# dnbaker/dashing2

Measured on AMD Instinct MI355X. Metric: all-pairs sketch comparison throughput (pairs/s), higher is better.
Workload: dtype u64

## Files before the change

### dashing2_amd/capi.py

```python
import ctypes as C
import os
import subprocess

import numpy as np

_HERE = os.path.dirname(os.path.abspath(__file__))
LIB_PATH = os.environ.get("D2G_LIB") or os.path.join(_HERE, "libd2g.so")
_lib = None

SIMILARITY, CONTAINMENT, SYMMETRIC_CONTAINMENT, POISSON_LLR, INTERSECTION, UNION_SIZE = range(6)
CMP_AUTO, CMP_DIRECT, CMP_BITSLICE, CMP_PLANES = 0, 1, 2, 3
BITSLICE_OPS_PER_GROUP_EXTRA = 1


TIME_K1, TIME_K2, TIME_K2PREP, TIME_K3, TIME_K0 = 2, 4, 8, 16, 32
TIME_KNN = 64
TIME_DEDUP = 128
TIME_FILTER = 256
TIME_KSET = 512
TIME_SCREEN = 1024


class D2GError(RuntimeError):
    def __init__(self, status, detail=""):
# ... 12 lines not shown
_pu64, _pu32, _pdbl, _pf32, _pu8 = (C.POINTER(C.c_uint64), C.POINTER(C.c_uint32), C.POINTER(C.c_double),
                                    C.POINTER(C.c_float), C.POINTER(C.c_uint8))

SIGNATURES = {
    "d2g_version": (_int, []),
    "d2g_strerror": (_cp, [_int]),
    "d2g_device_count": (_int, []),
    "d2g_ctx_create": (_int, [_int, C.POINTER(_vp)]),
    "d2g_ctx_destroy": (None, [_vp]),
    "d2g_last_error": (_cp, [_vp]),
    "d2g_ctx_device": (_int, [_vp]),
    "d2g_ctx_reload_tuning": (_int, [_vp]),
    "d2g_ctx_tuning": (_int, [_vp, C.c_char_p, _sz]),
    "d2g_sync": (_int, [_vp, _vp]),
    "d2g_malloc": (_int, [_vp, _sz, C.POINTER(_vp)]),
    "d2g_free": (_int, [_vp, _vp]),
    "d2g_malloc_host": (_int, [_vp, _sz, C.POINTER(_vp)]),
    "d2g_host_register": (_int, [_vp, _vp, _sz]),
    "d2g_host_unregister": (_int, [_vp, _vp]),
    "d2g_free_host": (_int, [_vp, _vp]),
    "d2g_memcpy_h2d": (_int, [_vp, _vp, _vp, _sz, _vp]),
    "d2g_memcpy_d2h": (_int, [_vp, _vp, _vp, _sz, _vp]),
    "d2g_set_timing": (_int, [_vp, _int]),
    "d2g_kernel_ms": (_int, [_vp, _cp, _int, C.POINTER(_int), C.POINTER(_f32), C.POINTER(_f32)]),
    "d2g_wang_hash": (_u64, [_u64]),
    "d2g_wang_hash_inverse": (_u64, [_u64]),
    "d2g_oph_kmer_ids": (_int, [_vp, _sz, _sz, _sz, _vp]),
    "d2g_seed_mask": (_u64, [_u64]),
    "d2g_oph_xor_const": (_u64, []),
    "d2g_oph_m": (_sz, [_sz]),
    "d2g_oph_card": (_dbl, [_pu64, _sz]),
    "d2g_oph_signatures": (_int, [_pu64, _sz, _pdbl]),
    "d2g_oph_finalize": (_int, [_pu64, _sz, _sz, _sz, _pdbl, _pdbl, _int]),
    "d2g_densify": (_int, [_pdbl, _sz, _sz, C.POINTER(_sz), _int]),
    "d2g_epilogue_gtlt": (_f32, [_u64, _u64, _sz, _dbl, _dbl, _int, _int]),
    "d2g_epilogue_neq": (_f32, [_u64, _sz, _dbl, _dbl, _int, _int]),
    "d2g_epilogue_ut": (_int, [_vp, _vp, _vp, _sz, _sz, _sz, _sz, _int, _int, _int, _int, _vp]),
    "d2g_epilogue_lut": (_int, [_sz, _int, _int, _int, _pf32]),
    "d2g_regs_truncate": (_int, [_vp, _sz, _sz, _int, _int, _vp, _vp, _vp, _int, C.c_char_p, _sz]),
    "d2g_epilogue_trunc_neq": (_f32, [_u64, _sz, _int, _dbl, _dbl, _int, _int]),
    "d2g_epilogue_trunc_gtlt": (_f32, [_u64, _u64, _sz, _vp, _dbl, _dbl, _int, _int]),
    "d2g_epilogue_trunc_ut": (_int, [_vp, _vp, _vp, _sz, _sz, _sz, _sz, _int, _int, _int, _vp, _int, _vp]),
    "d2g_epilogue_trunc_rect": (_int, [_vp, _vp, _vp, _sz, _sz, _sz, _sz, _sz, _sz, _int, _int, _int, _vp, _int, _vp]),
    "d2g_seqpack_create": (_int, [_int, C.POINTER(_vp)]),
    "d2g_seqpack_create_alphabet": (_int, [_int, _int, C.POINTER(_vp)]),
    "d2g_seqpack_alphabet": (_int, [_vp]),
    "d2g_alphabet_size": (_int, [_int]),
    "d2g_alphabet_max_k": (_int, [_int]),
    "d2g_alphabet_code": (_int, [_int, _int]),
    "d2g_alphabet_name": (C.c_char_p, [_int]),
    "d2g_key_bits": (_int, [_int, _int]),
    "d2g_oph_plan_create_alphabet": (_int, [_vp, _vp, _vp, _sz, _vp, _sz, _int, _int, C.POINTER(_vp)]),
    "d2g_sketcher_set_alphabet": (_int, [_vp, _int]),
    "d2g_kmer_filter_create_alphabet": (_int, [_vp, _vp, _sz, _vp, _vp, _sz, _int, _int, C.POINTER(_vp)]),
    "d2g_seqpack_destroy": (None, [_vp]),
    "d2g_seqpack_clear": (None, [_vp]),
    "d2g_seqpack_add_path": (_int, [_vp, _cp]),
    "d2g_seqpack_add_fastx": (_int, [_vp, _cp, _sz]),
    "d2g_seqpack_add_sequence": (_int, [_vp, _cp, _sz]),
    "d2g_seqpack_ngenomes": (_sz, [_vp]),
    "d2g_seqpack_nruns": (_sz, [_vp]),
    "d2g_seqpack_packed_bytes": (_sz, [_vp]),
    "d2g_seqpack_packed": (_pu8, [_vp]),
    "d2g_seqpack_run_start": (_pu64, [_vp]),
    "d2g_seqpack_run_len": (_pu32, [_vp]),
    "d2g_seqpack_genome_run_off": (_pu64, [_vp]),
    "d2g_seqpack_nkmers": (_u64, [_vp, _sz]),
    "d2g_seqpack_nbases": (_u64, [_vp]),
    "d2g_oph_sketch": (_int, [_vp, _vp, _sz, _vp, _vp, _sz, _vp, _sz, _int, _int, _u64, _sz, _vp]),
    "d2g_oph_plan_create": (_int, [_vp, _vp, _vp, _sz, _vp, _sz, _int, C.POINTER(_vp)]),
    "d2g_oph_plan_create_windowed": (_int, [_vp, _vp, _vp, _sz, _vp, _sz, _int, _int, C.POINTER(_vp)]),
    "d2g_run_emissions": (_u64, [_u64, _int, _int]),
    "d2g_sketcher_set_window": (_int, [_vp, _int]),
    "d2g_oph_plan_destroy": (None, [_vp]),
    "d2g_oph_plan_nkmers": (_u64, [_vp]),
    "d2g_oph_plan_nbases": (_u64, [_vp]),
    "d2g_oph_sketch_dev": (_int, [_vp, _vp, _vp, _int, _u64, _sz, _vp, _vp]),
    "d2g_oph_count_dev": (_int, [_vp, _vp, _vp, _int, _u64, _sz, _vp, _vp, _vp]),
    "d2g_oph_sketch_counts": (_int, [_vp, _vp, _sz, _vp, _vp, _sz, _vp, _sz, _int, _int, _u64, _sz, _vp, _vp]),
    "d2g_sketcher_run_counts": (_int, [_vp, _vp, _sz, _vp, _vp, _sz, _vp, _sz, _int, _int, _u64, _sz, _vp, _vp]),
    "d2g_oph_sketch_mincount": (_int, [_vp, _vp, _sz, _vp, _vp, _sz, _vp, _sz, _int, _int, _u64, _sz, C.c_uint32, _vp, _vp]),
    "d2g_sketcher_run_mincount": (_int, [_vp, _vp, _sz, _vp, _vp, _sz, _vp, _sz, _int, _int, _u64, _sz, C.c_uint32, _vp, _vp]),
    "d2g_oph_sketch_mincount_dev": (_int, [_vp, _vp, _vp, _int, _u64, _sz, C.c_uint32, _vp, _vp]),
    "d2g_kmer_filter_create_dev": (_int, [_vp, _vp, _vp, _int, _vp, C.POINTER(_vp)]),
    "d2g_kmer_filter_create": (_int, [_vp, _vp, _sz, _vp, _vp, _sz, _int, _int, C.POINTER(_vp)]),
    "d2g_kmer_filter_create_windowed": (_int, [_vp, _vp, _sz, _vp, _vp, _sz, _int, _int, _int, C.POINTER(_vp)]),
    "d2g_kmer_filter_destroy": (None, [_vp]),
    "d2g_kmer_filter_info": (_int, [_vp, _vp, C.POINTER(_u64), C.POINTER(_u64), C.POINTER(_sz)]),
    "d2g_kmer_filter_contains": (_int, [_vp, _vp, _vp, _sz, _vp]),
    "d2g_screen_create": (_int, [_vp, _vp, _sz, _sz, _int, _int, _u64, _sz, C.POINTER(_vp)]),
    "d2g_screen_destroy": (None, [_vp]),
    "d2g_screen_table_slots": (_int, [_u64, C.POINTER(_u64)]),
    "d2g_screen_reset": (_int, [_vp, _vp]),
    "d2g_screen_info": (_int, [_vp, _vp, C.POINTER(_u64), C.POINTER(_sz), C.POINTER(_sz)]),
    "d2g_screen_fed": (_int, [_vp, _vp, _sz, C.POINTER(_u64)]),
    "d2g_screen_set_fed": (_int, [_vp, _vp, _sz, _u64]),
    "d2g_screen_add_dev": (_int, [_vp, _vp, _vp, _vp, _vp, _vp]),
    "d2g_sketcher_run_screen": (_int, [_vp, _vp, _sz, _vp, _vp, _sz, _vp, _sz, _int, _int, _vp, _vp]),
    "d2g_screen_result": (_int, [_vp, _vp, _sz, _sz, _vp, _vp]),
    "d2g_screen_key_counts": (_int, [_vp, _vp, _sz, _vp, _vp]),
    "d2g_epilogue_contain": (_int, [_vp, _vp, _sz, _sz, _vp, _vp]),
    "d2g_mem_info": (_int, [_vp, C.POINTER(_sz), C.POINTER(_sz)]),
    "d2g_seqpack_add_file": (_int, [_vp, _cp]),
    "d2g_oph_plan_set_filter": (_int, [_vp, _vp]),
    "d2g_sketcher_set_filter": (_int, [_vp, _vp]),
    "d2g_sketcher_create": (_int, [_vp, C.POINTER(_vp)]),
    "d2g_sketcher_destroy": (None, [_vp]),
    "d2g_sketcher_run": (_int, [_vp, _vp, _sz, _vp, _vp, _sz, _vp, _sz, _int, _int, _u64, _sz, _vp]),
    "d2g_sketcher_run_bmh": (_int, [_vp, _vp, _sz, _vp, _vp, _sz, _vp, _sz, _int, _int, _u64, _sz, C.c_double, _vp, _vp]),
    "d2g_bmh_sketch_dev": (_int, [_vp, _vp, _vp, _int, _u64, _sz, C.c_double, _vp, _vp, _vp]),
    "d2g_bmh_sketch": (_int, [_vp, _vp, _sz, _vp, _vp, _sz, _vp, _sz, _int, _int, _u64, _sz, C.c_double, _vp, _vp]),
    "d2g_kmer_count": (_int, [_vp, _vp, _sz, _vp, _vp, _sz, _vp, _sz, _int, _int, _u64, C.c_double, _vp, _vp, _sz, _vp]),
    "d2g_kmer_distinct": (_int, [_vp, _vp, _sz, _vp, _vp, _sz, _vp, _sz, _int, _int, _u64, _vp]),
    "d2g_kmer_sets": (_int, [_vp, _vp, _sz, _vp, _vp, _sz, _vp, _sz, _int, _int, _u64, C.c_double, _vp, _vp, _sz, _vp, _vp]),
    "d2g_sketcher_run_sets": (_int, [_vp, _vp, _sz, _vp, _vp, _sz, _vp, _sz, _int, _int, _u64, C.c_double, _vp, _vp, _sz, _vp, _vp]),
    "d2g_kmer_sets_dev": (_int, [_vp, _vp, _vp, _int, _u64, C.c_double, _vp, _vp, _sz, _vp, _vp, _vp]),
    "d2g_kset_check": (_int, [_vp, _vp, _vp, _sz, C.c_char_p, _sz]),
    "d2g_kset_create": (_int, [_vp, _vp, _vp, _vp, _sz, C.POINTER(_vp)]),
    "d2g_kset_create_dev": (_int, [_vp, _vp, _vp, _vp, _sz, _vp, C.POINTER(_vp)]),
    "d2g_kset_destroy": (None, [_vp]),
    "d2g_kset_size": (_sz, [_vp]),
    "d2g_kset_device_bytes": (_sz, [_vp]),
    "d2g_kset_slice_bits": (_int, [_vp]),
    "d2g_kset_isz_ut_dev": (_int, [_vp, _vp, _sz, _sz, _vp, _vp]),
    "d2g_kset_isz_rect_dev": (_int, [_vp, _vp, _sz, _sz, _sz, _sz, _vp, _vp]),
    "d2g_epilogue_exact": (_f32, [_u64, _dbl, _dbl, _int, _int]),
    "d2g_epilogue_exact_ut": (_int, [_vp, _vp, _sz, _sz, _sz, _int, _int, _int, _vp]),
    "d2g_epilogue_exact_rect": (_int, [_vp, _vp, _sz, _sz, _sz, _sz, _sz, _int, _int, _int, _vp]),
    "d2g_sketcher_run_distinct": (_int, [_vp, _vp, _sz, _vp, _vp, _sz, _vp, _sz, _int, _int, _u64, _vp]),
    "d2g_sketcher_ingest_fasta": (_int, [_vp, _vp, _sz, _vp, _vp, _sz, _vp, _sz, _int]),
    "d2g_sketcher_ingested_runs": (_int, [_vp, C.POINTER(_vp), C.POINTER(_vp), C.POINTER(_sz), C.POINTER(_vp), C.POINTER(_vp), C.POINTER(_u64)]),
    "d2g_seqpack_add_path_by_record": (_int, [_vp, C.c_char_p]),
    "d2g_seqpack_add_fastx_by_record": (_int, [_vp, C.c_char_p, _sz]),
    "d2g_seqpack_name": (C.c_char_p, [_vp, _sz]),
    "d2g_bmh_sketch_cs": (_int, [_vp, _vp, _sz, _vp, _vp, _sz, _vp, _sz, _int, _int, _u64, _sz, _u64, C.c_double, _vp, _vp]),
    "d2g_bmh_sketch_cs_dev": (_int, [_vp, _vp, _vp, _int, _u64, _sz, _u64, C.c_double, _vp, _vp, _vp]),
    "d2g_sketcher_run_bmh_cs": (_int, [_vp, _vp, _sz, _vp, _vp, _sz, _vp, _sz, _int, _int, _u64, _sz, _u64, C.c_double, _vp, _vp]),
    "d2g_countsketch_table": (_int, [_vp, _vp, _sz, _vp, _vp, _sz, _vp, _sz, _int, _int, _u64, _u64, _vp]),
    "d2g_countsketch_cells": (_int, [_vp, _vp, _sz, _vp, _vp, _sz, _vp, _sz, _int, _int, _u64, _u64, C.c_double, _vp, _vp, _sz, _vp, _vp]),
    "d2g_countsketch_lds_cells": (_int, []),
    "d2g_countsketch_stats": (_int, [_vp, _vp, _vp, _vp]),
    "d2g_bmh_check_weights": (_int, [_vp, _vp, _sz, _sz, _dbl, C.c_char_p, _sz]),
    "d2g_bmh_from_weighted": (_int, [_vp, _vp, _vp, _vp, _sz, _sz, _vp, _vp]),
    "d2g_bmh_from_weighted_ids": (_int, [_vp, _vp, _vp, _vp, _sz, _sz, _vp, _vp, _vp]),
    "d2g_ut_count": (_sz, [_sz, _sz, _sz]),
    "d2g_cmp_set_create_dev": (_int, [_vp, _vp, _sz, _sz, _int, _vp, C.POINTER(_vp)]),
    "d2g_cmp_set_create": (_int, [_vp, _vp, _sz, _sz, _int, C.POINTER(_vp)]),
    "d2g_cmp_set_update_dev": (_int, [_vp, _vp, _vp, _vp]),
    "d2g_cmp_set_planes": (_int, [_vp, _vp, _vp, C.POINTER(C.c_uint), C.POINTER(_int), C.POINTER(_f32)]),
    "d2g_cmp_set_status": (_int, [_vp, _vp, _vp]),
    "d2g_cmp_set_sparse_info": (_int, [_vp, _vp, _vp, _vp]),
    "d2g_cmp_set_debug_pairs": (_int, [_vp, _vp, _vp, _vp, _sz, C.POINTER(_sz), _vp]),
    "d2g_cmp_set_sparse_detail": (_int, [_vp, _vp, _vp, _vp]),
    "d2g_sparse_bin_geometry": (_int, [_sz, C.POINTER(C.c_uint32), C.POINTER(C.c_uint32), C.POINTER(C.c_uint32), C.POINTER(_int)]),
    "d2g_warmup": (_int, [_vp, _int]),
    "d2g_device_name": (_int, [_int, C.c_char_p, _sz]),
    "d2g_comm_unique_id": (_int, [_vp]),
    "d2g_comm_create": (_int, [_vp, _vp, _int, _int, C.POINTER(_vp)]),
    "d2g_comm_create_all": (_int, [C.POINTER(_vp), _int, C.POINTER(_vp)]),
    "d2g_comm_destroy": (None, [_vp]),
    "d2g_comm_rank": (_int, [_vp]),
    "d2g_comm_world": (_int, [_vp]),
    "d2g_comm_is_rccl": (_int, [_vp]),
    "d2g_bcast_sigs": (_int, [C.POINTER(_vp), C.POINTER(_vp), _int, _vp, _sz, _sz, C.POINTER(_vp)]),
    "d2g_allpairs_create": (_int, [_vp, _vp, _sz, _sz, C.POINTER(_vp)]),
    "d2g_allpairs_destroy": (None, [_vp]),
    "d2g_allpairs_rows_held": (_int, [_vp, C.POINTER(_sz), C.POINTER(_sz)]),
    "d2g_allpairs_rows_computed": (_int, [_vp, C.POINTER(_sz), C.POINTER(_sz)]),
    "d2g_allpairs_prepare_dev": (_int, [_vp, _vp, _vp]),
    "d2g_allpairs_prepare_all": (_int, [C.POINTER(_vp), _int, C.POINTER(_vp), C.POINTER(_vp)]),
    "d2g_allpairs_operand": (_vp, [_vp]),
    "d2g_allpairs_status": (_int, [_vp, _vp]),
    "d2g_allpairs_chunks": (_int, [_vp]),
    "d2g_allpairs_set_phase_timing": (_int, [_vp, _int]),
    "d2g_allpairs_phase_times": (_int, [_vp, _int, C.POINTER(_int), _vp, _vp, _vp, _vp]),
    "d2g_allpairs_sparse_info": (_int, [_vp, _vp]),
    "d2g_allpairs_step_lut_dev": (_int, [_vp, _vp, _vp, _vp, _vp]),
    "d2g_allpairs_step_eqcount_dev": (_int, [_vp, _vp, _vp, _vp]),
    "d2g_allpairs_step_all": (_int, [C.POINTER(_vp), _int, C.POINTER(_vp), C.POINTER(_vp), C.POINTER(_vp), C.POINTER(_vp)]),
    "d2g_allpairs_enqueue_lut_dev": (_int, [_vp, _vp, _vp, _vp, _vp, _int]),
    "d2g_operand_layout": (_int, [_sz, _sz, C.POINTER(_sz), C.POINTER(_sz)]),
    "d2g_cmp_set_export_operand_dev": (_int, [_vp, _vp, _vp, _vp, _vp]),
    "d2g_cmp_set_from_planes_dev": (_int, [_vp, _sz, _sz, _vp, _vp, C.POINTER(_vp)]),
    "d2g_pack_column_slices_dev": (_int, [_vp, _vp, _sz, _sz, _int, _vp, _vp]),
    "d2g_cmp_set_destroy": (None, [_vp]),
    "d2g_cmp_set_algo": (_int, [_vp]),
    "d2g_cmp_eqcount_ut_dev": (_int, [_vp, _vp, _sz, _sz, _vp, _vp]),
    "d2g_cmp_lut_ut_dev": (_int, [_vp, _vp, _sz, _sz, _vp, _vp, _vp]),
    "d2g_cmp_ut_prefill_dev": (_int, [_vp, _vp, _sz, _sz, _vp, _vp, _vp, _vp]),
    "d2g_cmp_ut_announce_dev": (_int, [_vp, _vp, _sz, _sz, _vp, _vp, _vp]),
    "d2g_cmp_set_forget": (_int, [_vp, _vp]),
    "d2g_cmp_gtlt_ut_dev": (_int, [_vp, _vp, _sz, _sz, _vp, _vp, _vp]),
    "d2g_cmp_eqcount_rect_dev": (_int, [_vp, _vp, _sz, _sz, _sz, _sz, _vp, _vp]),
    "d2g_cmp_gtlt_rect_dev": (_int, [_vp, _vp, _sz, _sz, _sz, _sz, _vp, _vp, _vp]),
    "d2g_cmp_eqcount_ut": (_int, [_vp, _vp, _sz, _sz, _sz, _sz, _int, _vp]),
    "d2g_cmp_dist_ut": (_int, [_vp, _vp, _vp, _sz, _sz, _sz, _sz, _int, _int, _int, _int, _int, _vp]),
    "d2g_ut_partition": (_int, [_sz, _int, C.POINTER(_sz)]),
    "d2g_cmp_set_create_codes_dev": (_int, [_vp, _vp, _sz, _sz, _int, _vp, C.POINTER(_vp)]),
    "d2g_cmp_set_create_codes": (_int, [_vp, _vp, _sz, _sz, _int, C.POINTER(_vp)]),
    "d2g_cmp_set_operand_bytes": (_sz, [_vp]),
    "d2g_cmp_set_id_bits": (_int, [_vp]),
    "d2g_cmp_dist_trunc_ut": (_int, [_vp, _vp, _vp, _sz, _sz, _sz, _sz, _int, _int, _int, _int, _int, _vp]),
    "d2g_cmp_knn_dev": (_int, [_vp, _vp, _sz, _sz, _sz, C.c_uint32, _vp, _sz, _vp, _vp, _vp, _sz, _vp]),
    "d2g_knn_finish": (_int, [_vp, _vp, _vp, _sz, _sz, _vp, _sz, _int, _vp, _vp, _vp, _sz, C.POINTER(_sz), C.POINTER(_sz)]),
    "d2g_cmp_set_knn": (_int, [_vp, _vp, _sz, _sz, _vp, _int, _sz, _dbl, _sz, _sz, _vp, _vp, _vp, _sz, C.POINTER(_sz)]),
    "d2g_cmp_knn": (_int, [_vp, _vp, _sz, _sz, _sz, _sz, _int, _int, _int, _int, _sz, _dbl, _sz, _sz, _vp, _vp, _vp, _sz, C.POINTER(_sz)]),
    "d2g_cmp_dedup_dev": (_int, [_vp, _vp, C.c_uint32, _vp, _vp, _sz, _vp]),
    "d2g_dedup_clusters": (_int, [_vp, _sz, _vp, _vp, C.POINTER(_sz)]),
    "d2g_cmp_set_dedup": (_int, [_vp, _vp, _vp, _dbl, _sz, _vp]),
    "d2g_cmp_dedup": (_int, [_vp, _vp, _sz, _sz, _int, _int, _int, _int, _dbl, _sz, _vp]),
}


def sparse_info_dict(a):
    return {"sorted_operand": bool(a[0]), "tiles_listed": int(a[1]), "dense_decided_by_prepare": bool(a[2] & 1), "dense_kernel_ran": bool(a[2] & 2),
            "tiles_and_pair_list": bool(a[2] & 4), "callers_order_kept": bool(a[2] & 8), "ordering_skipped": bool(a[2] & 16), "pairs_listed": int(a[3])}


def lib():
    global _lib
    if _lib is None:
        if os.environ.get("D2G_NO_TORCH_PRELOAD") != "1":
            try:
                import torch
            except Exception:
                pass
        if not os.path.exists(LIB_PATH):
            raise OSError(f"{LIB_PATH} is missing: run `python -c 'import __graft_entry__ as g; g.build()'` "
                          "(dashing2_amd has no CPU fallback)")
        l = C.CDLL(LIB_PATH)
        for name, (res, args) in SIGNATURES.items():
            try:
                f = getattr(l, name)
            except AttributeError:
                if os.environ.get("D2G_LIB"):
                    continue
                raise
            f.restype = res
            f.argtypes = args
        _lib = l
    return _lib


def _np_ptr(a):
    return a.ctypes.data if a is not None else None


class _Runs:

    def __init__(self, src, canon):
        if hasattr(src, "arrays"):
            src = tuple(src.arrays()) + (src.k,)
        elif src[0] is None:
            src = (None,) + tuple(src[1][:3]) + (src[2],)
        packed, rs, rl, go, self.k = src
        self.packed = None if packed is None else np.ascontiguousarray(packed, np.uint8)
        self.rs, self.rl, self.go = np.ascontiguousarray(rs, np.uint64), np.ascontiguousarray(rl, np.uint32), np.ascontiguousarray(go, np.uint64)
        self.n = self.go.size - 1
        self.args = (_np_ptr(self.packed), 0 if packed is None else self.packed.size, _np_ptr(self.rs), _np_ptr(self.rl), self.rs.size,
                     _np_ptr(self.go), self.n, self.k, int(canon))

    @property
    def nkmers(self):
        return int(self.rl.astype(np.int64).sum()) - (self.k - 1) * self.rl.size if self.rl.size else 0


def wang_hash(x):
    return int(lib().d2g_wang_hash(x & 0xFFFFFFFFFFFFFFFF))


def wang_hash_inverse(x):
    return int(lib().d2g_wang_hash_inverse(x & 0xFFFFFFFFFFFFFFFF))


SCREEN_MAX_KEYS = 1 << 30


def run_emissions(length, k, w=0):
    return int(lib().d2g_run_emissions(int(length), int(k), int(w)))


def countsketch_lds_cells():
    return int(lib().d2g_countsketch_lds_cells())


def screen_table_slots(ndistinct):
    s = _u64()
    rc = lib().d2g_screen_table_slots(ndistinct, C.byref(s))
    if rc:
        raise D2GError(rc)
    return int(s.value)


def epilogue_contain(matches, matchsums, S):
    m = np.ascontiguousarray(matches, np.uint32)
    s = np.ascontiguousarray(matchsums, np.uint32)
    cov, dep = np.empty(m.shape, np.float32), np.empty(m.shape, np.float32)
    rc = lib().d2g_epilogue_contain(_np_ptr(m), _np_ptr(s), m.size, S, _np_ptr(cov), _np_ptr(dep))
    if rc:
        raise D2GError(rc)
    return cov, dep


def oph_kmer_ids(regs, S):
    regs = np.ascontiguousarray(regs, np.uint64)
    n, m = regs.shape
# ... 885 lines not shown

    def close(self):
        if getattr(self, "_h", None):
            lib().d2g_kmer_filter_destroy(self._h)
            self._h = None

    __del__ = close


class Screen:

    def __init__(self, ctx, h, nrefs, S, k, canon, nrows):
        self.ctx, self._h, self.nrefs, self.S, self.k, self.canon, self.nrows = ctx, h, nrefs, S, k, canon, nrows

    def info(self):
        nd, tb, cb = _u64(), _sz(), _sz()
        self.ctx._check(lib().d2g_screen_info(self.ctx._h, self._h, C.byref(nd), C.byref(tb), C.byref(cb)))
        return int(nd.value), int(tb.value), int(cb.value)

    def reset(self):
        self.ctx._check(lib().d2g_screen_reset(self.ctx._h, self._h))

    def fed(self, row):
        n = _u64()
        self.ctx._check(lib().d2g_screen_fed(self.ctx._h, self._h, row, C.byref(n)))
        return int(n.value)

    def set_fed(self, row, nkmers):
        self.ctx._check(lib().d2g_screen_set_fed(self.ctx._h, self._h, row, nkmers))

    def add_dev(self, plan, packed_dev_ptr, genome_row, stream=None):
        rows = np.ascontiguousarray(genome_row, np.uint32)
        assert rows.size == plan.n
        self.ctx._check(lib().d2g_screen_add_dev(self.ctx._h, self._h, plan._h, packed_dev_ptr, _np_ptr(rows), stream))

    def result(self, row0=0, nrows=None):
        nrows = self.nrows - row0 if nrows is None else nrows
        m = np.zeros((nrows, self.nrefs), np.uint32)
        s = np.zeros((nrows, self.nrefs), np.uint32)
        self.ctx._check(lib().d2g_screen_result(self.ctx._h, self._h, row0, nrows, _np_ptr(m), _np_ptr(s)))
        return m, s

    def key_counts(self, row):
        D = self.info()[0]
        keys, cnt = np.zeros(D, np.uint64), np.zeros(D, np.uint32)
        self.ctx._check(lib().d2g_screen_key_counts(self.ctx._h, self._h, row, _np_ptr(keys), _np_ptr(cnt)))
        return keys, cnt

    def close(self):
        if getattr(self, "_h", None):
            lib().d2g_screen_destroy(self._h)
            self._h = None

    __del__ = close


class KSet:

    def __init__(self, ctx, h):
        self.ctx, self._h = ctx, h
        self.N = int(lib().d2g_kset_size(h))

    @property
    def device_bytes(self):
        return int(lib().d2g_kset_device_bytes(self._h))

    @property
    def slice_bits(self):
        return int(lib().d2g_kset_slice_bits(self._h))

    def isz_ut_dev(self, r0, r1, out_dev_ptr, stream=None):
        self.ctx._check(lib().d2g_kset_isz_ut_dev(self.ctx._h, self._h, r0, r1, out_dev_ptr, stream))

    def isz_rect_dev(self, a0, a1, b0, b1, out_dev_ptr, stream=None):
        self.ctx._check(lib().d2g_kset_isz_rect_dev(self.ctx._h, self._h, a0, a1, b0, b1, out_dev_ptr, stream))

    def close(self):
        if getattr(self, "_h", None):
            lib().d2g_kset_destroy(self._h)
            self._h = None

    __del__ = close


class OphPlan:
    def __init__(self, ctx, h, n):
        self.ctx, self._h, self.n = ctx, h, n

    def set_filter(self, filt):
        self.ctx._check(lib().d2g_oph_plan_set_filter(self._h, filt._h if filt is not None else None))
        self._filter = filt

    @property
    def nkmers(self):
        return int(lib().d2g_oph_plan_nkmers(self._h))

    @property
    def nbases(self):
        return int(lib().d2g_oph_plan_nbases(self._h))

    def close(self):
        if self._h:
            lib().d2g_oph_plan_destroy(self._h)
            self._h = None

    __del__ = close


class CmpSet:

    def __init__(self, ctx, h, N, S, owned=True):
        self.ctx, self._h, self.N, self.S, self._owned = ctx, h, N, S, owned

    @property
    def algo(self):
        return int(lib().d2g_cmp_set_algo(self._h))

    @property
    def operand_bytes(self):
        return int(lib().d2g_cmp_set_operand_bytes(self._h))

    @property
    def id_bits(self):
        return int(lib().d2g_cmp_set_id_bits(self._h))

    def close(self):
        if getattr(self, "_h", None):
            if self._owned:
                lib().d2g_cmp_set_destroy(self._h)
            self._h = None

    __del__ = close

    def export_operand_dev(self, planes_out_ptr, meta_out_ptr, stream=None):
        self.ctx._check(lib().d2g_cmp_set_export_operand_dev(self.ctx._h, self._h, planes_out_ptr, meta_out_ptr, stream))

    def update_dev(self, dev_ptr, stream=None):
        self.ctx._check(lib().d2g_cmp_set_update_dev(self.ctx._h, self._h, dev_ptr, stream))

    def status(self, stream=None):
        self.ctx._check(lib().d2g_cmp_set_status(self.ctx._h, self._h, stream))

    def sparse_info(self, stream=None):
        a = np.zeros(4, np.uint32)
        self.ctx._check(lib().d2g_cmp_set_sparse_info(self.ctx._h, self._h, stream, a.ctypes.data))
        return sparse_info_dict(a)

    def sparse_detail(self, stream=None):
        a = np.zeros(10, np.uint64)
        self.ctx._check(lib().d2g_cmp_set_sparse_detail(self.ctx._h, self._h, stream, a.ctypes.data))
        return {"looked": bool(a[0]), "looked_dense": bool(a[1]), "entries": int(a[2]), "family_pairs": int(a[3]), "shared_values": int(a[4]),
                "planes": int(a[5]), "binned": bool(a[6]), "bin_cshift": int(a[7]), "schedule": "merged" if a[8] else "classic", "prepare_kernels": int(a[9])}

    def debug_pairs(self, cap=1 << 24, stream=None):
        buf = np.empty(cap, np.uint64)
        roots = np.empty(self.N, np.uint32)
        n = _sz()
        self.ctx._check(lib().d2g_cmp_set_debug_pairs(self.ctx._h, self._h, stream, buf.ctypes.data, cap, C.byref(n), roots.ctypes.data))
        e = buf[:n.value]
        e = e[e != np.uint64(0xFFFFFFFFFFFFFFFF)]
        return np.stack([(e & np.uint64(0xFFFFFFFF)).astype(np.uint32), (e >> np.uint64(32)).astype(np.uint32)], axis=1), roots

    def planes(self, stream=None):
        md, nb, mean = C.c_uint(), _int(), _f32()
        self.ctx._check(lib().d2g_cmp_set_planes(self.ctx._h, self._h, stream, C.byref(md), C.byref(nb), C.byref(mean)))
        return int(md.value), int(nb.value), float(mean.value)

    def eqcount_ut_dev(self, out_dev_ptr, r0=0, r1=None, stream=None):
        r1 = self.N if r1 is None else r1
        self.ctx._check(lib().d2g_cmp_eqcount_ut_dev(self.ctx._h, self._h, r0, r1, out_dev_ptr, stream))

    def lut_ut_dev(self, lut_dev_ptr, out_dev_ptr, r0=0, r1=None, stream=None):
        r1 = self.N if r1 is None else r1
        self.ctx._check(lib().d2g_cmp_lut_ut_dev(self.ctx._h, self._h, r0, r1, lut_dev_ptr, out_dev_ptr, stream))

    def prefill_ut_dev(self, out_dev_ptr, r0=0, r1=None, lut_dev_ptr=None, stream=None):
        r1 = self.N if r1 is None else r1
        if lut_dev_ptr is None:
            self.ctx._check(lib().d2g_cmp_ut_prefill_dev(self.ctx._h, self._h, r0, r1, out_dev_ptr, None, None, stream))
        else:
            self.ctx._check(lib().d2g_cmp_ut_prefill_dev(self.ctx._h, self._h, r0, r1, None, lut_dev_ptr, out_dev_ptr, stream))

    def forget(self):
        self.ctx._check(lib().d2g_cmp_set_forget(self.ctx._h, self._h))

    def announce_ut_dev(self, out_dev_ptr, r0=0, r1=None, lut_dev_ptr=None):
        r1 = self.N if r1 is None else r1
        if lut_dev_ptr is None:
            self.ctx._check(lib().d2g_cmp_ut_announce_dev(self.ctx._h, self._h, r0, r1, out_dev_ptr, None, None))
        else:
            self.ctx._check(lib().d2g_cmp_ut_announce_dev(self.ctx._h, self._h, r0, r1, None, lut_dev_ptr, out_dev_ptr))

    def gtlt_ut_dev(self, gt_dev_ptr, lt_dev_ptr, r0=0, r1=None, stream=None):
        r1 = self.N if r1 is None else r1
        self.ctx._check(lib().d2g_cmp_gtlt_ut_dev(self.ctx._h, self._h, r0, r1, gt_dev_ptr, lt_dev_ptr, stream))

    def eqcount_rect_dev(self, out_dev_ptr, a0, a1, b0, b1, stream=None):
        self.ctx._check(lib().d2g_cmp_eqcount_rect_dev(self.ctx._h, self._h, a0, a1, b0, b1, out_dev_ptr, stream))

    def knn_dev(self, rowcnt_dev_ptr, ids_dev_ptr, counts_dev_ptr, cap, K=0, min_count=0, cls_dev_ptr=None, r0=0, r1=None,
                band_rows=0, stream=None):
        r1 = self.N if r1 is None else r1
        self.ctx._check(lib().d2g_cmp_knn_dev(self.ctx._h, self._h, r0, r1, K, min_count, cls_dev_ptr, cap, rowcnt_dev_ptr, ids_dev_ptr,
                                              counts_dev_ptr, band_rows, stream))

    def knn(self, lut, isdist=False, K=0, threshold=0.0, r0=0, r1=None, cap=0, band_rows=0):
        lut = np.ascontiguousarray(lut, np.float32)
        assert lut.size == self.S + 1
        r1 = self.N if r1 is None else r1
        return _knn_csr(self.ctx, r1 - r0, K, lambda ip, ix, dt, oc, need: lib().d2g_cmp_set_knn(
            self.ctx._h, self._h, r0, r1, _np_ptr(lut), int(bool(isdist)), K, float(threshold), cap, band_rows, ip, ix, dt, oc, need))

    def dedup_dev(self, assign_dev_ptr, min_count, cls_dev_ptr=None, band_rows=0, stream=None):
        self.ctx._check(lib().d2g_cmp_dedup_dev(self.ctx._h, self._h, min_count, cls_dev_ptr, assign_dev_ptr, band_rows, stream))

    def dedup(self, lut, threshold, band_rows=0):
        lut = np.ascontiguousarray(lut, np.float32)
        assert lut.size == self.S + 1
        out = np.empty(self.N, np.uint32)
        self.ctx._check(lib().d2g_cmp_set_dedup(self.ctx._h, self._h, _np_ptr(lut), float(threshold), band_rows, _np_ptr(out)))
        return out

    def gtlt_rect_dev(self, gt_dev_ptr, lt_dev_ptr, a0, a1, b0, b1, stream=None):
        self.ctx._check(lib().d2g_cmp_gtlt_rect_dev(self.ctx._h, self._h, a0, a1, b0, b1, gt_dev_ptr, lt_dev_ptr, stream))

    def eqcount_ut(self, r0=0, r1=None):
        r1 = self.N if r1 is None else r1
        out = np.empty(ut_count(self.N, r0, r1) if r0 <= r1 <= self.N else 0, np.uint32)
        d = self.ctx.malloc(max(out.nbytes, 4))
        try:
            self.eqcount_ut_dev(d, r0, r1)
            if out.size:
                self.ctx.d2h(out, d)
        finally:
            self.ctx.free(d)
        return out

    def gtlt_ut(self, r0=0, r1=None):
        r1 = self.N if r1 is None else r1
        n = ut_count(self.N, r0, r1)
        gt, lt = np.empty(n, np.uint32), np.empty(n, np.uint32)
        if n == 0:
            return gt, lt
        dg, dl = self.ctx.malloc(gt.nbytes), self.ctx.malloc(lt.nbytes)
        try:
            self.gtlt_ut_dev(dg, dl, r0, r1)
            self.ctx.d2h(gt, dg)
            self.ctx.d2h(lt, dl)
        finally:
            self.ctx.free(dg)
            self.ctx.free(dl)
        return gt, lt

    def gtlt_rect(self, a0, a1, b0, b1):
        gt, lt = np.empty((a1 - a0, b1 - b0), np.uint32), np.empty((a1 - a0, b1 - b0), np.uint32)
        if gt.size == 0:
            return gt, lt
        dg, dl = self.ctx.malloc(gt.nbytes), self.ctx.malloc(lt.nbytes)
        try:
            self.gtlt_rect_dev(dg, dl, a0, a1, b0, b1)
            self.ctx.d2h(gt, dg)
            self.ctx.d2h(lt, dl)
        finally:
            self.ctx.free(dg)
            self.ctx.free(dl)
        return gt, lt

    def eqcount_rect(self, a0, a1, b0, b1):
        out = np.empty((a1 - a0, b1 - b0), np.uint32)
        if out.size == 0:
            return out
        d = self.ctx.malloc(out.nbytes)
        try:
            self.eqcount_rect_dev(d, a0, a1, b0, b1)
            self.ctx.d2h(out, d)
        finally:
            self.ctx.free(d)
        return out

    def lut_ut(self, lut, r0=0, r1=None):
        r1 = self.N if r1 is None else r1
        lut = np.ascontiguousarray(lut, np.float32)
        out = np.empty(ut_count(self.N, r0, r1), np.float32)
        if out.size == 0:
            return out
        dl, d = self.ctx.malloc(lut.nbytes), self.ctx.malloc(out.nbytes)
        try:
            self.ctx.h2d(dl, lut)
            self.lut_ut_dev(dl, d, r0, r1)
            self.ctx.d2h(out, d)
        finally:
            self.ctx.free(dl)
            self.ctx.free(d)
        return out


COMM_ID_BYTES = 128


def comm_unique_id():
    buf = C.create_string_buffer(COMM_ID_BYTES)
    rc = lib().d2g_comm_unique_id(buf)
    if rc:
        raise D2GError(rc, "d2g_comm_unique_id (RCCL not loadable?)")
    return buf.raw

# ... 124 lines not shown
```

### dashing2_amd/csrc/d2g_internal.h

```cpp
#pragma once
#include "../../include/d2g.h"
#include <hip/hip_runtime.h>
#include <cstdio>
#include <memory>
#include <string>
#include <utility>

#include <vector>
struct d2g_ctx;
int d2g_hip_status(d2g_ctx *ctx, hipError_t e, const char *what);

template <class T, bool Pinned> class d2g_owned {
    T *p_ = nullptr; size_t cap_ = 0;
public:
    d2g_owned() = default;
    d2g_owned(d2g_owned &&o) noexcept : p_(o.p_), cap_(o.cap_) { o.p_ = nullptr; o.cap_ = 0; }
    d2g_owned &operator=(d2g_owned &&o) noexcept { if (this != &o) { reset(); p_ = o.p_; cap_ = o.cap_; o.p_ = nullptr; o.cap_ = 0; } return *this; }
    ~d2g_owned() { reset(); }
    void reset() { if (p_) (void)(Pinned ? hipHostFree(p_) : hipFree(p_)); p_ = nullptr; cap_ = 0; }
    int alloc(d2g_ctx *ctx, size_t n, const char *what, unsigned flags = hipHostMallocDefault) {
        reset();
        const hipError_t e = Pinned ? hipHostMalloc((void **)&p_, n * sizeof(T), flags) : hipMalloc((void **)&p_, n * sizeof(T));
        if (e != hipSuccess) p_ = nullptr; else cap_ = n;
        return d2g_hip_status(ctx, e, what);
    }
    int grow(d2g_ctx *ctx, size_t need, size_t slack, const char *what = "work buffer", unsigned flags = hipHostMallocDefault) {
        return need <= cap_ ? D2G_OK : alloc(ctx, need + need / 4 + slack, what, flags);
    }
    T *get() const { return p_; }
    operator T *() const { return p_; }
    size_t cap() const { return cap_; }
};
template <class T> using d2g_dev = d2g_owned<T, false>;
template <class T> using d2g_pinned = d2g_owned<T, true>;

template <class H, hipError_t (*Destroy)(H)> class d2g_handle {
protected:
    H h_ = nullptr;
public:
    d2g_handle() = default;
    d2g_handle(d2g_handle &&o) noexcept : h_(o.h_) { o.h_ = nullptr; }
    d2g_handle &operator=(d2g_handle &&o) noexcept { if (this != &o) { reset(); h_ = o.h_; o.h_ = nullptr; } return *this; }
    ~d2g_handle() { reset(); }
    void reset() { if (h_) (void)Destroy(h_); h_ = nullptr; }
    operator H() const { return h_; }
};
struct d2g_stream : d2g_handle<hipStream_t, hipStreamDestroy> {
    hipError_t create(unsigned flags = hipStreamDefault) { reset(); return hipStreamCreateWithFlags(&h_, flags); }
};
struct d2g_event : d2g_handle<hipEvent_t, hipEventDestroy> {
    hipError_t create(unsigned flags = hipEventDefault) { reset(); return hipEventCreateWithFlags(&h_, flags); }
};

struct d2g_evlog {
    std::vector<d2g_event> a, b;
};

struct d2g_tuning {
    std::vector<std::pair<std::string, std::string>> kv;
    const char *get(const char *name) const {
        for (const auto &p : kv) if (p.first == name) return p.second.c_str();
        return nullptr;
    }
};
void d2g_tuning_load(d2g_tuning &t);
struct d2g_k2_tuning {
    bool sparse = true;
    size_t min_n = 8192;
    int link = 1;
    double tile_frac = 0.35;
    int olink = 1;
    int emit_big = 0;
    int ride = 63;
    int merge = 1;
    int remember = 1;
    size_t long_list = 786432;
    int predict = 1;
    int list_form = 0;
    size_t list_div = 8;
    bool sort = true;
    int tagbits_max = 31;
    int id16 = 1;
    int nsplit_req = 0;
};
d2g_k2_tuning d2g_k2_tuning_resolve(const d2g_tuning &t);
std::string d2g_k2_tuning_json(const d2g_ctx *ctx);
uint64_t d2g_k2_tuning_hash(const d2g_ctx *ctx);

constexpr int K3_MAXBBITS = 12;
constexpr int K3_ROUND_KEYS = 1400;
constexpr int K3_TARGET = 1024;
constexpr int K3_L1BITS = 8;
constexpr uint64_t K3_SPLIT_MIN = 4 * 1400;
struct d2g_k3_tuning {
    bool compact = false;
    bool light = true;
    uint32_t l1bits = K3_L1BITS;
    uint64_t bucket_keys = K3_TARGET;
    uint64_t sub_keys = K3_TARGET;
    uint64_t split_min = 0;
    size_t subbatch = 0;
    uint32_t round_keys = K3_ROUND_KEYS;
    double guess_scale = 1.0;
    size_t grid_per_cu = 48;
    bool gq_scale_set = false;
    double gq_scale = 2.0;
    uint64_t gq_slack = 256;
    uint64_t sort_keys = K3_TARGET;
    uint64_t cs_table_bytes = 0;
    int cs_lds_cells = -1;
};
struct d2g_kset_tuning {
    int split = 0;
    int pbits = -1;
};
d2g_k3_tuning d2g_k3_tuning_resolve(const d2g_tuning &t);
constexpr int MG_MAX_CHUNKS = 4;
void d2g_tuning_resolve(d2g_ctx *ctx);

struct d2g_ctx {
    int device = -1;
    d2g_tuning tune;
    d2g_k2_tuning k2;
    d2g_k3_tuning k3_tune;
    d2g_kset_tuning kset;
    int mgpu_chunks = 0;
    int num_cus = 0;
    std::string last_error;
    int timing = 0;
    d2g_evlog ev_k1, ev_k2, ev_k2prep, ev_k3, ev_k0, ev_knn;
    d2g_evlog ev_k1count;
    d2g_evlog ev_filter;
    d2g_evlog ev_k3k, ev_k3kcompact, ev_k3kbmh;
    d2g_evlog ev_k3s, ev_kset, ev_ksetprep;
    d2g_evlog ev_screen, ev_screenreduce, ev_screenbuild;
    d2g_evlog ev_dedup, ev_dedup_resolve;
    struct d2g_k3_state *k3 = nullptr;
    uint64_t cs_table_bytes = 0, cs_groups = 0, cs_batches = 0;
    d2g_dev<uint32_t> knn_band;
    d2g_dev<unsigned long long> dedup_keys;
};
void d2g_k3_state_destroy(struct d2g_k3_state *st);
void d2g_screen_rank_keys(const uint64_t *keys, size_t n, uint64_t xormask, std::vector<uint64_t> &distinct, std::vector<uint64_t> &raw,
                          std::vector<uint32_t> &rank);
inline int d2g_hip_status(d2g_ctx *ctx, hipError_t e, const char *what) {
    if (e == hipSuccess) return D2G_OK;
    ctx->last_error = std::string(what) + ": " + hipGetErrorString(e);
    return e == hipErrorOutOfMemory ? D2G_ERR_NOMEM : D2G_ERR_HIP;
}

#define D2G_HIP(ctx, call)                                                            \
    do {                                                                              \
        hipError_t e__ = (call);                                                      \
        if (e__ != hipSuccess) {                                                      \
            (ctx)->last_error = std::string(#call) + ": " + hipGetErrorString(e__);   \
            return e__ == hipErrorOutOfMemory ? D2G_ERR_NOMEM : D2G_ERR_HIP;          \
        }                                                                             \
    } while (0)

#define D2G_CHECK(ctx, cond, msg)                      \
    do {                                               \
        if (!(cond)) {                                 \
            (ctx)->last_error = (msg);                 \
            return D2G_ERR_INVALID;                    \
        }                                              \
    } while (0)

struct d2g_timer {
    d2g_evlog *ev; hipStream_t s; bool on;
    d2g_timer(d2g_ctx *c, d2g_evlog *e, hipStream_t st) : ev(e), s(st), on(false) {
        const int bit = (e == &c->ev_k1 || e == &c->ev_k1count) ? D2G_TIME_K1 : e == &c->ev_k2 ? D2G_TIME_K2 : e == &c->ev_k2prep ? D2G_TIME_K2PREP : e == &c->ev_k0 ? D2G_TIME_K0 : e == &c->ev_knn ? D2G_TIME_KNN : e == &c->ev_filter ? D2G_TIME_FILTER : (e == &c->ev_k3s || e == &c->ev_kset || e == &c->ev_ksetprep) ? D2G_TIME_KSET : (e == &c->ev_dedup || e == &c->ev_dedup_resolve) ? D2G_TIME_DEDUP : (e == &c->ev_screen || e == &c->ev_screenreduce || e == &c->ev_screenbuild) ? D2G_TIME_SCREEN : D2G_TIME_K3;
        on = (c->timing & bit) != 0;
        if (on) {
            d2g_event x, y;
            if (x.create() != hipSuccess || y.create() != hipSuccess) { on = false; return; }
            (void)hipEventRecord(x, s);
            ev->a.push_back(std::move(x)); ev->b.push_back(std::move(y));
        }
    }
    void stop() { if (on) (void)hipEventRecord(ev->b.back(), s); }
};

void d2g_warm_filter(); void d2g_warm_k0(); void d2g_warm_k1(); void d2g_warm_k2(); void d2g_warm_k2_bitslice(); void d2g_warm_k2_planes(); void d2g_warm_k3(); void d2g_warm_kset(); void d2g_warm_screen(); void d2g_warm_knn(); void d2g_warm_dedup();

static inline hipStream_t as_stream(void *s) { return reinterpret_cast<hipStream_t>(s); }

template <class T> static inline T div_up(T a, T b) { return (a + b - 1) / b; }
```

### dashing2_amd/csrc/d2g_k2.h

```cpp
#pragma once
#include "d2g_internal.h"

#include <algorithm>

struct SpRider { uint32_t *out; size_t cnt; const uint32_t *vsrc; uint32_t vimm, own, piece0; };
constexpr SpRider SP_NO_RIDER{nullptr, 0, nullptr, 0u, 0xFFFFFFFFu, 0u};
constexpr int SP_FILL_PER_THREAD = 8, SP_FILL_THREADS = 256;
inline size_t sp_fill_pieces(size_t cnt) { return div_up<size_t>(cnt / 4 + 1, (size_t)SP_FILL_THREADS * SP_FILL_PER_THREAD); }
#ifndef D2G_SP_RW_M_LINK0
#define D2G_SP_RW_M_LINK0 8
#endif
#ifndef D2G_SP_RW_M_PLANES
#define D2G_SP_RW_M_PLANES 5
#endif
constexpr unsigned SP_RW_PLAN = 6, SP_RW_FLATTEN = 5, SP_RW_COUNT = 5, SP_RW_ATTACH = 5, SP_RW_SCAN = 8, SP_RW_ALL = 35;
constexpr unsigned SP_RW_M_LINK0 = D2G_SP_RW_M_LINK0, SP_RW_M_PLANES = D2G_SP_RW_M_PLANES;

struct SpInit {
    uint32_t *label = nullptr, *ones = nullptr, *zero = nullptr;
    uint32_t n = 0, owords = 0, zwords = 0;
};
#ifdef __HIPCC__
__device__ __forceinline__ void sp_init_part(const SpInit &si, size_t lin, size_t nthreads) {
    if (!si.label) return;
    if (lin < si.n) si.label[lin] = (uint32_t)lin;
    for (size_t x = lin; x < si.owords; x += nthreads) si.ones[x] = 0xFFFFFFFFu;
    for (size_t x = lin; x < si.zwords; x += nthreads) si.zero[x] = 0;
}
#endif

struct SpAnnounced {
    uint32_t *out = nullptr; size_t cnt = 0; const uint32_t *vsrc = nullptr; uint32_t vimm = 0;
    uint32_t next = 0, total = 0;
    int mask = 0;
    void announce(uint32_t *o, size_t n, const uint32_t *src) { out = o; cnt = n; vsrc = src; vimm = 0; }
    void cancel() { out = nullptr; }
    void served() { out = nullptr; total = 0; }
    void begin(int ride_mask, bool carry) {
        mask = ride_mask; next = 0;
        const size_t pieces = sp_fill_pieces(cnt);
        total = (out && carry && mask && pieces <= 0x7FFFFFFFu) ? (uint32_t)pieces : 0u;
    }
    uint32_t riding() const { return total; }
    SpRider take_all() { next = total; return SpRider{out, cnt, vsrc, vimm, 0u, 0u}; }
    SpRider take(unsigned own, unsigned weight, bool last, int bit, unsigned *grid) {
        *grid = own;
        if (next >= total || !(mask & bit)) return SP_NO_RIDER;
        const uint32_t left = total - next;
        uint32_t n = last ? left : (uint32_t)std::min<uint64_t>(left, ((uint64_t)total * weight + SP_RW_ALL - 1) / SP_RW_ALL);
        n = std::min<uint32_t>(n, 0x7FFFFFFFu - own);
        const SpRider r{out, cnt, vsrc, vimm, own, next};
        next += n;
        *grid = own + n;
        return r;
    }
};

struct SpFilled {
    uint32_t *out = nullptr;
    size_t cnt = 0;
    size_t pieces = 0;
    const uint32_t *src = nullptr;
    bool by_riders = false;
    void set_early(uint32_t *o, size_t n, const uint32_t *s) { out = o; cnt = n; pieces = (size_t)-1; src = s; by_riders = false; }
    void set_by_riders(const SpAnnounced &a) { out = a.out; cnt = a.cnt; pieces = a.next; src = a.vsrc; by_riders = true; }
    size_t done_for(const uint32_t *o, size_t n, const uint32_t *s, size_t npieces) const { return (out == o && cnt == n && src == s) ? std::min(pieces, npieces) : 0; }
    void void_after_prepare() { if (by_riders) out = nullptr; }
    void clear() { out = nullptr; }
};

enum SpMappedWord : uint32_t { SP_MW_GAVEUP = 0, SP_MW_LIST_LEN = 1, SP_MW_SUMS = 2, SP_MW_TICKET = 6, SP_MW_WORDS = 16 };

struct SpDecision {
    unsigned prepares = 0; bool skipped = false;
    bool merged = false; unsigned kernels = 0;
    int skip_cached = -1;
    bool sample_pending = false; uint32_t sample_ticket = 0;
    bool pred_valid = false, pred_dense = false; double pred_entries = 0, pred_family_pairs = 0;
    bool big = true;
    bool looked = false, looked_dense = false; uint32_t samp_sums[4] = {0, 0, 0, 0};
};

struct SpState {
    unsigned sp_launch = 0;
    d2g_dev<uint32_t> d_stream_s;
    d2g_dev<uint32_t> d_sperm;
    d2g_dev<uint32_t> d_sinv;
    d2g_dev<uint32_t> d_label;
    d2g_dev<uint32_t> d_owner;
    size_t owner_stride = 0;
    d2g_dev<uint32_t> d_segend;
    d2g_dev<uint32_t> d_posseg;
    d2g_dev<uint32_t> d_hint;
    d2g_dev<uint32_t> d_spz;
    size_t spz_words = 0;
    uint32_t *d_lcnt = nullptr;
    uint32_t *d_gbm = nullptr;
    uint32_t *d_order = nullptr;
    uint32_t *d_plctl = nullptr;
    d2g_dev<uint32_t> d_rowpos;
    d2g_dev<uint32_t> d_rowk;
    d2g_dev<uint32_t> d_rowstream;
    d2g_dev<uint32_t> d_tiles, d_spctl; uint32_t *d_tilebm = nullptr;
    d2g_dev<uint32_t> d_tiles_full; uint32_t *d_fullctl = nullptr;
    bool full_list_valid = false;
    d2g_pinned<uint32_t> h_gaveup; uint32_t *d_gaveup = nullptr;
    d2g_stream fill_stream; d2g_event fill_fork, fill_join;
    d2g_stream samp_stream; d2g_event samp_event;
    d2g_dev<uint32_t> d_samp;
    SpDecision dec;
    SpAnnounced announced;
    SpFilled filled;
    const uint32_t *last_ctl = nullptr;
    d2g_dev<unsigned long long> d_plist;
    size_t plist_cap = 0;
    d2g_dev<unsigned long long> d_plist2;
    uint32_t *d_binc = nullptr;
    d2g_dev<uint32_t> d_bstart;
    d2g_dev<uint32_t> d_cw_ents; d2g_dev<unsigned long long> d_cw_vals; size_t cw_ecap = 0, cw_vcap = 0;
    d2g_dev<uint32_t> d_hoff;
    uint32_t nbins = 0, bin_nch = 0, bin_cshift = 10, bin_nwg = 1;
    bool bin_ok = true;
    size_t tilebm_words = 0, tiles_cap = 0;
};

struct d2g_cmp_set {
    d2g_ctx *ctx = nullptr;
    size_t N = 0, S = 0;
    size_t Npad = 0;
    int algo = D2G_CMP_DIRECT;
    d2g_dev<uint64_t> d_rows;
    d2g_dev<uint64_t> d_cols;
    d2g_dev<uint32_t> d_cplanes;
    int cplanes = 0;
    d2g_dev<uint32_t> own_planes, own_meta;
    uint32_t *d_planes = nullptr;
    d2g_dev<uint32_t> d_stream;
    size_t Nstride = 0;
    int nbits_cap = 0;
    int ntb = 0;
    uint32_t *d_meta = nullptr;
    d2g_dev<uint32_t> d_ids;
    int id_bits = 32;
    uint32_t T = 0; int logT = 0;
    bool borrowed = false;
    bool want_exchange = false;
    d2g_dev<uint32_t> d_colcnt;
    d2g_dev<uint32_t> d_perm;
    int nsplit = 1;
    bool export_only = false;
    uint32_t *ex_planes = nullptr, *ex_meta = nullptr, *ex_status = nullptr;
    bool managed = false;
    const uint32_t *status_words = nullptr; int n_status = 0;
    std::unique_ptr<SpState> sp;
    bool sparse_ok() const { return sp != nullptr; }
    size_t ncols = 0;
    bool srt_valid = false;
    mutable bool nat_valid = false;
};
constexpr int BS_CC_STRIDE = 8;

struct PairShape;
int  finish_shape(d2g_ctx *ctx, PairShape &sh, unsigned rb);

int  d2g_planes_gtlt(d2g_ctx *ctx, const d2g_cmp_set *set, const PairShape &sh, uint32_t *gt, uint32_t *lt, hipStream_t s);
int  d2g_planes_eq(d2g_ctx *ctx, const d2g_cmp_set *set, const PairShape &sh, uint32_t *eq, hipStream_t s);

void d2g_bitslice_geometry(d2g_cmp_set *set);
int  d2g_bitslice_alloc(d2g_ctx *ctx, d2g_cmp_set *set);
int  d2g_bitslice_prepare(d2g_ctx *ctx, d2g_cmp_set *set, hipStream_t s);
int  d2g_bitslice_export(d2g_ctx *ctx, d2g_cmp_set *set, hipStream_t s);
int  d2g_bitslice_alloc_stream(d2g_ctx *ctx, d2g_cmp_set *set);
int  d2g_bitslice_ensure_natural(d2g_ctx *ctx, const d2g_cmp_set *set, hipStream_t s);
int  d2g_bitslice_managed_sparse_alloc(d2g_ctx *ctx, d2g_cmp_set *set);
int  d2g_bitslice_managed_ready(d2g_ctx *ctx, d2g_cmp_set *set, hipStream_t s);
int  d2g_bitslice_sparse_info(d2g_ctx *ctx, const d2g_cmp_set *set, hipStream_t s, uint32_t *out4);
int  d2g_bitslice_sparse_detail(d2g_ctx *ctx, const d2g_cmp_set *set, hipStream_t s, uint64_t *out10);
SpInit d2g_bitslice_sp_init(const d2g_cmp_set *set);
int  d2g_bitslice_debug_read(d2g_ctx *ctx, const d2g_cmp_set *set, hipStream_t s, uint64_t *pairs_out, size_t cap, size_t *npairs, uint32_t *root_out);
int  d2g_bitslice_status(d2g_ctx *ctx, const d2g_cmp_set *set, hipStream_t s);
int  d2g_bitslice_exporter_create(d2g_ctx *ctx, size_t N, size_t S_local, d2g_cmp_set **out);
void d2g_bitslice_set_export_target(d2g_cmp_set *set, uint32_t *planes, uint32_t *meta, uint32_t *status);
int  d2g_bitslice_prepare_slice(d2g_ctx *ctx, d2g_cmp_set *set, const uint64_t *rows_dev, hipStream_t s);
int  d2g_bitslice_derive_groups(d2g_ctx *ctx, const d2g_cmp_set *set, int g0, int g1, hipStream_t s);
int  d2g_bitslice_ut(d2g_ctx *ctx, const d2g_cmp_set *set, size_t r0, size_t r1, uint32_t *eq_out,
                     const float *lut, float *fout, hipStream_t s);
int  d2g_bitslice_prefill(d2g_ctx *ctx, d2g_cmp_set *set, size_t r0, size_t r1, uint32_t *eq_out, const float *lut, float *fout, hipStream_t s);
int  d2g_bitslice_announce(d2g_ctx *ctx, d2g_cmp_set *set, size_t r0, size_t r1, uint32_t *eq_out, const float *lut, float *fout);
void d2g_bitslice_forget(d2g_cmp_set *set);
int  d2g_bitslice_rect(d2g_ctx *ctx, const d2g_cmp_set *set, size_t a0, size_t a1, size_t b0, size_t b1,
                       uint32_t *eq_out, hipStream_t s);
```

### dashing2_amd/csrc/d2g_k2.hip

```cpp
#include "d2g_internal.h"
#include "d2g_k2.h"
#include "d2g_k2_shape.h"
#include <algorithm>
#include <new>
#include <vector>

namespace {

constexpr int K2_THREADS = 256;
constexpr int K2_IW = 8;
constexpr int K2_JR = 4;
constexpr int K2_RB = 4 * K2_IW;
constexpr int K2_CB = 64 * K2_JR;
constexpr int K2_TC = 2;

}
int finish_shape(d2g_ctx *ctx, PairShape &sh, unsigned rb) {
    sh.rb = rb;
    sh.nrt = (unsigned)div_up<size_t>(sh.i_hi - sh.i_lo, rb);
    sh.ct0 = (unsigned)(sh.j_lo / 256);
    sh.nct = (unsigned)(div_up<size_t>(sh.j_hi, 256) - sh.ct0);
    size_t total = 0;
    for (unsigned c = 0; c < sh.nct; ++c) total += tiles_in_column(sh, c);
    D2G_CHECK(ctx, total < (1ull << 31), "pair tile grid too large; shard rows");
// ... 147 lines not shown
    delete set;
}

int d2g_cmp_set_algo(const d2g_cmp_set *set) { return set ? set->algo : D2G_ERR_INVALID; }

int d2g_cmp_set_id_bits(const d2g_cmp_set *set) { return (set && set->algo == D2G_CMP_BITSLICE && set->d_ids) ? set->id_bits : 0; }

size_t d2g_cmp_set_operand_bytes(const d2g_cmp_set *set) {
    if (!set) return 0;
    return (set->d_rows.cap() + set->d_cols.cap()) * sizeof(uint64_t) +
           (set->own_planes.cap() + set->d_stream.cap() + (set->sp ? set->sp->d_stream_s.cap() : 0) + set->d_cplanes.cap()) * sizeof(uint32_t);
}

#define D2G_NO_CODE_SET(ctx, set, what) D2G_CHECK(ctx, (set)->algo != D2G_CMP_PLANES, what ": not available for a set of truncated codes")

static int cmp_set_load(d2g_ctx *ctx, d2g_cmp_set *set, const uint64_t *sig_bits_dev, hipStream_t s) {
    const size_t N = set->N, S = set->S;
    if (set->d_rows) D2G_HIP(ctx, hipMemcpyAsync(set->d_rows, sig_bits_dev, N * S * sizeof(uint64_t), hipMemcpyDeviceToDevice, s));
    d2g_timer tm(ctx, &ctx->ev_k2prep, s);
    launch_transpose(ctx, sig_bits_dev, set->d_cols, N, S, set->Npad, set->algo == D2G_CMP_BITSLICE ? set->d_meta + set->ntb : nullptr,
                     set->algo == D2G_CMP_BITSLICE ? d2g_bitslice_sp_init(set) : SpInit{}, s);
    int rc = D2G_OK;
    if (set->algo == D2G_CMP_BITSLICE) rc = d2g_bitslice_prepare(ctx, set, s);
    tm.stop();
    if (rc) return rc;
    D2G_HIP(ctx, hipGetLastError());
    return D2G_OK;
}

}

int d2g_bitslice_prepare_slice(d2g_ctx *ctx, d2g_cmp_set *set, const uint64_t *rows_dev, hipStream_t s) {
    d2g_timer tm(ctx, &ctx->ev_k2prep, s);
    launch_transpose(ctx, rows_dev, set->d_cols, set->N, set->S, set->Npad, set->d_meta + set->ntb, d2g_bitslice_sp_init(set), s);
    const int rc = d2g_bitslice_prepare(ctx, set, s);
    tm.stop();
    if (rc) return rc;
    D2G_HIP(ctx, hipGetLastError());
    return D2G_OK;
}

extern "C" {

int d2g_cmp_set_create_dev(d2g_ctx *ctx, const uint64_t *sig_bits_dev, size_t N, size_t S, int algo,
                           void *stream, d2g_cmp_set **out) {
    if (!ctx || !out) return D2G_ERR_INVALID;
    *out = nullptr;
    D2G_CHECK(ctx, N >= 1 && S >= 1, "cmp_set: empty matrix");
    D2G_CHECK(ctx, S < (1ull << 31), "cmp_set: sketchsize too large");
    D2G_CHECK(ctx, sig_bits_dev != nullptr, "cmp_set: null signatures");
    D2G_CHECK(ctx, algo == D2G_CMP_AUTO || algo == D2G_CMP_DIRECT || algo == D2G_CMP_BITSLICE, "cmp_set: bad algo");
    D2G_HIP(ctx, hipSetDevice(ctx->device));
    hipStream_t s = as_stream(stream);
    d2g_cmp_set *set = new (std::nothrow) d2g_cmp_set();
    if (!set) return D2G_ERR_NOMEM;
    set->ctx = ctx; set->N = N; set->S = S;
    set->Npad = div_up<size_t>(N, K2_CB) * K2_CB;
    if (int rc = set->d_cols.alloc(ctx, set->Npad * S, "cmp_set alloc")) { d2g_cmp_set_destroy(set); return rc; }
    set->algo = D2G_CMP_DIRECT;
    if (algo != D2G_CMP_DIRECT) {
        int rc = d2g_bitslice_alloc(ctx, set);
        if (rc == D2G_OK) set->algo = D2G_CMP_BITSLICE;
        else if (!(rc == D2G_ERR_UNSUPPORTED && algo == D2G_CMP_AUTO)) { d2g_cmp_set_destroy(set); return rc; }
    }
    if (set->algo == D2G_CMP_DIRECT) {
        if (int rc = set->d_rows.alloc(ctx, (N + K2_RB) * S, "cmp_set alloc")) { d2g_cmp_set_destroy(set); return rc; }
        (void)hipMemsetAsync(set->d_rows + N * S, 0, (size_t)K2_RB * S * sizeof(uint64_t), s);
    }
    int rc = cmp_set_load(ctx, set, sig_bits_dev, s);
    if (rc) { d2g_cmp_set_destroy(set); return rc; }
    *out = set;
    return D2G_OK;
}

int d2g_cmp_set_update_dev(d2g_ctx *ctx, d2g_cmp_set *set, const uint64_t *sig_bits_dev, void *stream) {
    if (!ctx) return D2G_ERR_INVALID;
    D2G_CHECK(ctx, set && set->ctx == ctx, "cmp_set_update: set belongs to another context");
    D2G_CHECK(ctx, !set->borrowed, "cmp_set_update: this set wraps a caller-owned operand");
    D2G_NO_CODE_SET(ctx, set, "cmp_set_update");
    D2G_CHECK(ctx, sig_bits_dev != nullptr, "cmp_set_update: null signatures");
    D2G_HIP(ctx, hipSetDevice(ctx->device));
    return cmp_set_load(ctx, set, sig_bits_dev, as_stream(stream));
}

int d2g_cmp_set_planes(d2g_ctx *ctx, const d2g_cmp_set *set, void *stream, unsigned *max_distinct, int *nbits, float *mean_nbits) {
    if (!ctx) return D2G_ERR_INVALID;
    D2G_CHECK(ctx, set && set->ctx == ctx, "cmp_set_planes: set belongs to another context");
    unsigned md = 0; int nb = 0;
    if (set->algo == D2G_CMP_BITSLICE) {
        std::vector<unsigned> m(set->ntb);
        D2G_HIP(ctx, hipSetDevice(ctx->device));
        D2G_HIP(ctx, hipMemcpyAsync(m.data(), set->d_meta, m.size() * sizeof(unsigned), hipMemcpyDeviceToHost, as_stream(stream)));
        D2G_HIP(ctx, hipStreamSynchronize(as_stream(stream)));
        double sum = 0;
        if (int rc = d2g_bitslice_status(ctx, set, as_stream(stream))) return rc;
        for (unsigned x : m) {
            md = std::max(md, x);
            int b = 1;
            while ((1ull << b) <= x) ++b;
            nb = std::max(nb, b);
            sum += b;
        }
        if (mean_nbits) *mean_nbits = m.empty() ? 0.f : float(sum / m.size());
    } else if (mean_nbits) *mean_nbits = 0.f;
    if (max_distinct) *max_distinct = md;
    if (nbits) *nbits = nb;
    return D2G_OK;
}

int d2g_cmp_set_create(d2g_ctx *ctx, const uint64_t *sig_bits_host, size_t N, size_t S, int algo, d2g_cmp_set **out) {
    if (!ctx || !out) return D2G_ERR_INVALID;
    D2G_CHECK(ctx, sig_bits_host != nullptr && N >= 1 && S >= 1, "cmp_set: bad host matrix");
    D2G_HIP(ctx, hipSetDevice(ctx->device));
    d2g_dev<uint64_t> tmp;
    if (int rc = tmp.alloc(ctx, N * S, "cmp_set staging alloc")) return rc;
    hipError_t e = hipMemcpy(tmp, sig_bits_host, N * S * sizeof(uint64_t), hipMemcpyHostToDevice);
    if (e != hipSuccess) { ctx->last_error = hipGetErrorString(e); return D2G_ERR_HIP; }
    int rc = d2g_cmp_set_create_dev(ctx, tmp, N, S, algo, nullptr, out);
    (void)hipStreamSynchronize(nullptr);
    if (rc == D2G_OK && (*out)->algo == D2G_CMP_BITSLICE && d2g_bitslice_status(ctx, *out, nullptr) != D2G_OK) {
        d2g_cmp_set_destroy(*out);
        *out = nullptr;
        rc = algo == D2G_CMP_AUTO ? d2g_cmp_set_create_dev(ctx, tmp, N, S, D2G_CMP_DIRECT, nullptr, out) : (int)D2G_ERR_INTERNAL;
        (void)hipStreamSynchronize(nullptr);
    }
    return rc;
}

int d2g_cmp_set_sparse_info(d2g_ctx *ctx, const d2g_cmp_set *set, void *stream, uint32_t *info4) {
    if (!ctx || !set || !info4) return D2G_ERR_INVALID;
    D2G_NO_CODE_SET(ctx, set, "cmp_set_sparse_info");
    D2G_HIP(ctx, hipSetDevice(ctx->device));
    if (set->algo != D2G_CMP_BITSLICE) { info4[0] = info4[1] = info4[2] = info4[3] = 0; return D2G_OK; }
    return d2g_bitslice_sparse_info(ctx, set, as_stream(stream), info4);
}

int d2g_cmp_set_debug_pairs(d2g_ctx *ctx, const d2g_cmp_set *set, void *stream, uint64_t *pairs_out, size_t cap, size_t *npairs, uint32_t *root_out) {
    if (!ctx || !set || !npairs) return D2G_ERR_INVALID;
    D2G_NO_CODE_SET(ctx, set, "cmp_set_debug_pairs");
    D2G_HIP(ctx, hipSetDevice(ctx->device));
    *npairs = 0;
    if (set->algo != D2G_CMP_BITSLICE) return D2G_OK;
    return d2g_bitslice_debug_read(ctx, set, as_stream(stream), pairs_out, cap, npairs, root_out);
}

int d2g_cmp_set_sparse_detail(d2g_ctx *ctx, const d2g_cmp_set *set, void *stream, uint64_t *out10) {
    if (!ctx || !out10) return D2G_ERR_INVALID;
    D2G_CHECK(ctx, set && set->ctx == ctx, "cmp_set_sparse_detail: set belongs to another context");
    D2G_NO_CODE_SET(ctx, set, "cmp_set_sparse_detail");
    D2G_HIP(ctx, hipSetDevice(ctx->device));
    for (int x = 0; x < 10; ++x) out10[x] = 0;
    if (set->algo != D2G_CMP_BITSLICE) { D2G_HIP(ctx, hipStreamSynchronize(as_stream(stream))); return D2G_OK; }
    return d2g_bitslice_sparse_detail(ctx, set, as_stream(stream), out10);
}

int d2g_cmp_set_status(d2g_ctx *ctx, const d2g_cmp_set *set, void *stream) {
    if (!ctx) return D2G_ERR_INVALID;
    D2G_CHECK(ctx, set && set->ctx == ctx, "cmp_set_status: set belongs to another context");
    D2G_HIP(ctx, hipSetDevice(ctx->device));
    if (set->algo != D2G_CMP_BITSLICE) { D2G_HIP(ctx, hipStreamSynchronize(as_stream(stream))); return D2G_OK; }
    return d2g_bitslice_status(ctx, set, as_stream(stream));
}

static int check_rows(d2g_ctx *ctx, const d2g_cmp_set *set, size_t r0, size_t r1) {
    D2G_CHECK(ctx, set && set->ctx == ctx, "cmp: set belongs to another context");
    D2G_CHECK(ctx, r0 <= r1 && r1 <= set->N, "cmp: row range out of bounds");
    return D2G_OK;
}

int d2g_cmp_eqcount_ut_dev(d2g_ctx *ctx, const d2g_cmp_set *set, size_t r0, size_t r1, uint32_t *out, void *stream) {
    if (!ctx) return D2G_ERR_INVALID;
    if (int rc = check_rows(ctx, set, r0, r1)) return rc;
    if (d2g_ut_count(set->N, r0, r1) == 0) return D2G_OK;
    D2G_CHECK(ctx, out != nullptr, "cmp: null output");
    D2G_HIP(ctx, hipSetDevice(ctx->device));
    if (set->algo == D2G_CMP_BITSLICE) return d2g_bitslice_ut(ctx, set, r0, r1, out, nullptr, nullptr, as_stream(stream));
    if (set->algo == D2G_CMP_PLANES) return d2g_planes_eq(ctx, set, ut_shape(set->N, r0, r1), out, as_stream(stream));
    return launch_direct<false>(ctx, set, ut_shape(set->N, r0, r1), StoreEq{out}, as_stream(stream));
}

int d2g_cmp_lut_ut_dev(d2g_ctx *ctx, const d2g_cmp_set *set, size_t r0, size_t r1, const float *lut, float *out, void *stream) {
    if (!ctx) return D2G_ERR_INVALID;
    if (int rc = check_rows(ctx, set, r0, r1)) return rc;
    D2G_NO_CODE_SET(ctx, set, "cmp_lut_ut");
    if (d2g_ut_count(set->N, r0, r1) == 0) return D2G_OK;
    D2G_CHECK(ctx, out != nullptr && lut != nullptr, "cmp: null output/lut");
    D2G_HIP(ctx, hipSetDevice(ctx->device));
    if (set->algo == D2G_CMP_BITSLICE) return d2g_bitslice_ut(ctx, set, r0, r1, nullptr, lut, out, as_stream(stream));
    return launch_direct<false>(ctx, set, ut_shape(set->N, r0, r1), StoreLut{out, lut}, as_stream(stream));
}

int d2g_cmp_ut_prefill_dev(d2g_ctx *ctx, d2g_cmp_set *set, size_t r0, size_t r1, uint32_t *neq_out, const float *lut, float *out, void *stream) {
    if (!ctx) return D2G_ERR_INVALID;
    if (int rc = check_rows(ctx, set, r0, r1)) return rc;
    D2G_NO_CODE_SET(ctx, set, "cmp_ut_prefill");
    if (d2g_ut_count(set->N, r0, r1) == 0) return D2G_OK;
    D2G_CHECK(ctx, (neq_out != nullptr) != (lut != nullptr && out != nullptr), "cmp prefill: give the count output, or the table and the float output");
    if (set->algo != D2G_CMP_BITSLICE) return D2G_OK;
    D2G_HIP(ctx, hipSetDevice(ctx->device));
    return d2g_bitslice_prefill(ctx, set, r0, r1, neq_out, lut, out, as_stream(stream));
}

int d2g_cmp_ut_announce_dev(d2g_ctx *ctx, d2g_cmp_set *set, size_t r0, size_t r1, uint32_t *neq_out, const float *lut, float *out) {
    if (!ctx) return D2G_ERR_INVALID;
    if (int rc = check_rows(ctx, set, r0, r1)) return rc;
    D2G_NO_CODE_SET(ctx, set, "cmp_ut_announce");
    if (d2g_ut_count(set->N, r0, r1) == 0) return D2G_OK;
    if (set->algo != D2G_CMP_BITSLICE || set->borrowed) return D2G_OK;
    D2G_CHECK(ctx, (!neq_out && !out) || (neq_out != nullptr) != (lut != nullptr && out != nullptr), "cmp announce: give the count output, or the table and the float output");
    return d2g_bitslice_announce(ctx, set, r0, r1, neq_out, lut, out);
}

int d2g_cmp_set_forget(d2g_ctx *ctx, d2g_cmp_set *set) {
    if (!ctx) return D2G_ERR_INVALID;
    D2G_CHECK(ctx, set && set->ctx == ctx, "cmp_set_forget: set belongs to another context");
    if (set->algo == D2G_CMP_BITSLICE) d2g_bitslice_forget(set);
    return D2G_OK;
}

int d2g_cmp_gtlt_ut_dev(d2g_ctx *ctx, const d2g_cmp_set *set, size_t r0, size_t r1, uint32_t *gt, uint32_t *lt, void *stream) {
    if (!ctx) return D2G_ERR_INVALID;
    if (int rc = check_rows(ctx, set, r0, r1)) return rc;
    if (d2g_ut_count(set->N, r0, r1) == 0) return D2G_OK;
    D2G_CHECK(ctx, gt != nullptr && lt != nullptr, "cmp: null output");
    if (set->algo == D2G_CMP_PLANES) {
        D2G_HIP(ctx, hipSetDevice(ctx->device));
        return d2g_planes_gtlt(ctx, set, ut_shape(set->N, r0, r1), gt, lt, as_stream(stream));
    }
    D2G_CHECK(ctx, set->d_rows != nullptr, "cmp: (gt,lt) needs the raw patterns: create the set with D2G_CMP_DIRECT");
    D2G_HIP(ctx, hipSetDevice(ctx->device));
    return launch_direct<true>(ctx, set, ut_shape(set->N, r0, r1), StoreGtLt{gt, lt, (uint32_t)set->S}, as_stream(stream));
}

int d2g_cmp_eqcount_rect_dev(d2g_ctx *ctx, const d2g_cmp_set *set, size_t a0, size_t a1, size_t b0, size_t b1,
                             uint32_t *out, void *stream) {
    if (!ctx) return D2G_ERR_INVALID;
    D2G_CHECK(ctx, set && set->ctx == ctx, "cmp: set belongs to another context");
    D2G_CHECK(ctx, a0 <= a1 && a1 <= set->N && b0 <= b1 && b1 <= set->N, "cmp: rect out of bounds");
    if (a0 == a1 || b0 == b1) return D2G_OK;
    D2G_CHECK(ctx, out != nullptr, "cmp: null output");
    D2G_HIP(ctx, hipSetDevice(ctx->device));
    const PairShape sh = rect_shape(set->N, a0, a1, b0, b1);
    if (set->algo == D2G_CMP_BITSLICE) return d2g_bitslice_rect(ctx, set, a0, a1, b0, b1, out, as_stream(stream));
    if (set->algo == D2G_CMP_PLANES) return d2g_planes_eq(ctx, set, sh, out, as_stream(stream));
    return launch_direct<false>(ctx, set, sh, StoreEq{out}, as_stream(stream));
}

int d2g_cmp_gtlt_rect_dev(d2g_ctx *ctx, const d2g_cmp_set *set, size_t a0, size_t a1, size_t b0, size_t b1,
                          uint32_t *gt, uint32_t *lt, void *stream) {
    if (!ctx) return D2G_ERR_INVALID;
    D2G_CHECK(ctx, set && set->ctx == ctx, "cmp: set belongs to another context");
    D2G_CHECK(ctx, a0 <= a1 && a1 <= set->N && b0 <= b1 && b1 <= set->N, "cmp: rect out of bounds");
    if (a0 == a1 || b0 == b1) return D2G_OK;
    D2G_CHECK(ctx, gt != nullptr && lt != nullptr, "cmp: null output");
    D2G_CHECK(ctx, set->d_rows != nullptr || set->algo == D2G_CMP_PLANES, "cmp: (gt,lt) needs the raw patterns: create the set with D2G_CMP_DIRECT");
    D2G_HIP(ctx, hipSetDevice(ctx->device));
    const PairShape sh = rect_shape(set->N, a0, a1, b0, b1);
    if (set->algo == D2G_CMP_PLANES) return d2g_planes_gtlt(ctx, set, sh, gt, lt, as_stream(stream));
    return launch_direct<true>(ctx, set, sh, StoreGtLt{gt, lt, (uint32_t)set->S}, as_stream(stream));
}

int d2g_operand_layout(size_t N, size_t S, size_t *group_words, size_t *ngroups) {
    if (!N || !S) return D2G_ERR_INVALID;
    d2g_cmp_set tmp;
    tmp.N = N; tmp.S = S; tmp.Npad = div_up<size_t>(N, K2_CB) * K2_CB;
    d2g_bitslice_geometry(&tmp);
    if (group_words) *group_words = (size_t)(tmp.nbits_cap + 1) * tmp.Nstride;
    if (ngroups) *ngroups = (size_t)tmp.ntb;
    return D2G_OK;
}

int d2g_cmp_set_export_operand_dev(d2g_ctx *ctx, const d2g_cmp_set *set, uint32_t *planes_out_dev, uint32_t *meta_out_dev, void *stream) {
    if (!ctx) return D2G_ERR_INVALID;
    D2G_CHECK(ctx, set && set->ctx == ctx, "export_operand: set belongs to another context");
    D2G_CHECK(ctx, set->algo == D2G_CMP_BITSLICE, "export_operand: not a bit-sliced set");
    D2G_CHECK(ctx, planes_out_dev && meta_out_dev, "export_operand: null output");
    D2G_HIP(ctx, hipSetDevice(ctx->device));
    const size_t words = (size_t)set->ntb * (set->nbits_cap + 1) * set->Nstride;
    if (int rc = d2g_bitslice_export(ctx, const_cast<d2g_cmp_set *>(set), as_stream(stream))) return rc;
    D2G_HIP(ctx, hipMemcpyAsync(planes_out_dev, set->d_planes, words * sizeof(uint32_t), hipMemcpyDeviceToDevice, as_stream(stream)));
    D2G_HIP(ctx, hipMemcpyAsync(meta_out_dev, set->d_meta, (size_t)set->ntb * sizeof(uint32_t), hipMemcpyDeviceToDevice, as_stream(stream)));
    return D2G_OK;
}

int d2g_cmp_set_from_planes_dev(d2g_ctx *ctx, size_t N, size_t S, const uint32_t *planes_dev, const uint32_t *meta_dev, d2g_cmp_set **out) {
    if (!ctx || !out) return D2G_ERR_INVALID;
    *out = nullptr;
    D2G_CHECK(ctx, N >= 1 && S >= 1 && N < (1ull << 30) && S < (1ull << 31), "from_planes: bad shape");
    D2G_CHECK(ctx, planes_dev && meta_dev, "from_planes: null operand");
    d2g_cmp_set *set = new (std::nothrow) d2g_cmp_set();
    if (!set) return D2G_ERR_NOMEM;
    set->ctx = ctx; set->N = N; set->S = S;
    set->Npad = div_up<size_t>(N, K2_CB) * K2_CB;
    d2g_bitslice_geometry(set);
    set->algo = D2G_CMP_BITSLICE;
    set->borrowed = true;
    set->d_planes = const_cast<uint32_t *>(planes_dev);
    set->d_meta = const_cast<uint32_t *>(meta_dev);
    D2G_HIP(ctx, hipSetDevice(ctx->device));
    if (int rc = d2g_bitslice_alloc_stream(ctx, set)) { delete set; return rc; }
    *out = set;
    return D2G_OK;
}

int d2g_pack_column_slices_dev(d2g_ctx *ctx, const uint64_t *rows_dev, size_t n, size_t S, int W, uint64_t *out_dev, void *stream) {
    if (!ctx) return D2G_ERR_INVALID;
// ... 79 lines not shown
```

### dashing2_amd/csrc/d2g_k2_bitslice.hip

```cpp
#include "d2g_internal.h"
#include "d2g_k2.h"
#include "d2g_k2_shape.h"
#include <chrono>
#include <cstring>
#include <algorithm>
#include <vector>

namespace {

typedef uint32_t u32x16 __attribute__((ext_vector_type(16)));
typedef u32x16 __attribute__((aligned(4))) u32x16_u;
constexpr uint32_t BS_EMPTY = 0xFFFFFFFFu;
constexpr int BS_RANK_THREADS = 1024;

constexpr uint32_t BS_DUP = 0x80000000u;
constexpr uint32_t BS_UNIQ = 0x80000000u;
constexpr uint32_t BS_PENDING = 0x40000000u;
constexpr int BS_LOG_TLDS_MAX = 15;
template <typename IdT> struct BsId;
template <> struct BsId<uint32_t> { static constexpr uint32_t UNIQ = BS_UNIQ; static constexpr int UBIT = 31; };
template <> struct BsId<uint16_t> { static constexpr uint32_t UNIQ = 0x8000u; static constexpr int UBIT = 15; };
constexpr size_t BS_ID16_MAX_N = ((size_t(1) << BS_LOG_TLDS_MAX) * 2) / 3;
static_assert(BS_ID16_MAX_N / 2 < BsId<uint16_t>::UNIQ, "16-bit ids: the highest rank (N / 2) must stay below the unique flag");
static_assert((size_t(1) << BS_LOG_TLDS_MAX) - 1 <= 0xFFFFu, "16-bit ids: the general single-partition kernel parks a table slot in ids[] between its two loops");

__device__ __forceinline__ uint32_t bs_hash(uint64_t v, int logT) {
    return (uint32_t)((v * 0x9E3779B97F4A7C15ull) >> (64 - logT));
}

constexpr uint32_t BS_SPLIT_SHIFT = 28, BS_RANK_MASK = (1u << BS_SPLIT_SHIFT) - 1u;
#ifdef D2G_RANK_TRACE
__device__ unsigned long long g_rank_trace[8192 * 16];
#define RK_STAMP(k) do { if (threadIdx.x == 0 && blockIdx.x < 8192 && (k) < 16) g_rank_trace[blockIdx.x * 16 + (k)] = __builtin_amdgcn_s_memrealtime(); } while (0)
#else
#define RK_STAMP(k) do { } while (0)
#endif
template <bool MULTI, bool FAST, typename IdT = uint32_t>
__global__ __launch_bounds__(BS_RANK_THREADS) void bs_rank_kernel(const uint64_t *__restrict__ cols, size_t N, size_t Npad,
                                                                  uint32_t T, int logT, void *ids_void, uint32_t *colcnt,
                                                                  uint32_t *status, int tagbits_max, uint32_t S, int nsplit,
                                                                  uint32_t *__restrict__ owner_all, size_t ostride) {
    extern __shared__ __attribute__((aligned(16))) uint32_t own[];
    const uint32_t split = MULTI ? blockIdx.x / S : 0u;
    const size_t t = MULTI ? blockIdx.x - split * S : blockIdx.x;
    const uint32_t htag = (MULTI && nsplit > 1) ? split << BS_SPLIT_SHIFT : 0u;
    const uint64_t *col = cols + t * Npad;
    static_assert(!MULTI || sizeof(IdT) == 4, "bs_rank_kernel: the pending words and split tags of the MULTI kernel need 32-bit ids");
    IdT *ids = static_cast<IdT *>(ids_void) + t * Npad;
    const int tid = threadIdx.x;
    const int logTl = logT < BS_LOG_TLDS_MAX ? logT : BS_LOG_TLDS_MAX;
    const uint32_t Tl = 1u << logTl, mask = Tl - 1, nparts = MULTI ? (T >> logTl) : 1u;
    const uint32_t part_lo = MULTI ? split * (nparts / (uint32_t)nsplit) : 0u, part_hi = MULTI ? part_lo + nparts / (uint32_t)nsplit : 1u;
    __shared__ uint32_t wave_tot[BS_RANK_THREADS / 64];
    __shared__ uint32_t running;
    constexpr uint32_t BS_MAXFIX = 64;
    __shared__ uint32_t nfix, fix_j[BS_MAXFIX], fix_h[BS_MAXFIX];
    RK_STAMP(0);
    if (tid == 0) { running = 1; nfix = 0; }
    const int lane = tid & 63, wave = tid >> 6;
    uint32_t *owner = (owner_all && nsplit == 1) ? owner_all + t * ostride : nullptr;
    const int ib0 = 32 - __clz((uint32_t)N);
    const uint32_t ownmask = (ib0 >= 32 ? 0xFFFFFFFFu : (1u << ib0) - 1u) & ~BS_DUP;

    auto compact = [&]() {
        uint32_t cnt = 0;
        for (uint32_t h = tid; h < Tl; h += BS_RANK_THREADS) {
            const uint32_t cur = own[h];
            cnt += (cur != BS_EMPTY) && (cur & BS_DUP);
        }
        uint32_t incl = cnt;
        for (int o = 1; o < 64; o <<= 1) { const uint32_t x = __shfl_up(incl, o); if (lane >= o) incl += x; }
        if (lane == 63) wave_tot[wave] = incl;
        __syncthreads();
        uint32_t woff = 0, tot = 0;
        for (int w = 0; w < BS_RANK_THREADS / 64; ++w) {
            const uint32_t x = wave_tot[w];
            if (w < wave) woff += x;
            tot += x;
        }
        uint32_t r = running + woff + (incl - cnt);
        for (uint32_t h = tid; h < Tl; h += BS_RANK_THREADS) {
            const uint32_t cur = own[h];
            if (cur != BS_EMPTY) {
                if ((cur & BS_DUP) && owner) owner[r - 1] = cur & ownmask;
                own[h] = (cur & BS_DUP) ? (r++ | htag) : BsId<IdT>::UNIQ;
            }
        }
        __syncthreads();
        if (tid == 0) running += tot;
        __syncthreads();
    };
    const int ib = 32 - __clz((uint32_t)N);
    const uint32_t idxmask = (ib >= 32 ? 0xFFFFFFFFu : (1u << ib) - 1u) & ~BS_DUP;
    const uint32_t tagfield = ~BS_DUP & ~idxmask & (ib + tagbits_max >= 31 ? 0xFFFFFFFFu : (1u << (ib + tagbits_max)) - 1u);
    auto slot_word = [&](uint64_t prod, uint32_t j) {
        return j | ((uint32_t)((prod << logT) >> 33) & tagfield);
    };
    auto insert = [&](uint64_t v, uint32_t j, uint32_t h) {
        const uint32_t mine = slot_word(v * 0x9E3779B97F4A7C15ull, j);
        for (uint32_t probes = 0; probes < Tl; ++probes) {
            const uint32_t cur = atomicCAS(&own[h], BS_EMPTY, mine);
            if (cur == BS_EMPTY) return h;
            if (!((cur ^ mine) & tagfield) && col[cur & idxmask] == v) {
                if (!(cur & BS_DUP)) atomicOr(&own[h], BS_DUP);
                return h;
            }
            h = (h + 1) & mask;
        }
        atomicOr(status, 1u);
        return h;
    };

    constexpr int PF = 12;
    if constexpr (FAST) {
        uint64_t v[PF];
        uint32_t hs[PF];
#pragma unroll
        for (int i = 0; i < PF; ++i) {
            const size_t j = (size_t)i * BS_RANK_THREADS + tid;
            v[i] = j < N ? col[j] : 0;
        }
        for (uint32_t h = tid; h < Tl; h += BS_RANK_THREADS) own[h] = BS_EMPTY;
        __syncthreads();
        RK_STAMP(1);
        uint32_t candidate = 0;
#pragma unroll
        for (int i = 0; i < PF; ++i) {
            const size_t j = (size_t)i * BS_RANK_THREADS + tid;
            hs[i] = 0;
            if (j < N) {
                const uint64_t prod = v[i] * 0x9E3779B97F4A7C15ull;
                const uint32_t mine = slot_word(prod, (uint32_t)j);
                uint32_t h = (uint32_t)(prod >> (64 - logT)) & mask, probes = 0;
                for (; probes < Tl; ++probes) {
                    const uint32_t cur = atomicCAS(&own[h], BS_EMPTY, mine);
                    if (cur == BS_EMPTY) break;
                    if (!((cur ^ mine) & tagfield)) { candidate |= 1u << i; break; }
                    h = (h + 1) & mask;
                }
                if (probes == Tl) atomicOr(status, 1u);
                hs[i] = h;
            }
        }
        constexpr int CB = 2;
        uint32_t redo = 0;
#ifdef D2G_RANK_TRACE
        __syncthreads();
        RK_STAMP(2);
#endif
#pragma unroll
        for (int c = 0; c < PF; c += CB) {
            uint32_t o[CB];
            uint64_t w[CB];
#pragma unroll
            for (int g = 0; g < CB; ++g)
                if (candidate >> (c + g) & 1) o[g] = own[hs[c + g]];
#pragma unroll
            for (int g = 0; g < CB; ++g)
                if (candidate >> (c + g) & 1) w[g] = col[o[g] & idxmask];
#pragma unroll
            for (int g = 0; g < CB; ++g)
                if (candidate >> (c + g) & 1) {
                    if (w[g] == v[c + g]) {
                        if (!(o[g] & BS_DUP)) atomicOr(&own[hs[c + g]], BS_DUP);
                    } else redo |= 1u << (c + g);
                }
            __builtin_amdgcn_sched_barrier(0);
        }
        const uint32_t skip = redo;
        while (redo) {
            const int i = __ffs(redo) - 1;
            redo &= redo - 1;
            const uint32_t j = (uint32_t)i * BS_RANK_THREADS + tid;
            const uint64_t vv = col[j];
            const uint32_t h2 = insert(vv, j, bs_hash(vv, logT) & mask);
            const uint32_t k = atomicAdd(&nfix, 1u);
            if (k < BS_MAXFIX) { fix_j[k] = j; fix_h[k] = h2; }
            else atomicOr(status, 1u);
        }
        __syncthreads();
        RK_STAMP(3);
        compact();
        RK_STAMP(4);
#pragma unroll
        for (int i = 0; i < PF; ++i) {
            const size_t j = (size_t)i * BS_RANK_THREADS + tid;
            if (j < N && !(skip >> i & 1)) ids[j] = (IdT)own[hs[i]];
        }
#ifdef D2G_RANK_TRACE
        __syncthreads();
        RK_STAMP(5);
#endif
        for (uint32_t k = tid; k < nfix && k < BS_MAXFIX; k += BS_RANK_THREADS) ids[fix_j[k]] = (IdT)own[fix_h[k]];
        if (tid == 0) { colcnt[t * BS_CC_STRIDE] = running - 1; colcnt[t * BS_CC_STRIDE + 5] = running - 1; }
        return;
    }

    const bool tagged = MULTI && nsplit > 1;
    for (uint32_t part = part_lo; part < part_hi; ++part) {
        const uint32_t ptag = BS_PENDING | (tagged ? part << 15 : 0u);
        for (uint32_t h = tid; h < Tl; h += BS_RANK_THREADS) own[h] = BS_EMPTY;
        __syncthreads();
        constexpr int PG = 8;
        const bool mine_known = N <= (size_t)8 * PG * BS_RANK_THREADS;
        unsigned long long mine_all = 0;
        int batch = 0;
        for (size_t j0 = 0; j0 < N; j0 += (size_t)PG * BS_RANK_THREADS) {
            uint64_t v[PG];
            uint32_t hs[PG];
#pragma unroll
            for (int i = 0; i < PG; ++i) {
                const size_t j = j0 + (size_t)i * BS_RANK_THREADS + tid;
                v[i] = j < N ? col[j] : 0;
            }
            uint32_t mineb = 0, candidate = 0, redo = 0;
#pragma unroll
            for (int i = 0; i < PG; ++i) {
                const size_t j = j0 + (size_t)i * BS_RANK_THREADS + tid;
                const uint64_t prod = v[i] * 0x9E3779B97F4A7C15ull;
                const uint32_t hh = (uint32_t)(prod >> (64 - logT));
                hs[i] = 0;
                if (j < N && (!MULTI || (hh >> logTl) == part)) {
                    mineb |= 1u << i;
                    const uint32_t mine = slot_word(prod, (uint32_t)j);
                    uint32_t h = hh & mask, probes = 0;
                    for (; probes < Tl; ++probes) {
                        const uint32_t cur = atomicCAS(&own[h], BS_EMPTY, mine);
                        if (cur == BS_EMPTY) break;
                        if (!((cur ^ mine) & tagfield)) { candidate |= 1u << i; break; }
                        h = (h + 1) & mask;
                    }
                    if (probes == Tl) atomicOr(status, 1u);
                    hs[i] = h;
                }
            }
            {
                uint32_t o[PG];
                uint64_t w[PG];
#pragma unroll
                for (int i = 0; i < PG; ++i)
                    if (candidate >> i & 1) o[i] = own[hs[i]];
#pragma unroll
                for (int i = 0; i < PG; ++i)
                    if (candidate >> i & 1) w[i] = col[o[i] & idxmask];
#pragma unroll
                for (int i = 0; i < PG; ++i)
                    if (candidate >> i & 1) {
                        if (w[i] == v[i]) { if (!(o[i] & BS_DUP)) atomicOr(&own[hs[i]], BS_DUP); }
                        else redo |= 1u << i;
                    }
            }
#pragma unroll
            for (int i = 0; i < PG; ++i) {
                const size_t j = j0 + (size_t)i * BS_RANK_THREADS + tid;
                if ((mineb & ~redo) >> i & 1) ids[j] = (IdT)(hs[i] | (MULTI ? ptag : 0u));
                else if (MULTI && !tagged && part == 0 && j < N && !(redo >> i & 1)) ids[j] = 0;
            }
            while (redo) {
                const int i = __ffs(redo) - 1;
                redo &= redo - 1;
                const size_t j = j0 + (size_t)i * BS_RANK_THREADS + tid;
                const uint64_t vv = col[j];
                ids[j] = (IdT)(insert(vv, (uint32_t)j, bs_hash(vv, logT) & mask) | (MULTI ? ptag : 0u));
            }
            if (batch < 8) mine_all |= (unsigned long long)mineb << (8 * batch);
            ++batch;
        }
        __syncthreads();
        RK_STAMP(1 + 2 * (part - part_lo));
        compact();
        batch = 0;
        for (size_t j0 = 0; j0 < N; j0 += (size_t)PG * BS_RANK_THREADS, ++batch) {
            uint32_t sl[PG];
            const uint32_t mb = mine_known ? (uint32_t)(mine_all >> (8 * batch)) & 0xFFu : 0xFFu;
#pragma unroll
            for (int i = 0; i < PG; ++i) {
                const size_t j = j0 + (size_t)i * BS_RANK_THREADS + tid;
                sl[i] = (j < N && (mb >> i & 1)) ? ids[j] : 0;
            }
#pragma unroll
            for (int i = 0; i < PG; ++i) {
                const size_t j = j0 + (size_t)i * BS_RANK_THREADS + tid;
                if (j < N && (mb >> i & 1) && (mine_known || !MULTI || (tagged ? (sl[i] & ~0x7FFFu) == ptag : (sl[i] & BS_PENDING) != 0)))
                    ids[j] = (IdT)own[sl[i] & (tagged ? 0x7FFFu : ~BS_PENDING)];
            }
        }
        __syncthreads();
        RK_STAMP(2 + 2 * (part - part_lo));
    }
    if (tid == 0) { colcnt[t * BS_CC_STRIDE + split] = running - 1; if (nsplit == 1) colcnt[t * BS_CC_STRIDE + 5] = running - 1; }
}

__device__ __forceinline__ int live_planes(const uint32_t *meta, int tb) {
    const uint32_t md = meta[tb];
    return md <= 1 ? 1 : 32 - __clz(md);
}

__device__ __forceinline__ size_t stream_slot(const uint32_t *meta, int tb) {
    size_t q = 0;
    for (int t = 0; t < tb; ++t) q += (size_t)live_planes(meta, t);
    return q;
}

__device__ __forceinline__ size_t stream_slot_wave(const uint32_t *meta, int tb) {
    const int lane = threadIdx.x & 63;
    uint32_t q = 0;
    for (int t0 = 0; t0 < tb; t0 += 64) {
        const int t = t0 + lane;
        uint32_t v = t < tb ? (uint32_t)live_planes(meta, t) : 0u;
        for (int o = 32; o > 0; o >>= 1) v += __shfl_xor(v, o);
        q += v;
    }
    return (size_t)__builtin_amdgcn_readfirstlane(q);
}

__device__ __forceinline__ void sp_ride_piece(const SpRider &r, size_t piece) {
    typedef uint32_t u32x4 __attribute__((ext_vector_type(4)));
    const uint32_t v = r.vsrc ? r.vsrc[0] : r.vimm;
    const size_t head = min(r.cnt, (size_t)((16 - ((uintptr_t)r.out & 15)) & 15) / 4);
    u32x4 *body = reinterpret_cast<u32x4 *>(r.out + head);
    const size_t nb = (r.cnt - head) / 4;
    const size_t end = min((piece + 1) * (size_t)2048, nb);
    for (size_t i = piece * 2048 + threadIdx.x; i < end; i += blockDim.x) __builtin_nontemporal_store(u32x4{v, v, v, v}, &body[i]);
    if (piece == 0) {
        if (threadIdx.x < head) r.out[threadIdx.x] = v;
        const size_t tail0 = head + nb * 4;
        if (tail0 + threadIdx.x < r.cnt) r.out[tail0 + threadIdx.x] = v;
    }
}
__device__ __forceinline__ void sp_ride(const SpRider &r) { sp_ride_piece(r, (size_t)r.piece0 + (blockIdx.x - r.own)); }
#define SP_RIDE_OR_WORK(r) do { if (blockIdx.x >= (r).own) { sp_ride(r); return; } } while (0)
__global__ __launch_bounds__(256) void sp_side_fill_kernel(SpRider r, uint32_t pieces) {
    for (size_t p = blockIdx.x; p < pieces; p += gridDim.x) sp_ride_piece(r, p);
}
constexpr uint32_t SP_SIDE_FILL_PIECES = 32768;
inline unsigned sp_side_fill_grid(const d2g_ctx *ctx, uint32_t pieces, size_t words, size_t N, size_t S) {
    const double need = (double)words * 4.0 / (1.3 * 21.0 * (double)N * ((double)S / 1024.0));
    const unsigned cus = (unsigned)ctx->num_cus;
    const unsigned g = need <= 3700.0 ? cus / 2 : need <= 4400.0 ? cus * 3 / 4 : need <= 5000.0 ? cus * 3 / 2 : pieces;
    return std::max(1u, std::min<unsigned>(pieces, g));
}

constexpr int BS_PLAN_THREADS = 1024;
constexpr int BS_PLAN_MAXS = 4096;
constexpr uint32_t BS_NOCOL = 0xFFFFFFFFu;
__device__ __forceinline__ int plane_class(uint32_t d2) { return d2 == 0 ? 1 : 32 - __clz(d2 + 1); }

struct BsPlanArgs {
    uint32_t *colcnt; uint32_t S; int ntb, nsplit; uint32_t *perm, *meta; const uint32_t *status; uint32_t *ex_meta, *ex_status; int sort;
};
struct BsPlanLds { uint32_t *d2s, *cell, *wave_tot; uint16_t *perm_s; };
__host__ __device__ inline uint32_t bs_plan_sorted(uint32_t Spad, int sort) { return sort && Spad <= (uint32_t)BS_PLAN_MAXS; }
__host__ __device__ inline size_t bs_plan_lds_words(uint32_t Spad, int sort) {
    return bs_plan_sorted(Spad, sort) ? (size_t)Spad + 32 * (size_t)((Spad + 63) / 64) + 16 + (Spad + 1) / 2 : 0;
}
__device__ __forceinline__ BsPlanLds bs_plan_lds(uint32_t *base, uint32_t Spad) {
    const uint32_t ncell = 32 * ((Spad + 63) / 64);
    return BsPlanLds{base, base + Spad, base + Spad + ncell, reinterpret_cast<uint16_t *>(base + Spad + ncell + 16)};
}
template <int T>
__device__ __forceinline__ void bs_colplan_body(const BsPlanArgs &pa, const BsPlanLds &l) {
    static_assert(T % 64 == 0 && T <= 1024 && BS_PLAN_MAXS % T == 0 && (32 * (BS_PLAN_MAXS / 64)) % T == 0, "bs_colplan_body: block size");
    uint32_t *const colcnt = pa.colcnt, *const perm = pa.perm, *const meta = pa.meta, *const ex_meta = pa.ex_meta;
    const uint32_t S = pa.S;
    const int ntb = pa.ntb, nsplit = pa.nsplit;
    uint32_t *const d2s = l.d2s, *const cell = l.cell, *const wave_tot = l.wave_tot;
    uint16_t *const perm_s = l.perm_s;
    const int tid = threadIdx.x, lane = tid & 63, wave = tid >> 6;
    const uint32_t Spad = (uint32_t)ntb * 32u;
    auto column_total = [&](uint32_t t) {
        uint32_t run = 0;
        for (int h = 0; h < nsplit; ++h) { const uint32_t c = colcnt[(size_t)t * BS_CC_STRIDE + h]; colcnt[(size_t)t * BS_CC_STRIDE + h] = run; run += c; }
        colcnt[(size_t)t * BS_CC_STRIDE + 4] = run;
        return run;
    };
    if (tid == 0 && pa.ex_status) *pa.ex_status = *pa.status;
    if (!bs_plan_sorted(Spad, pa.sort)) {
        for (uint32_t t = tid; t < S; t += T) (void)column_total(t);
        for (uint32_t p = tid; p < Spad; p += T) perm[p] = p < S ? p : BS_NOCOL;
        __threadfence();
        __syncthreads();
        for (int g = tid; g < ntb; g += T) {
            uint32_t mx = 0;
            for (uint32_t x = 0; x < 32; ++x) { const uint32_t t = (uint32_t)g * 32 + x; if (t < S) mx = max(mx, colcnt[(size_t)t * BS_CC_STRIDE + 4]); }
            meta[g] = mx + 1;
            if (ex_meta) ex_meta[g] = mx + 1;
        }
        return;
    }
    const uint32_t nchunk = (Spad + 63) / 64, ncell = 32 * nchunk;
    for (uint32_t c = tid; c < ncell; c += T) cell[c] = 0;
    __syncthreads();
    constexpr int IT = BS_PLAN_MAXS / T;
    uint32_t mine[IT];
#pragma unroll
    for (int it = 0; it < IT; ++it) {
        const uint32_t t = (uint32_t)it * T + tid;
        mine[it] = 0;
        if (t - lane < Spad) {
            uint32_t d2 = 0;
            int cls = 0;
            if (t < S) { d2 = column_total(t); cls = plane_class(d2); }
            if (t < Spad) d2s[t] = d2;
            unsigned long long todo = __ballot(t < Spad);
            while (todo) {
                const int k = __shfl(cls, __ffsll((long long)todo) - 1);
                const unsigned long long m = __ballot(cls == k && t < Spad);
                const uint32_t ci = (uint32_t)(31 - k) * nchunk + t / 64;
                if (cls == k && t < Spad) mine[it] = ci << 6 | (uint32_t)__popcll(m & ((1ull << lane) - 1));
                if (lane == 0) cell[(uint32_t)(31 - k) * nchunk + (t - lane) / 64] = __popcll(m);
                todo &= ~m;
            }
        }
    }
    __syncthreads();
    {
        constexpr int CPT = 32 * (BS_PLAN_MAXS / 64) / T;
        const uint32_t c0 = (uint32_t)CPT * tid;
        uint32_t v[CPT], sum = 0;
#pragma unroll
        for (int x = 0; x < CPT; ++x) { v[x] = c0 + x < ncell ? cell[c0 + x] : 0u; sum += v[x]; }
        uint32_t incl = sum;
        for (int o = 1; o < 64; o <<= 1) { const uint32_t x = __shfl_up(incl, o); if (lane >= o) incl += x; }
        if (lane == 63) wave_tot[wave] = incl;
        __syncthreads();
        uint32_t ex = incl - sum;
        for (int w = 0; w < wave; ++w) ex += wave_tot[w];
#pragma unroll
        for (int x = 0; x < CPT; ++x) { if (c0 + x < ncell) cell[c0 + x] = ex; ex += v[x]; }
    }
    __syncthreads();
#pragma unroll
    for (int it = 0; it < IT; ++it) {
        const uint32_t t = (uint32_t)it * T + tid;
        if (t < Spad) perm_s[cell[mine[it] >> 6] + (mine[it] & 63u)] = (uint16_t)t;
    }
    __syncthreads();
    for (uint32_t p = tid; p < Spad; p += T) { const uint32_t t = perm_s[p]; perm[p] = t < S ? t : BS_NOCOL; }
    for (int g = tid; g < ntb; g += T) {
        uint32_t mx = 0;
        for (uint32_t x = 0; x < 32; ++x) mx = max(mx, d2s[perm_s[(uint32_t)g * 32 + x]]);
        meta[g] = mx + 1;
        if (ex_meta) ex_meta[g] = mx + 1;
    }
}

__global__ __launch_bounds__(BS_PLAN_THREADS) void bs_colplan_kernel(BsPlanArgs pa, SpRider rider) {
    SP_RIDE_OR_WORK(rider);
    extern __shared__ __attribute__((aligned(16))) uint32_t plan_lds[];
    bs_colplan_body<BS_PLAN_THREADS>(pa, bs_plan_lds(plan_lds, (uint32_t)pa.ntb * 32u));
}

constexpr int BS_FORM_STREAM = 1, BS_FORM_EXCHANGE = 2;
constexpr size_t BS_SLACK = 64;
struct BsPlanesArgs {
    const void *ids; size_t N, Npad; uint32_t *planes, *stream; size_t Nstride; int nbits_cap; const uint32_t *meta; int forms;
    const uint32_t *perm, *colcnt, *sperm;
};
BsPlanesArgs planes_args_of(const d2g_cmp_set *set, uint32_t *planes, int forms) {
    return BsPlanesArgs{set->d_ids.get(), set->N, set->Npad, planes, set->d_stream, set->Nstride, set->nbits_cap, set->d_meta, forms, set->d_perm, set->d_colcnt, nullptr};
}
template <bool SPLIT, typename IdT = uint32_t>
__device__ __forceinline__ void bs_planes_body(const BsPlanesArgs &a, size_t bx, size_t tb) {
    static_assert(!SPLIT || sizeof(IdT) == 4, "bs_planes_body: split ranks are 32-bit ids");
    constexpr int UBIT = BsId<IdT>::UBIT;
    const IdT *__restrict__ ids = static_cast<const IdT *>(a.ids);
    const uint32_t *__restrict__ meta = a.meta, *__restrict__ perm = a.perm, *__restrict__ colcnt = a.colcnt, *__restrict__ sperm = a.sperm;
    uint32_t *__restrict__ planes = a.planes, *__restrict__ stream = a.stream;
    const size_t N = a.N, Npad = a.Npad, Nstride = a.Nstride;
    const int nbits_cap = a.nbits_cap, forms = a.forms;
    const size_t jpos = bx * 256 + threadIdx.x;
    const size_t slot = (forms & BS_FORM_STREAM) ? stream_slot_wave(meta, (int)tb) : 0;
    if (jpos >= Nstride) return;
    const size_t j = sperm ? (size_t)sperm[jpos] : jpos;
    const int nbits = live_planes(meta, (int)tb);
    typedef const u32x16_u __attribute__((address_space(4))) *slots_ptr;
    const u32x16_u pa = *(slots_ptr)(uintptr_t)(perm + tb * 32), pb = *(slots_ptr)(uintptr_t)(perm + tb * 32 + 16);
    uint32_t id[32];
#pragma unroll
    for (int x = 0; x < 32; ++x) {
        const uint32_t t = x < 16 ? pa[x] : pb[x - 16];
// ... 144 lines not shown
    uint32_t acc[IW][JR];
#pragma unroll
    for (int i = 0; i < IW; ++i)
#pragma unroll
        for (int c = 0; c < JR; ++c) acc[i][c] = 0;

    const uint32_t *ptr = stream + iw0;
    const uint32_t coff = (uint32_t)(Nstride - iw0 + j0 + (size_t)lane) * 4u;
    const size_t step = 2 * Nstride;

    BsOperands<JR> nx = bs_fetch<JR>(ptr, coff, step);
    int nbits_nx = live_planes(meta, 0);
    for (int tb = 0; tb < ntb; ++tb) {
        const int nbits = nbits_nx;
        nbits_nx = live_planes(meta, tb + 1 < ntb ? tb + 1 : 0);
        bs_group<JR>(nbits, ptr, coff, step, nx, acc);
    }

    const bool interior = iw0 + IW <= sh.i_hi && j0 >= sh.j_lo && j0 + 64 * JR <= sh.j_hi &&
                          (sh.ut ? j0 > iw0 + IW - 1 : (j0 > iw0 + IW - 1 || j0 + 64 * JR <= iw0));
    if (interior) {
        uint32_t val[IW][JR];
#pragma unroll
        for (int i = 0; i < IW; ++i)
#pragma unroll
            for (int c = 0; c < JR; ++c) val[i][c] = store.value_from_mismatches(S, acc[i][c]);
        const uint32_t jl = (uint32_t)j0 + (uint32_t)lane;
#pragma unroll
        for (int i = 0; i < IW; ++i) {
            const size_t rb = out_row_base(sh, iw0 + i);
#pragma unroll
            for (int c = 0; c < JR; ++c) store.put_row(rb, jl + 64u * c, val[i][c]);
        }
        return;
    }
    uint32_t val[IW][JR];
#pragma unroll
    for (int i = 0; i < IW; ++i)
#pragma unroll
        for (int c = 0; c < JR; ++c)
            val[i][c] = store.value((iw0 + i) == (j0 + lane + 64 * c) ? S : S - acc[i][c]);
#pragma unroll
    for (int i = 0; i < IW; ++i) {
        const size_t ii = iw0 + i;
        if (ii >= sh.i_hi) break;
#pragma unroll
        for (int c = 0; c < JR; ++c) {
            const size_t jj = j0 + lane + 64 * c;
            if (jj < sh.j_hi && jj >= sh.j_lo && (!sh.ut || jj > ii)) store.put(out_pos(sh, ii, jj), val[i][c]);
        }
    }
}

#include "d2g_k2_sparse.h"

int refresh_borrowed(d2g_ctx *ctx, const d2g_cmp_set *set, hipStream_t s) {
    if (!set->borrowed || set->managed) return D2G_OK;
    return d2g_bitslice_derive_groups(ctx, set, 0, set->ntb, s);
}


template <class Store>
int launch_bitslice(d2g_ctx *ctx, const d2g_cmp_set *set, PairShape sh, Store store, hipStream_t s) {
    if (int rc = finish_shape(ctx, sh, BS_JR == 2 ? 32u : 64u)) return rc;
    if (sh.nvalid_total == 0) return D2G_OK;
    if (int rc = refresh_borrowed(ctx, set, s)) return rc;
    if (int rc = d2g_bitslice_ensure_natural(ctx, set, s)) return rc;
    d2g_timer tm(ctx, &ctx->ev_k2, s);
    hipLaunchKernelGGL((k2_bitslice_kernel<BS_JR, Store>), dim3(sh.per_xcd * 8), dim3(BS_THREADS), 0, s, set->d_stream,
                       set->Nstride, set->d_meta, set->ntb, (uint32_t)set->S, sh, store, (const uint32_t *)nullptr, 0u, SpPatchArgs{});
    tm.stop();
    D2G_HIP(ctx, hipGetLastError());
    return D2G_OK;
}

}

void d2g_bitslice_geometry(d2g_cmp_set *set) {
    set->nbits_cap = 1;
    while ((1ull << set->nbits_cap) < set->N / 2 + 2) ++set->nbits_cap;
    set->ntb = (int)div_up<size_t>(set->S, 32);
    set->Nstride = set->Npad + BS_SLACK;
}

int d2g_bitslice_alloc_stream(d2g_ctx *ctx, d2g_cmp_set *set) {
    return set->d_stream.alloc(ctx, ((size_t)set->ntb * set->nbits_cap + 1) * 2 * set->Nstride, "bitslice alloc");
}

namespace {
int alloc_prepare_workspace(d2g_ctx *ctx, d2g_cmp_set *set) {
    const size_t N = set->N, S = set->S, Npad = set->Npad;
    if (N >= (1ull << 30)) { ctx->last_error = "bitslice: N too large"; return D2G_ERR_UNSUPPORTED; }
    d2g_bitslice_geometry(set);
    set->T = 64; set->logT = 6;
    while ((uint64_t)set->T * 2 < (uint64_t)N * 3) { set->T <<= 1; ++set->logT; }
    set->nsplit = 1;
    if (set->logT > BS_LOG_TLDS_MAX && N < (1ull << BS_SPLIT_SHIFT)) {
        const uint32_t nparts = set->T >> BS_LOG_TLDS_MAX;
        int want = 1;
        while (want < 4 && (uint32_t)want * 2 <= nparts && S * (size_t)want < (size_t)std::max(ctx->num_cus, 1)) want *= 2;
        if (ctx->k2.nsplit_req && (uint32_t)ctx->k2.nsplit_req <= nparts) want = ctx->k2.nsplit_req;
        set->nsplit = want;
    }
    const char *what = "bitslice alloc";
    int rc;
    set->id_bits = (ctx->k2.id16 && set->logT <= BS_LOG_TLDS_MAX) ? 16 : 32;
    D2G_CHECK(ctx, set->id_bits == 32 || (N <= BS_ID16_MAX_N && set->nsplit == 1), "bitslice: 16-bit ids need a single-partition rank kernel");
    const size_t id_words = set->id_bits == 16 ? (S * Npad + 1) / 2 : S * Npad;
    if ((rc = set->d_ids.alloc(ctx, id_words, what)) ||
        (rc = d2g_hip_status(ctx, hipMemset(set->d_ids, 0, id_words * sizeof(uint32_t)), what)) ||
        (rc = set->d_colcnt.alloc(ctx, S * BS_CC_STRIDE, what)) ||
        (rc = set->d_perm.alloc(ctx, (size_t)set->ntb * 32, what)) ||
        (rc = set->own_meta.alloc(ctx, (size_t)(set->ntb + 4), what)) ||
        (rc = d2g_hip_status(ctx, hipMemset(set->own_meta, 0, (size_t)(set->ntb + 4) * sizeof(uint32_t)), what))) return rc;
    set->d_meta = set->own_meta;
    return D2G_OK;
}
int launch_planes(d2g_ctx *ctx, const d2g_cmp_set *set, uint32_t *planes, int forms, hipStream_t s) {
    const dim3 grid((unsigned)div_up<size_t>(set->Nstride, 256), (unsigned)set->ntb);
    const bool split = set->logT > BS_LOG_TLDS_MAX && set->nsplit > 1;
    D2G_CHECK(ctx, !(split && set->id_bits == 16), "bitslice: a split set with 16-bit ids");
    hipLaunchKernelGGL((set->id_bits == 16 ? bs_planes_kernel<false, uint16_t> : split ? bs_planes_kernel<true> : bs_planes_kernel<false>), grid, dim3(256), 0, s, planes_args_of(set, planes, forms));
    D2G_HIP(ctx, hipGetLastError());
    return D2G_OK;
}
struct JoinOnExit {
    hipStream_t s; hipEvent_t ev = nullptr;
    ~JoinOnExit() { if (ev) (void)hipStreamWaitEvent(s, ev, 0); }
};
}

int d2g_bitslice_alloc(d2g_ctx *ctx, d2g_cmp_set *set) {
    if (int rc = alloc_prepare_workspace(ctx, set)) return rc;
    if (int rc = set->own_planes.alloc(ctx, (size_t)set->ntb * (set->nbits_cap + 1) * set->Nstride, "bitslice alloc")) return rc;
    set->d_planes = set->own_planes;
    if (int rc = d2g_bitslice_alloc_stream(ctx, set)) return rc;
    set->ncols = set->S;
    if (sparse_enabled(ctx, set->N) && set->S < 65536 && sp_alloc(ctx, set) != D2G_OK) (void)hipGetLastError();
    if (set->sparse_ok() && set->nsplit == 1) {
        set->sp->owner_stride = set->N / 2 + 8;
        if (set->sp->d_owner.alloc(ctx, set->S * set->sp->owner_stride, "bitslice owner alloc") != D2G_OK) (void)hipGetLastError();
    }
    return D2G_OK;
}

int d2g_bitslice_prepare(d2g_ctx *ctx, d2g_cmp_set *set, hipStream_t s) {
    const size_t N = set->N, S = set->S, Npad = set->Npad;
    SpState *const sp = set->sp.get();
    const bool sparse_path = sp && !set->export_only && !set->want_exchange;
    JoinOnExit join{s};
    if (sp) {
        sp->dec.skip_cached = sparse_path ? (sp_will_skip(ctx, *sp) ? 1 : 0) : -1;
        sp->announced.begin(ctx->k2.ride, sparse_path && sp->dec.skip_cached != 1);
    }
    if (sp && sp->announced.riding() >= SP_SIDE_FILL_PIECES) {
        if (!sp->fill_stream) {
            if (sp->fill_stream.create(hipStreamNonBlocking) != hipSuccess || sp->fill_fork.create(hipEventDisableTiming) != hipSuccess ||
                sp->fill_join.create(hipEventDisableTiming) != hipSuccess) { (void)hipGetLastError(); sp->fill_stream.reset(); sp->fill_fork.reset(); sp->fill_join.reset(); }
        }
        if (sp->fill_stream) {
            hipStream_t fs = sp->fill_stream;
            D2G_HIP(ctx, hipEventRecord(sp->fill_fork, s));
            D2G_HIP(ctx, hipStreamWaitEvent(fs, sp->fill_fork, 0));
            join.ev = sp->fill_join;
            const uint32_t pieces = sp->announced.riding();
            const SpRider all = sp->announced.take_all();
            const unsigned fgrid = sp_side_fill_grid(ctx, pieces, all.cnt, N, S);
            hipLaunchKernelGGL(sp_side_fill_kernel, dim3(fgrid), dim3(256), 0, fs, all, pieces);
            D2G_HIP(ctx, hipEventRecord(sp->fill_join, fs));
        }
    }
    const bool multi = set->logT > BS_LOG_TLDS_MAX;
    const int nsplit = multi ? set->nsplit : 1;
    {
        const int logTl = set->logT < BS_LOG_TLDS_MAX ? set->logT : BS_LOG_TLDS_MAX;
        const size_t lds = (size_t(1) << logTl) * sizeof(uint32_t);
        const bool id16 = set->id_bits == 16;
        D2G_CHECK(ctx, !(multi && id16), "bitslice: the multi-partition rank kernel with 16-bit ids");
        void (*kern)(const uint64_t *, size_t, size_t, uint32_t, int, void *, uint32_t *, uint32_t *, int, uint32_t, int, uint32_t *, size_t) = bs_rank_kernel<false, false>;
        if (multi) kern = bs_rank_kernel<true, false>;
        else if (N <= (size_t)12 * BS_RANK_THREADS) kern = id16 ? bs_rank_kernel<false, true, uint16_t> : bs_rank_kernel<false, true>;
        else if (id16) kern = bs_rank_kernel<false, false, uint16_t>;
        if (lds > 48 * 1024)
            D2G_HIP(ctx, hipFuncSetAttribute((const void *)kern, hipFuncAttributeMaxDynamicSharedMemorySize, (int)lds));
        if (nsplit > 1) D2G_HIP(ctx, hipMemsetAsync(set->d_ids, 0, S * Npad * sizeof(uint32_t), s));
        hipLaunchKernelGGL(kern, dim3((unsigned)(S * nsplit)), dim3(BS_RANK_THREADS), lds, s, set->d_cols, N, Npad, set->T, set->logT,
                           (void *)set->d_ids.get(), set->d_colcnt, set->d_meta + set->ntb, ctx->k2.tagbits_max, (uint32_t)S, nsplit,
                           (sp && nsplit == 1) ? sp->d_owner.get() : (uint32_t *)nullptr, sp ? sp->owner_stride : 0);
        if (sp) sp->dec.kernels = 2 + (join.ev ? 1 : 0);
        const bool look = sparse_path && sp_sample_due(ctx, set);
        if (look) { if (int rc = sp_sample_enqueue(ctx, set, s)) return rc; if (sp->dec.sample_pending) sp->dec.kernels += 2; }
        const bool merged = sparse_path && !look && ctx->k2.merge && nsplit == 1 && sp->d_owner && ctx->k2.olink && ctx->k2.link && sp->dec.skip_cached != 1;
        if (sp) sp->dec.merged = merged;
        if (!merged) {
            unsigned g = 1; const SpRider rd = sp ? sp->announced.take(1, SP_RW_PLAN, false, 1, &g) : SP_NO_RIDER;
            const BsPlanArgs pa{set->d_colcnt, (uint32_t)S, set->ntb, nsplit, set->d_perm, set->d_meta, set->d_meta + set->ntb, set->ex_meta, set->ex_status, ctx->k2.sort ? 1 : 0};
            hipLaunchKernelGGL(bs_colplan_kernel, dim3(g), dim3(BS_PLAN_THREADS), bs_plan_lds_words((uint32_t)set->ntb * 32u, pa.sort) * 4, s, pa, rd);
            if (sp) sp->dec.kernels += 1;
        }
    }
    if (sparse_path) {
        if (!sp->dec.merged) { if (int rc = launch_planes(ctx, set, set->d_planes, BS_FORM_STREAM, s)) return rc; sp->dec.kernels += 1; }
        if (int rc = sp_sample_collect(ctx, set, s)) return rc;
        if (int rc = sp_prepare_order(ctx, set, nsplit > 1, s)) return rc;
        if (int rc = sp_permute(ctx, set, s)) return rc;
        set->srt_valid = true; set->nat_valid = true;
        if (sp->announced.riding()) sp->filled.set_by_riders(sp->announced);
        else sp->filled.void_after_prepare();
        sp->announced.served();
        D2G_HIP(ctx, hipGetLastError());
        return D2G_OK;
    }
    if (sp) sp->announced.served();
    const int forms = set->export_only ? BS_FORM_EXCHANGE : (BS_FORM_STREAM | (set->want_exchange ? BS_FORM_EXCHANGE : 0));
    if (int rc = launch_planes(ctx, set, set->export_only ? set->ex_planes : set->d_planes, forms, s)) return rc;
    if (sp) sp->dec.kernels += 1;
    set->srt_valid = false; set->nat_valid = true;
    return D2G_OK;
}

SpInit d2g_bitslice_sp_init(const d2g_cmp_set *set) { return sp_init_of(set); }

int d2g_bitslice_ensure_natural(d2g_ctx *ctx, const d2g_cmp_set *set, hipStream_t s) {
    if (set->nat_valid || set->borrowed || set->export_only) return D2G_OK;
    if (int rc = launch_planes(ctx, set, set->d_planes, BS_FORM_STREAM, s)) return rc;
    set->nat_valid = true;
    return D2G_OK;
}

int d2g_bitslice_export(d2g_ctx *ctx, d2g_cmp_set *set, hipStream_t s) {
    if (set->borrowed || set->want_exchange || set->export_only) return D2G_OK;
    set->want_exchange = true;
    return launch_planes(ctx, set, set->d_planes, BS_FORM_EXCHANGE, s);
}

int d2g_bitslice_exporter_create(d2g_ctx *ctx, size_t N, size_t S_local, d2g_cmp_set **out) {
    *out = nullptr;
    d2g_cmp_set *set = new (std::nothrow) d2g_cmp_set();
    if (!set) return D2G_ERR_NOMEM;
    set->ctx = ctx; set->N = N; set->S = S_local;
    set->Npad = div_up<size_t>(N, BS_CB) * BS_CB;
    set->algo = D2G_CMP_BITSLICE;
    set->export_only = true;
    if (int rc = set->d_cols.alloc(ctx, set->Npad * S_local, "bitslice exporter alloc")) { delete set; return rc; }
    if (int rc = alloc_prepare_workspace(ctx, set)) { delete set; return rc; }
    *out = set;
    return D2G_OK;
}
void d2g_bitslice_set_export_target(d2g_cmp_set *set, uint32_t *planes, uint32_t *meta, uint32_t *status) {
    set->ex_planes = planes; set->ex_meta = meta; set->ex_status = status;
}

int d2g_bitslice_derive_groups(d2g_ctx *ctx, const d2g_cmp_set *set, int g0, int g1, hipStream_t s) {
    if (g1 <= g0) return D2G_OK;
    dim3 grid((unsigned)div_up<size_t>(set->Nstride, 256), (unsigned)(g1 - g0));
    hipLaunchKernelGGL(bs_derive_kernel, grid, dim3(256), 0, s, set->d_planes, set->d_stream, set->Nstride, set->nbits_cap, set->d_meta, g0);
    D2G_HIP(ctx, hipGetLastError());
    return D2G_OK;
}

int d2g_bitslice_status(d2g_ctx *ctx, const d2g_cmp_set *set, hipStream_t s) {
    uint32_t st = 0;
    if (set->borrowed) {
        if (!set->status_words || set->n_status <= 0) { D2G_HIP(ctx, hipStreamSynchronize(s)); return D2G_OK; }
        std::vector<uint32_t> w((size_t)set->n_status);
        D2G_HIP(ctx, hipMemcpyAsync(w.data(), set->status_words, w.size() * sizeof(uint32_t), hipMemcpyDeviceToHost, s));
        D2G_HIP(ctx, hipStreamSynchronize(s));
        for (uint32_t x : w) st |= x;
    } else {
        D2G_HIP(ctx, hipMemcpyAsync(&st, set->d_meta + set->ntb, sizeof(st), hipMemcpyDeviceToHost, s));
        D2G_HIP(ctx, hipStreamSynchronize(s));
    }
    if (st & 1u) {
        ctx->last_error = "bitslice prepare: a register column put more distinct values into one hash partition than its LDS table holds "
                          "(adversarial / extremely skewed column); use D2G_CMP_DIRECT for this matrix";
        return D2G_ERR_INTERNAL;
    }
    return D2G_OK;
}

int d2g_bitslice_ut(d2g_ctx *ctx, const d2g_cmp_set *set, size_t r0, size_t r1, uint32_t *eq_out, const float *lut,
                    float *fout, hipStream_t s) {
    const PairShape sh = ut_shape(set->N, r0, r1);
    if (set->srt_valid) {
        if (eq_out) return launch_sparse(ctx, set, sh, StoreEq{eq_out}, eq_out, s);
        return launch_sparse(ctx, set, sh, StoreLut{fout, lut}, reinterpret_cast<uint32_t *>(fout), s);
    }
    if (set->sp) set->sp->filled.clear();
    if (eq_out) return launch_bitslice(ctx, set, sh, StoreEq{eq_out}, s);
    return launch_bitslice(ctx, set, sh, StoreLut{fout, lut}, s);
}

int d2g_bitslice_prefill(d2g_ctx *ctx, d2g_cmp_set *set, size_t r0, size_t r1, uint32_t *eq_out, const float *lut, float *fout, hipStream_t s) {
    if (eq_out) return sp_prefill(ctx, set, r0, r1, StoreEq{eq_out}, eq_out, s);
    return sp_prefill(ctx, set, r0, r1, StoreLut{fout, lut}, reinterpret_cast<uint32_t *>(fout), s);
}

int d2g_bitslice_announce(d2g_ctx *, d2g_cmp_set *set, size_t r0, size_t r1, uint32_t *eq_out, const float *lut, float *fout) {
    const size_t cnt = d2g_ut_count(set->N, r0, r1);
    if (!set->sp) return D2G_OK;
    SpAnnounced &an = set->sp->announced;
    an.cancel();
    if (!cnt || (!eq_out && !fout)) return D2G_OK;
    if (eq_out) an.announce(eq_out, cnt, nullptr);
    else an.announce(reinterpret_cast<uint32_t *>(fout), cnt, reinterpret_cast<const uint32_t *>(lut));
    return D2G_OK;
}

int d2g_bitslice_rect(d2g_ctx *ctx, const d2g_cmp_set *set, size_t a0, size_t a1, size_t b0, size_t b1, uint32_t *eq_out,
                      hipStream_t s) {
    return launch_bitslice(ctx, set, rect_shape(set->N, a0, a1, b0, b1), StoreEq{eq_out}, s);
}

int d2g_bitslice_managed_sparse_alloc(d2g_ctx *ctx, d2g_cmp_set *set) {
    if (!set->borrowed || set->sparse_ok()) return D2G_OK;
    set->ncols = (size_t)set->ntb * 32;
    if (!(sparse_enabled(ctx, set->N) && set->S < 65536)) return D2G_OK;
    const char *what = "bitslice sparse alloc";
    if (set->d_ids.alloc(ctx, set->ncols * set->Npad, what) != D2G_OK ||
        set->d_colcnt.alloc(ctx, set->ncols * BS_CC_STRIDE, what) != D2G_OK ||
        hipMemset(set->d_colcnt, 0, set->ncols * BS_CC_STRIDE * sizeof(uint32_t)) != hipSuccess) {
        set->d_ids.reset(); set->d_colcnt.reset();
        (void)hipGetLastError();
        return D2G_OK;
    }
    if (sp_alloc(ctx, set) != D2G_OK) (void)hipGetLastError();
    return D2G_OK;
}

int d2g_bitslice_managed_ready(d2g_ctx *ctx, d2g_cmp_set *set, hipStream_t s) {
    if (!set->borrowed || !set->sparse_ok()) return D2G_OK;
    dim3 grid((unsigned)div_up<size_t>(set->Npad, 256), (unsigned)set->ntb);
    set->sp->dec.merged = false; set->sp->dec.kernels = 1;
    hipLaunchKernelGGL(sp_unpack_kernel, grid, dim3(256), 0, s, set->d_planes, set->Nstride, set->nbits_cap, set->d_meta, set->N, set->Npad, set->d_ids, set->d_colcnt, sp_init_of(set));
    if (int rc = sp_prepare_order(ctx, set, false, s)) return rc;
    if (int rc = sp_permute(ctx, set, s)) return rc;
    D2G_HIP(ctx, hipGetLastError());
    set->srt_valid = true;
    return D2G_OK;
}

void d2g_bitslice_forget(d2g_cmp_set *set) {
    if (!set->sp) return;
    if (set->sp->h_gaveup) { set->sp->h_gaveup[SP_MW_GAVEUP] = 0; set->sp->h_gaveup[SP_MW_LIST_LEN] = 0; }
    set->sp->dec.prepares = 0; set->sp->dec.pred_valid = false;
}

int d2g_bitslice_sparse_info(d2g_ctx *ctx, const d2g_cmp_set *set, hipStream_t s, uint32_t *out4) {
    out4[0] = out4[1] = out4[2] = out4[3] = 0;
    if (!set->srt_valid || !set->sp) { D2G_HIP(ctx, hipStreamSynchronize(s)); return D2G_OK; }
    const SpState &sp = *set->sp;
    uint32_t c[4] = {0, 0, 0, 0}, ord[4] = {0, 0, 0, 0}, pl = 0;
    if (!sp.last_ctl) { D2G_HIP(ctx, hipStreamSynchronize(s)); out4[0] = 1; return D2G_OK; }
    D2G_HIP(ctx, hipMemcpyAsync(c, sp.last_ctl, sizeof c, hipMemcpyDeviceToHost, s));
    D2G_HIP(ctx, hipMemcpyAsync(ord, sp.d_order, sizeof ord, hipMemcpyDeviceToHost, s));
    D2G_HIP(ctx, hipMemcpyAsync(&pl, sp.d_plctl, sizeof pl, hipMemcpyDeviceToHost, s));
    D2G_HIP(ctx, hipStreamSynchronize(s));
    const bool dense = (c[1] & 1u) || (size_t)c[0] * 5 > (size_t)c[3] * 2;
    out4[0] = 1; out4[1] = c[0]; out4[2] = (ord[0] ? 1u : 0u) | (dense ? 2u : 4u) | (ord[0] ? 8u : 0u) | (sp.dec.skipped ? 16u : 0u);
    out4[3] = ord[0] ? 0u : (uint32_t)std::min<size_t>(pl, sp.plist_cap);
    return D2G_OK;
}

int d2g_bitslice_sparse_detail(d2g_ctx *ctx, const d2g_cmp_set *set, hipStream_t s, uint64_t *out8) {
    uint32_t binned = 0;
    if (set->sp) D2G_HIP(ctx, hipMemcpyAsync(&binned, set->sp->d_plctl + SP_PL_BINNED, 4, hipMemcpyDeviceToHost, s));
    D2G_HIP(ctx, hipStreamSynchronize(s));
    if (!set->sp) return D2G_OK;
    const SpState &sp = *set->sp;
    out8[0] = sp.dec.looked ? 1 : 0; out8[1] = sp.dec.looked_dense ? 1 : 0;
    if (sp.dec.looked) for (int x = 0; x < 4; ++x) out8[2 + x] = sp.dec.samp_sums[x];
    out8[6] = binned ? 1 : 0; out8[7] = sp.bin_cshift;
    out8[8] = sp.dec.merged ? 1 : 0; out8[9] = sp.dec.kernels;
    return D2G_OK;
}

int d2g_sparse_bin_geometry(size_t N, uint32_t *cshift, uint32_t *nch, uint32_t *nbins, int *binned_ok) {
    if (!N) return D2G_ERR_INVALID;
    const SpBinGeom g = sp_bin_geometry(N);
    if (cshift) *cshift = g.cshift;
    if (nch) *nch = g.nch;
    if (nbins) *nbins = g.nbins;
    if (binned_ok) *binned_ok = g.ok ? 1 : 0;
    return D2G_OK;
}

int d2g_bitslice_debug_read(d2g_ctx *ctx, const d2g_cmp_set *set, hipStream_t s, uint64_t *pairs_out, size_t cap, size_t *npairs, uint32_t *root_out ) {
    *npairs = 0;
    if (!set->srt_valid || !set->sp) { D2G_HIP(ctx, hipStreamSynchronize(s)); return D2G_OK; }
    const SpState &sp = *set->sp;
    uint32_t n = 0;
    D2G_HIP(ctx, hipMemcpyAsync(&n, sp.d_plctl, 4, hipMemcpyDeviceToHost, s));
    D2G_HIP(ctx, hipStreamSynchronize(s));
    const size_t m = std::min<size_t>(std::min<size_t>(n, sp.plist_cap), cap);
    if (m && pairs_out) D2G_HIP(ctx, hipMemcpy(pairs_out, sp.d_plist, m * 8, hipMemcpyDeviceToHost));
    if (root_out) D2G_HIP(ctx, hipMemcpy(root_out, sp.d_label + set->Npad, set->N * 4, hipMemcpyDeviceToHost));
    *npairs = m;
    return D2G_OK;
}

uint64_t d2g_k2_tuning_hash(const d2g_ctx *ctx) {
    const d2g_k2_tuning &t = ctx->k2;
    const long long v[] = {t.sparse, (long long)t.min_n, t.link, (long long)(t.tile_frac * 1e6), t.olink, t.emit_big, t.ride, t.remember, (long long)t.list_div, (long long)t.long_list,
                           t.list_form, t.predict, t.sort ? 1 : 0, t.tagbits_max, t.nsplit_req, t.merge};
    uint64_t h = 1469598103934665603ull;
    for (long long x : v) for (int b = 0; b < 8; ++b) { h ^= (uint64_t)(x >> (8 * b)) & 0xFF; h *= 1099511628211ull; }
    return h;
}

std::string d2g_k2_tuning_json(const d2g_ctx *ctx) {
    const d2g_k2_tuning &t = ctx->k2;
    char b[640];
    std::snprintf(b, sizeof b, "{\"D2G_BS_SPARSE\": %d, \"D2G_BS_SPARSE_MIN_N\": %zu, \"D2G_BS_SORT\": %d, \"D2G_SP_LINK\": %d, \"D2G_SP_OLINK\": %d, \"D2G_SP_TILE_FRAC\": %.3f, "
                  "\"D2G_SP_LIST_DIV\": %zu, \"D2G_SP_LONG_LIST\": %zu, \"D2G_SP_LIST_FORM\": %d, \"D2G_SP_PREDICT\": %d, \"D2G_SP_REMEMBER\": %d, \"D2G_SP_RIDE\": %d, \"D2G_SP_EMIT_BIG\": %d, \"D2G_K2_MERGE\": %d, \"D2G_BS_ID16\": %d}",
                  t.sparse ? 1 : 0, t.min_n, t.sort ? 1 : 0, t.link, t.olink, t.tile_frac, t.list_div, t.long_list, t.list_form, t.predict, t.remember, t.ride, t.emit_big, t.merge, t.id16);
    return b;
}

void d2g_warm_k2_bitslice() { hipFuncAttributes a; (void)hipFuncGetAttributes(&a, reinterpret_cast<const void *>(&bs_colplan_kernel)); }

#ifdef D2G_RANK_TRACE
extern "C" int d2g_debug_rank_trace(unsigned long long *out, size_t n) {
    return hipMemcpyFromSymbol(out, HIP_SYMBOL(g_rank_trace), std::min<size_t>(n, 8192 * 16) * 8) == hipSuccess ? 0 : -1;
}
#endif
#ifdef D2G_SP_TRACE
extern "C" int d2g_debug_emit_trace(unsigned long long *out, size_t n) {
    return hipMemcpyFromSymbol(out, HIP_SYMBOL(g_emit_trace), std::min<size_t>(n, 4096 * 16) * 8) == hipSuccess ? 0 : -1;
}
extern "C" int d2g_debug_sp_trace(unsigned long long *out, size_t n) {
    return hipMemcpyFromSymbol(out, HIP_SYMBOL(g_sp_trace), std::min<size_t>(n, 16384 * 8) * 8) == hipSuccess ? 0 : -1;
}
#endif
```

### dashing2_amd/csrc/d2g_runtime.hip

```cpp
#include "d2g_internal.h"
#include <algorithm>
#include <cstdlib>
#include <cstring>
#include <new>

static const char *const kTuningNames[] = {
    "D2G_BS_SORT", "D2G_BS_NSPLIT", "D2G_BS_TAGBITS", "D2G_BS_ID16", "D2G_K2_MERGE",
    "D2G_BS_SPARSE", "D2G_BS_SPARSE_MIN_N", "D2G_SP_LINK", "D2G_SP_TILE_FRAC", "D2G_SP_LIST_DIV", "D2G_SP_LONG_LIST", "D2G_SP_LIST_FORM", "D2G_SP_PREDICT", "D2G_SP_REMEMBER", "D2G_SP_EMIT_BIG", "D2G_SP_OLINK", "D2G_SP_RIDE",
    "D2G_MGPU_CHUNKS",
    "D2G_K3_COMPACT", "D2G_K3_L1BITS", "D2G_K3_BUCKET_KEYS", "D2G_K3_SUB_KEYS", "D2G_K3_SPLIT_MIN", "D2G_K3_SUBBATCH", "D2G_K3_ROUND_KEYS",
    "D2G_K3_GUESS_SCALE", "D2G_K3_GRID_PER_CU", "D2G_K3_LIGHT", "D2G_K3_GQ_SCALE",
    "D2G_K3S_RANGE_KEYS", "D2G_KSET_SPLIT", "D2G_KSET_PBITS",
    "D2G_CS_TABLE_BYTES", "D2G_CS_LDS_CELLS",
};
void d2g_tuning_load(d2g_tuning &t) {
    t.kv.clear();
    for (const char *n : kTuningNames)
        if (const char *v = std::getenv(n)) t.kv.emplace_back(n, v);
}

d2g_k2_tuning d2g_k2_tuning_resolve(const d2g_tuning &t) {
    d2g_k2_tuning v;
    if (const char *e = t.get("D2G_BS_SPARSE")) v.sparse = !(e[0] == '0');
    if (const char *e = t.get("D2G_BS_SPARSE_MIN_N")) v.min_n = (size_t)std::atoll(e);
    if (const char *e = t.get("D2G_SP_LINK")) v.link = std::atoi(e) != 0;
    if (const char *e = t.get("D2G_SP_TILE_FRAC")) { const double f = std::atof(e); if (f > 0 && f <= 1) v.tile_frac = f; }
    if (const char *e = t.get("D2G_SP_OLINK")) v.olink = std::atoi(e) != 0;
    if (const char *e = t.get("D2G_K2_MERGE")) v.merge = std::atoi(e) != 0;
    if (const char *e = t.get("D2G_SP_EMIT_BIG")) v.emit_big = std::atoi(e) != 0;
    if (const char *e = t.get("D2G_SP_REMEMBER")) v.remember = std::atoi(e) != 0;
    if (const char *e = t.get("D2G_SP_RIDE")) v.ride = std::atoi(e) & 63;
    if (const char *e = t.get("D2G_SP_LONG_LIST")) { const long long d = std::atoll(e); if (d >= 0) v.long_list = (size_t)d; }
    if (const char *e = t.get("D2G_SP_PREDICT")) v.predict = std::atoi(e) != 0;
    if (const char *e = t.get("D2G_SP_LIST_FORM")) { const int d = std::atoi(e); if (d >= 0 && d <= 2) v.list_form = d; }
    if (const char *e = t.get("D2G_SP_LIST_DIV")) { const long d = std::atol(e); if (d >= 1 && d <= (1 << 20)) v.list_div = (size_t)d; }
    if (const char *e = t.get("D2G_BS_SORT")) v.sort = !(e[0] == '0');
    if (const char *e = t.get("D2G_BS_TAGBITS")) { const int d = std::atoi(e); if (d >= 0 && d < 31) v.tagbits_max = d; }
    if (const char *e = t.get("D2G_BS_ID16")) v.id16 = std::atoi(e) != 0;
    if (const char *e = t.get("D2G_BS_NSPLIT")) { const int d = std::atoi(e); if (d == 1 || d == 2 || d == 4) v.nsplit_req = d; }
    return v;
}

d2g_k3_tuning d2g_k3_tuning_resolve(const d2g_tuning &t) {
    d2g_k3_tuning v;
    if (const char *e = t.get("D2G_K3_COMPACT")) v.compact = e[0] == '1';
    if (const char *e = t.get("D2G_K3_LIGHT")) v.light = !(e[0] == '0');
    if (const char *e = t.get("D2G_K3_L1BITS")) { const int d = std::atoi(e); if (d >= 0 && d <= K3_MAXBBITS) v.l1bits = (uint32_t)d; }
    if (const char *e = t.get("D2G_K3_BUCKET_KEYS")) { const long d = std::atol(e); if (d >= 1) v.bucket_keys = (uint64_t)d; }
    if (const char *e = t.get("D2G_K3_SUB_KEYS")) { const long d = std::atol(e); if (d >= 1) v.sub_keys = (uint64_t)d; }
    if (const char *e = t.get("D2G_K3_SPLIT_MIN")) { const long d = std::atol(e); if (d >= 1) v.split_min = (uint64_t)d; }
    if (const char *e = t.get("D2G_K3_SUBBATCH")) { const int d = std::atoi(e); if (d >= 1 && d <= 8) v.subbatch = (size_t)d; }
    if (const char *e = t.get("D2G_K3_ROUND_KEYS")) { const int d = std::atoi(e); if (d >= 1 && d <= K3_ROUND_KEYS) v.round_keys = (uint32_t)d; }
    if (const char *e = t.get("D2G_K3_GUESS_SCALE")) { const double d = std::atof(e); if (d > 0.) v.guess_scale = d; }
    if (const char *e = t.get("D2G_K3_GRID_PER_CU")) { const int d = std::atoi(e); if (d >= 1 && d <= 256) v.grid_per_cu = (size_t)d; }
    if (const char *e = t.get("D2G_K3_GQ_SCALE")) { v.gq_scale_set = true; v.gq_scale = std::max(0.0, std::atof(e)); }
    v.gq_slack = v.gq_scale_set ? 1 : v.grid_per_cu > 24 ? 256 : 1024;
    if (const char *e = t.get("D2G_K3S_RANGE_KEYS")) { const long d = std::atol(e); if (d >= 1 && d <= K3_TARGET) v.sort_keys = (uint64_t)d; }
    if (const char *e = t.get("D2G_CS_TABLE_BYTES")) { const long long d = std::atoll(e); if (d >= 1) v.cs_table_bytes = (uint64_t)d; }
    if (const char *e = t.get("D2G_CS_LDS_CELLS")) { const int d = std::atoi(e); if (d >= 0 && d <= 40960) v.cs_lds_cells = d; }
    return v;
}

void d2g_tuning_resolve(d2g_ctx *c) {
    d2g_tuning_load(c->tune);
    c->k2 = d2g_k2_tuning_resolve(c->tune);
    c->k3_tune = d2g_k3_tuning_resolve(c->tune);
    c->kset = d2g_kset_tuning();
    if (const char *e = c->tune.get("D2G_KSET_SPLIT")) { const int v = std::atoi(e); if (v >= 1 && v <= 65535) c->kset.split = v; }
    if (const char *e = c->tune.get("D2G_KSET_PBITS")) { const int v = std::atoi(e); if (v >= 0 && v <= 20) c->kset.pbits = v; }
    c->mgpu_chunks = 0;
    if (const char *e = c->tune.get("D2G_MGPU_CHUNKS")) { const int v = std::atoi(e); if (v >= 1 && v <= MG_MAX_CHUNKS) c->mgpu_chunks = v; }
}

extern "C" {

int d2g_ctx_reload_tuning(d2g_ctx *c) {
    if (!c) return D2G_ERR_INVALID;
    d2g_tuning_resolve(c);
    return D2G_OK;
}

int d2g_ctx_tuning(const d2g_ctx *c, char *buf, size_t cap) {
    if (!c) return D2G_ERR_INVALID;
    std::string j = "{";
    for (size_t i = 0; i < c->tune.kv.size(); ++i) {
        if (i) j += ", ";
        j += "\"" + c->tune.kv[i].first + "\": \"";
        for (char ch : c->tune.kv[i].second) { if (ch == '"' || ch == '\\') j += '\\'; if ((unsigned char)ch >= 0x20) j += ch; }
        j += "\"";
    }
    j += std::string(c->tune.kv.empty() ? "" : ", ") + "\"resolved\": " + d2g_k2_tuning_json(c);
    j += "}";
    if (buf && cap) { std::snprintf(buf, cap, "%s", j.c_str()); }
    return (int)j.size();
}

int d2g_device_count(void) {
    int n = 0;
    if (hipGetDeviceCount(&n) != hipSuccess) return 0;
    return n;
}

int d2g_ctx_create(int device, d2g_ctx **out) {
    if (!out) return D2G_ERR_INVALID;
    *out = nullptr;
    int n = 0;
    if (hipGetDeviceCount(&n) != hipSuccess || n <= 0) return D2G_ERR_NODEVICE;
    if (device < 0 || device >= n) return D2G_ERR_INVALID;
    if (hipSetDevice(device) != hipSuccess) return D2G_ERR_NODEVICE;
    hipDeviceProp_t prop;
    if (hipGetDeviceProperties(&prop, device) != hipSuccess) return D2G_ERR_NODEVICE;
    if (std::strncmp(prop.gcnArchName, "gfx950", 6) != 0) return D2G_ERR_NODEVICE;
    d2g_ctx *c = new (std::nothrow) d2g_ctx();
    if (!c) return D2G_ERR_NOMEM;
    c->device = device;
    c->num_cus = prop.multiProcessorCount;
    d2g_tuning_resolve(c);
    *out = c;
    return D2G_OK;
}

void d2g_ctx_destroy(d2g_ctx *c) {
    if (!c) return;
    (void)hipSetDevice(c->device);
    if (c->k3) d2g_k3_state_destroy(c->k3);
    delete c;
}

const char *d2g_last_error(const d2g_ctx *c) { return c ? c->last_error.c_str() : "null ctx"; }
int d2g_ctx_device(const d2g_ctx *c) { return c ? c->device : -1; }

int d2g_sync(d2g_ctx *c, void *stream) {
    if (!c) return D2G_ERR_INVALID;
    D2G_HIP(c, hipSetDevice(c->device));
    D2G_HIP(c, hipStreamSynchronize(as_stream(stream)));
    return D2G_OK;
}

int d2g_malloc(d2g_ctx *c, size_t nbytes, void **dptr) {
    if (!c || !dptr) return D2G_ERR_INVALID;
    D2G_HIP(c, hipSetDevice(c->device));
    D2G_HIP(c, hipMalloc(dptr, nbytes ? nbytes : 1));
    return D2G_OK;
}
int d2g_free(d2g_ctx *c, void *dptr) {
    if (!c) return D2G_ERR_INVALID;
    if (!dptr) return D2G_OK;
    D2G_HIP(c, hipSetDevice(c->device));
    D2G_HIP(c, hipFree(dptr));
    return D2G_OK;
}
int d2g_mem_info(d2g_ctx *c, size_t *free_bytes, size_t *total_bytes) {
    if (!c) return D2G_ERR_INVALID;
    D2G_HIP(c, hipSetDevice(c->device));
    size_t f = 0, t = 0;
    D2G_HIP(c, hipMemGetInfo(&f, &t));
    if (free_bytes) *free_bytes = f;
    if (total_bytes) *total_bytes = t;
    return D2G_OK;
}
int d2g_malloc_host(d2g_ctx *c, size_t nbytes, void **hptr) {
    if (!c || !hptr) return D2G_ERR_INVALID;
    D2G_HIP(c, hipSetDevice(c->device));
    D2G_HIP(c, hipHostMalloc(hptr, nbytes ? nbytes : 1, hipHostMallocDefault));
    return D2G_OK;
}
int d2g_host_register(d2g_ctx *c, void *hptr, size_t nbytes) {
    if (!c || !hptr || !nbytes) return D2G_ERR_INVALID;
    D2G_HIP(c, hipSetDevice(c->device));
    D2G_HIP(c, hipHostRegister(hptr, nbytes, hipHostRegisterDefault));
    return D2G_OK;
}
int d2g_host_unregister(d2g_ctx *c, void *hptr) {
    if (!c || !hptr) return D2G_ERR_INVALID;
    D2G_HIP(c, hipHostUnregister(hptr));
    return D2G_OK;
}
int d2g_free_host(d2g_ctx *c, void *hptr) {
    if (!c) return D2G_ERR_INVALID;
    if (!hptr) return D2G_OK;
    D2G_HIP(c, hipHostFree(hptr));
    return D2G_OK;
}
int d2g_memcpy_h2d(d2g_ctx *c, void *dst, const void *src, size_t n, void *stream) {
// ... 92 lines not shown
```

### include/d2g.h

```cpp
#ifndef D2G_H
#define D2G_H
#include <stddef.h>
#include <stdint.h>

#ifdef __cplusplus
extern "C" {
#endif

#define D2G_VERSION_MAJOR 0
#define D2G_VERSION_MINOR 1

typedef struct d2g_ctx d2g_ctx;

enum d2g_status {
    D2G_OK = 0,
    D2G_ERR_INVALID = -1,
    D2G_ERR_NODEVICE = -2,
    D2G_ERR_HIP = -3,
    D2G_ERR_NOMEM = -4,
    D2G_ERR_UNSUPPORTED = -5,
    D2G_ERR_IO = -6,
    D2G_ERR_INTERNAL = -7
};

// ... 142 lines not shown
                          const uint64_t *run_start, const uint32_t *run_len, size_t nrun,
                          const uint64_t *genome_run_off, size_t n,
                          int k, int canon, uint64_t xormask, size_t sketchsize,
                          uint64_t *regs_out , uint32_t *counts_out );

typedef struct d2g_sketcher d2g_sketcher;
int  d2g_sketcher_create(d2g_ctx *ctx, d2g_sketcher **out);
void d2g_sketcher_destroy(d2g_sketcher *sk);
int  d2g_sketcher_set_window(d2g_sketcher *sk, int w);
int  d2g_sketcher_set_alphabet(d2g_sketcher *sk, int alphabet);
int  d2g_sketcher_run(d2g_sketcher *sk, const uint8_t *packed, size_t packed_bytes,
                      const uint64_t *run_start, const uint32_t *run_len, size_t nrun,
                      const uint64_t *genome_run_off, size_t n, int k, int canon, uint64_t xormask,
                      size_t sketchsize, uint64_t *regs_out );

int  d2g_sketcher_run_counts(d2g_sketcher *sk, const uint8_t *packed, size_t packed_bytes,
                             const uint64_t *run_start, const uint32_t *run_len, size_t nrun,
                             const uint64_t *genome_run_off, size_t n, int k, int canon, uint64_t xormask,
                             size_t sketchsize, uint64_t *regs_out , uint32_t *counts_out );

int d2g_oph_sketch_mincount(d2g_ctx *ctx, const uint8_t *packed, size_t packed_bytes,
                            const uint64_t *run_start, const uint32_t *run_len, size_t nrun,
                            const uint64_t *genome_run_off, size_t n,
                            int k, int canon, uint64_t xormask, size_t sketchsize, uint32_t mincount,
                            uint64_t *regs_out , uint32_t *counts_out );
int d2g_oph_sketch_mincount_dev(d2g_ctx *ctx, const d2g_oph_plan *plan, const uint8_t *packed_dev,
                                int canon, uint64_t xormask, size_t sketchsize, uint32_t mincount,
                                uint64_t *regs_out_dev , void *stream);
int d2g_sketcher_run_mincount(d2g_sketcher *sk, const uint8_t *packed, size_t packed_bytes,
                              const uint64_t *run_start, const uint32_t *run_len, size_t nrun,
                              const uint64_t *genome_run_off, size_t n, int k, int canon, uint64_t xormask,
                              size_t sketchsize, uint32_t mincount,
                              uint64_t *regs_out , uint32_t *counts_out );

typedef struct d2g_kmer_filter d2g_kmer_filter;
int  d2g_kmer_filter_create_dev(d2g_ctx *ctx, const d2g_oph_plan *plan, const uint8_t *packed_dev, int canon, void *stream,
                                d2g_kmer_filter **out);
int  d2g_kmer_filter_create(d2g_ctx *ctx, const uint8_t *packed, size_t packed_bytes, const uint64_t *run_start, const uint32_t *run_len,
                            size_t nrun, int k, int canon, d2g_kmer_filter **out);
int  d2g_kmer_filter_create_windowed(d2g_ctx *ctx, const uint8_t *packed, size_t packed_bytes, const uint64_t *run_start,
                                     const uint32_t *run_len, size_t nrun, int k, int canon, int w, d2g_kmer_filter **out);
int  d2g_kmer_filter_create_alphabet(d2g_ctx *ctx, const uint8_t *packed, size_t packed_bytes, const uint64_t *run_start,
                                     const uint32_t *run_len, size_t nrun, int k, int alphabet, d2g_kmer_filter **out);
void d2g_kmer_filter_destroy(d2g_kmer_filter *filter);
int  d2g_kmer_filter_info(d2g_ctx *ctx, const d2g_kmer_filter *filter, uint64_t *noccurrences, uint64_t *ndistinct, size_t *table_bytes);
int  d2g_kmer_filter_contains(d2g_ctx *ctx, const d2g_kmer_filter *filter, const uint64_t *kmers, size_t n, uint8_t *out);
int  d2g_oph_plan_set_filter(d2g_oph_plan *plan, const d2g_kmer_filter *filter);
int  d2g_sketcher_set_filter(d2g_sketcher *sk, const d2g_kmer_filter *filter);

#define D2G_SCREEN_MAX_KEYS (1ull << 30)
typedef struct d2g_screen d2g_screen;
int  d2g_screen_table_slots(uint64_t ndistinct, uint64_t *slots);
int  d2g_screen_create(d2g_ctx *ctx, const uint64_t *keys , size_t nrefs, size_t sketchsize, int k, int canon,
                       uint64_t xormask, size_t nrows, d2g_screen **out);
void d2g_screen_destroy(d2g_screen *screen);
int  d2g_screen_reset(d2g_ctx *ctx, d2g_screen *screen);
int  d2g_screen_info(d2g_ctx *ctx, const d2g_screen *screen, uint64_t *ndistinct, size_t *table_bytes, size_t *counter_bytes);
int  d2g_screen_fed(d2g_ctx *ctx, const d2g_screen *screen, size_t row, uint64_t *nkmers);
int  d2g_screen_set_fed(d2g_ctx *ctx, d2g_screen *screen, size_t row, uint64_t nkmers);
int  d2g_screen_add_dev(d2g_ctx *ctx, d2g_screen *screen, const d2g_oph_plan *plan, const uint8_t *packed_dev,
                        const uint32_t *genome_row , void *stream);
int  d2g_sketcher_run_screen(d2g_sketcher *sk, const uint8_t *packed, size_t packed_bytes,
                             const uint64_t *run_start, const uint32_t *run_len, size_t nrun,
                             const uint64_t *genome_run_off, size_t n, int k, int canon,
                             d2g_screen *screen, const uint32_t *genome_row );
int  d2g_screen_result(d2g_ctx *ctx, const d2g_screen *screen, size_t row0, size_t nrows,
                       uint32_t *matches_out , uint32_t *matchsums_out );
int  d2g_screen_key_counts(d2g_ctx *ctx, const d2g_screen *screen, size_t row, uint64_t *keys_out ,
                           uint32_t *counts_out );
int  d2g_epilogue_contain(const uint32_t *matches, const uint32_t *matchsums, size_t n, size_t sketchsize,
                          float *coverage_out , float *depth_out );

int d2g_sketcher_ingest_fasta(d2g_sketcher *sk, const uint8_t *raw, size_t raw_bytes, const uint64_t *file_off,
                              const uint64_t *file_len, size_t nfiles, const uint64_t *genome_file_off , size_t n, int k);
int d2g_sketcher_ingested_runs(const d2g_sketcher *sk, const uint64_t **run_start, const uint32_t **run_len, size_t *nrun,
                               const uint64_t **genome_run_off , const uint64_t **genome_nkmers ,
                               uint64_t *nbases );

int d2g_bmh_sketch(d2g_ctx *ctx, const uint8_t *packed, size_t packed_bytes,
                   const uint64_t *run_start, const uint32_t *run_len, size_t nrun,
                   const uint64_t *genome_run_off, size_t n,
                   int k, int canon, uint64_t xormask, size_t sketchsize, double count_threshold,
                   double *sig_out , double *total_weight_out );
int d2g_bmh_sketch_dev(d2g_ctx *ctx, const d2g_oph_plan *plan, const uint8_t *packed_dev,
                       int canon, uint64_t xormask, size_t sketchsize, double count_threshold,
                       double *sig_out_dev , double *total_weight_out_dev , void *stream);
int d2g_sketcher_run_bmh(d2g_sketcher *sk, const uint8_t *packed, size_t packed_bytes,
                         const uint64_t *run_start, const uint32_t *run_len, size_t nrun,
                         const uint64_t *genome_run_off, size_t n, int k, int canon, uint64_t xormask,
                         size_t sketchsize, double count_threshold,
                         double *sig_out , double *total_weight_out );
int d2g_kmer_count(d2g_ctx *ctx, const uint8_t *packed, size_t packed_bytes,
                   const uint64_t *run_start, const uint32_t *run_len, size_t nrun,
                   const uint64_t *genome_run_off, size_t n, int k, int canon, uint64_t xormask,
                   double count_threshold, uint64_t *keys_out, uint32_t *counts_out, size_t cap,
                   uint64_t *genome_off_out );
int d2g_kmer_distinct(d2g_ctx *ctx, const uint8_t *packed, size_t packed_bytes,
                      const uint64_t *run_start, const uint32_t *run_len, size_t nrun,
                      const uint64_t *genome_run_off, size_t n, int k, int canon, uint64_t xormask,
                      uint64_t *ndistinct_out );
int d2g_sketcher_run_distinct(d2g_sketcher *sk, const uint8_t *packed, size_t packed_bytes,
                              const uint64_t *run_start, const uint32_t *run_len, size_t nrun,
                              const uint64_t *genome_run_off, size_t n, int k, int canon, uint64_t xormask,
                              uint64_t *ndistinct_out );
int d2g_bmh_check_weights(const double *weights , const uint64_t *set_off , size_t nsets,
                          size_t sketchsize, double scale, char *err, size_t errcap);
int d2g_bmh_from_weighted(d2g_ctx *ctx, const uint64_t *ids, const double *weights,
                          const uint64_t *set_off , size_t nsets, size_t sketchsize,
                          double *sig_out , double *total_weight_out );
int d2g_bmh_from_weighted_ids(d2g_ctx *ctx, const uint64_t *ids, const double *weights,
                              const uint64_t *set_off , size_t nsets, size_t sketchsize,
                              double *sig_out , double *total_weight_out ,
                              uint64_t *owner_out );

int d2g_bmh_sketch_cs(d2g_ctx *ctx, const uint8_t *packed, size_t packed_bytes,
                      const uint64_t *run_start, const uint32_t *run_len, size_t nrun,
                      const uint64_t *genome_run_off, size_t n,
                      int k, int canon, uint64_t xormask, size_t sketchsize, uint64_t cells, double count_threshold,
                      double *sig_out , double *total_weight_out );
int d2g_bmh_sketch_cs_dev(d2g_ctx *ctx, const d2g_oph_plan *plan, const uint8_t *packed_dev,
                          int canon, uint64_t xormask, size_t sketchsize, uint64_t cells, double count_threshold,
                          double *sig_out_dev , double *total_weight_out_dev , void *stream);
int d2g_sketcher_run_bmh_cs(d2g_sketcher *sk, const uint8_t *packed, size_t packed_bytes,
                            const uint64_t *run_start, const uint32_t *run_len, size_t nrun,
                            const uint64_t *genome_run_off, size_t n, int k, int canon, uint64_t xormask,
                            size_t sketchsize, uint64_t cells, double count_threshold,
                            double *sig_out , double *total_weight_out );
int d2g_countsketch_table(d2g_ctx *ctx, const uint8_t *packed, size_t packed_bytes,
                          const uint64_t *run_start, const uint32_t *run_len, size_t nrun,
                          const uint64_t *genome_run_off, size_t n, int k, int canon, uint64_t xormask,
                          uint64_t cells, int32_t *table_out );
int d2g_countsketch_cells(d2g_ctx *ctx, const uint8_t *packed, size_t packed_bytes,
                          const uint64_t *run_start, const uint32_t *run_len, size_t nrun,
                          const uint64_t *genome_run_off, size_t n, int k, int canon, uint64_t xormask,
                          uint64_t cells, double count_threshold, uint64_t *ids_out, double *w_out, size_t cap,
                          uint64_t *set_off_out , uint64_t *total_out );
int d2g_countsketch_lds_cells(void);
int d2g_countsketch_stats(d2g_ctx *ctx, uint64_t *table_bytes, uint64_t *groups, uint64_t *batches);

size_t d2g_ut_count(size_t N, size_t r0, size_t r1);
typedef struct d2g_cmp_set d2g_cmp_set;
int  d2g_cmp_set_create_dev(d2g_ctx *ctx, const uint64_t *sig_bits_dev, size_t N, size_t sketchsize,
                            int algo, void *stream, d2g_cmp_set **out);
int  d2g_cmp_set_create(d2g_ctx *ctx, const uint64_t *sig_bits_host, size_t N, size_t sketchsize,
                        int algo, d2g_cmp_set **out);
int  d2g_cmp_set_update_dev(d2g_ctx *ctx, d2g_cmp_set *set, const uint64_t *sig_bits_dev, void *stream);
int  d2g_cmp_set_status(d2g_ctx *ctx, const d2g_cmp_set *set, void *stream);
int  d2g_cmp_set_planes(d2g_ctx *ctx, const d2g_cmp_set *set, void *stream, unsigned *max_distinct, int *nbits,
                        float *mean_nbits);
int  d2g_cmp_set_id_bits(const d2g_cmp_set *set);
int  d2g_cmp_set_sparse_info(d2g_ctx *ctx, const d2g_cmp_set *set, void *stream, uint32_t *info4);
int  d2g_cmp_set_debug_pairs(d2g_ctx *ctx, const d2g_cmp_set *set, void *stream, uint64_t *pairs_out, size_t cap, size_t *npairs, uint32_t *root_out);
int  d2g_cmp_set_sparse_detail(d2g_ctx *ctx, const d2g_cmp_set *set, void *stream, uint64_t *out10);
int  d2g_sparse_bin_geometry(size_t N, uint32_t *cshift, uint32_t *nch, uint32_t *nbins, int *binned_ok);
int  d2g_operand_layout(size_t N, size_t sketchsize, size_t *group_words, size_t *ngroups);
int  d2g_cmp_set_export_operand_dev(d2g_ctx *ctx, const d2g_cmp_set *set, uint32_t *planes_out_dev,
                                    uint32_t *meta_out_dev, void *stream);
int  d2g_cmp_set_from_planes_dev(d2g_ctx *ctx, size_t N, size_t sketchsize, const uint32_t *planes_dev,
                                 const uint32_t *meta_dev, d2g_cmp_set **out);
int  d2g_pack_column_slices_dev(d2g_ctx *ctx, const uint64_t *rows_dev, size_t n, size_t sketchsize, int nslices,
                                uint64_t *out_dev, void *stream);
void d2g_cmp_set_destroy(d2g_cmp_set *set);
int  d2g_cmp_set_algo(const d2g_cmp_set *set);
int  d2g_cmp_eqcount_ut_dev(d2g_ctx *ctx, const d2g_cmp_set *set, size_t r0, size_t r1,
                            uint32_t *neq_out_dev, void *stream);
int  d2g_cmp_lut_ut_dev(d2g_ctx *ctx, const d2g_cmp_set *set, size_t r0, size_t r1,
                        const float *lut_dev, float *out_dev, void *stream);
int  d2g_cmp_ut_prefill_dev(d2g_ctx *ctx, d2g_cmp_set *set, size_t r0, size_t r1, uint32_t *neq_out_dev,
                            const float *lut_dev, float *out_dev, void *stream);
int  d2g_cmp_ut_announce_dev(d2g_ctx *ctx, d2g_cmp_set *set, size_t r0, size_t r1, uint32_t *neq_out_dev,
                             const float *lut_dev, float *out_dev);
int  d2g_cmp_set_forget(d2g_ctx *ctx, d2g_cmp_set *set);
int  d2g_cmp_gtlt_ut_dev(d2g_ctx *ctx, const d2g_cmp_set *set, size_t r0, size_t r1,
                         uint32_t *gt_out_dev, uint32_t *lt_out_dev, void *stream);
int  d2g_cmp_eqcount_rect_dev(d2g_ctx *ctx, const d2g_cmp_set *set, size_t a0, size_t a1,
                              size_t b0, size_t b1, uint32_t *neq_out_dev, void *stream);

int  d2g_cmp_gtlt_rect_dev(d2g_ctx *ctx, const d2g_cmp_set *set, size_t a0, size_t a1, size_t b0, size_t b1,
                           uint32_t *gt_out_dev, uint32_t *lt_out_dev, void *stream);

int  d2g_cmp_eqcount_ut(d2g_ctx *ctx, const uint64_t *sig_bits, size_t N, size_t sketchsize,
                        size_t r0, size_t r1, int algo, uint32_t *neq_out);
int  d2g_cmp_dist_ut(d2g_ctx *ctx, const uint64_t *sig_bits, const double *cards, size_t N,
                     size_t sketchsize, size_t r0, size_t r1, int measure, int k, int multiset_space,
                     int algo, int nthreads, float *out);

int  d2g_cmp_set_create_codes_dev(d2g_ctx *ctx, const void *codes_dev, size_t N, size_t sketchsize, int regbytes, void *stream,
                                  d2g_cmp_set **out);
int  d2g_cmp_set_create_codes(d2g_ctx *ctx, const void *codes_host, size_t N, size_t sketchsize, int regbytes, d2g_cmp_set **out);
size_t d2g_cmp_set_operand_bytes(const d2g_cmp_set *set);
int  d2g_cmp_dist_trunc_ut(d2g_ctx *ctx, const double *sigs, const double *cards, size_t N, size_t sketchsize, size_t r0, size_t r1,
                           int measure, int k, int regbytes, int bbit, int nthreads, float *out);

int  d2g_cmp_knn_dev(d2g_ctx *ctx, const d2g_cmp_set *set, size_t r0, size_t r1, size_t K, uint32_t min_count,
                     const uint32_t *cls_dev, size_t cap, uint32_t *rowcnt_dev , uint32_t *ids_dev ,
                     uint32_t *counts_dev , size_t band_rows, void *stream);
int  d2g_knn_finish(const uint32_t *rowcnt, const uint32_t *ids, const uint32_t *counts, size_t nrows, size_t cap, const float *lut,
                    size_t sketchsize, int isdist, uint64_t *indptr_out , uint32_t *indices_out, float *data_out,
                    size_t out_cap, size_t *nnz_needed, size_t *overflow_rows);
int  d2g_cmp_set_knn(d2g_ctx *ctx, const d2g_cmp_set *set, size_t r0, size_t r1, const float *lut, int isdist, size_t K,
                     double threshold, size_t cap, size_t band_rows, uint64_t *indptr_out , uint32_t *indices_out,
                     float *data_out, size_t out_cap, size_t *nnz_needed);
int  d2g_cmp_knn(d2g_ctx *ctx, const uint64_t *sig_bits, size_t N, size_t sketchsize, size_t r0, size_t r1, int measure, int k,
                 int multiset_space, int algo, size_t K, double threshold, size_t cap, size_t band_rows,
                 uint64_t *indptr_out , uint32_t *indices_out, float *data_out, size_t out_cap, size_t *nnz_needed);

int  d2g_cmp_dedup_dev(d2g_ctx *ctx, const d2g_cmp_set *set, uint32_t min_count, const uint32_t *cls_dev ,
                       uint32_t *assign_dev , size_t band_rows, void *stream);
int  d2g_dedup_clusters(const uint32_t *assign, size_t N, uint64_t *indptr_out, uint32_t *indices_out , size_t *nclusters);
int  d2g_cmp_set_dedup(d2g_ctx *ctx, const d2g_cmp_set *set, const float *lut, double threshold, size_t band_rows,
                       uint32_t *assign_out );
int  d2g_cmp_dedup(d2g_ctx *ctx, const uint64_t *sig_bits, size_t N, size_t sketchsize, int measure, int k, int multiset_space,
                   int algo, double threshold, size_t band_rows, uint32_t *assign_out );

typedef struct d2g_comm d2g_comm;
#define D2G_COMM_ID_BYTES 128
int  d2g_comm_unique_id(void *id_out );
int  d2g_comm_create(d2g_ctx *ctx, const void *id, int rank, int world, d2g_comm **out);
int  d2g_comm_create_all(d2g_ctx **ctxs, int nctx, d2g_comm **comms_out );
void d2g_comm_destroy(d2g_comm *comm);
int  d2g_comm_rank(const d2g_comm *comm);
int  d2g_comm_world(const d2g_comm *comm);
int  d2g_comm_is_rccl(const d2g_comm *comm);
int  d2g_bcast_sigs(d2g_ctx **ctxs, d2g_comm **comms, int nctx, const uint64_t *host_sig, size_t N, size_t sketchsize,
                    uint64_t **sig_dev_out );

typedef struct d2g_allpairs d2g_allpairs;
int  d2g_allpairs_create(d2g_ctx *ctx, d2g_comm *comm, size_t N, size_t sketchsize, d2g_allpairs **out);
void d2g_allpairs_destroy(d2g_allpairs *eng);
int  d2g_allpairs_rows_held(const d2g_allpairs *eng, size_t *lo, size_t *hi);
int  d2g_allpairs_rows_computed(const d2g_allpairs *eng, size_t *r0, size_t *r1);
int  d2g_allpairs_prepare_dev(d2g_allpairs *eng, const uint64_t *my_rows_dev , void *stream);
int  d2g_allpairs_prepare_all(d2g_allpairs **engs, int n, const uint64_t *const *rows_dev, void *const *streams);
const d2g_cmp_set *d2g_allpairs_operand(const d2g_allpairs *eng);
int  d2g_allpairs_status(d2g_allpairs *eng, void *stream);
int  d2g_allpairs_chunks(const d2g_allpairs *eng);
int  d2g_allpairs_step_lut_dev(d2g_allpairs *eng, const uint64_t *my_rows_dev, const float *lut_dev, float *out_dev, void *stream);
int  d2g_allpairs_step_eqcount_dev(d2g_allpairs *eng, const uint64_t *my_rows_dev, uint32_t *out_dev, void *stream);
int  d2g_allpairs_step_all(d2g_allpairs **engs, int n, const uint64_t *const *rows_dev, const float *const *lut_dev,
                           void *const *out_dev, void *const *streams);
#define D2G_PHASE_PACK    0
#define D2G_PHASE_X1      1
#define D2G_PHASE_PREPARE 2
#define D2G_PHASE_X2      3
#define D2G_PHASE_DERIVE  4
#define D2G_PHASE_PAIR    5
#define D2G_PHASE_ORDER   6
#define D2G_PHASE_FILL    7
int  d2g_allpairs_set_phase_timing(d2g_allpairs *eng, int on);
int  d2g_allpairs_phase_times(d2g_allpairs *eng, int cap, int *n_out, int *kind , int *chunk ,
                              float *start_ms , float *dur_ms );
int  d2g_allpairs_sparse_info(d2g_allpairs *eng, uint32_t *info4);
int  d2g_allpairs_enqueue_lut_dev(d2g_allpairs *eng, const uint64_t *my_rows_dev, const float *lut_dev, float *out_dev,
                                  void *stream, int input_ready);

int d2g_kmer_sets(d2g_ctx *ctx, const uint8_t *packed, size_t packed_bytes,
                  const uint64_t *run_start, const uint32_t *run_len, size_t nrun,
                  const uint64_t *genome_run_off, size_t n, int k, int canon, uint64_t xormask,
                  double count_threshold, uint64_t *keys_out, uint32_t *counts_out , size_t cap,
                  uint64_t *set_off_out , uint64_t *cards_out );
int d2g_sketcher_run_sets(d2g_sketcher *sk, const uint8_t *packed, size_t packed_bytes,
                          const uint64_t *run_start, const uint32_t *run_len, size_t nrun,
                          const uint64_t *genome_run_off, size_t n, int k, int canon, uint64_t xormask,
                          double count_threshold, uint64_t *keys_out, uint32_t *counts_out , size_t cap,
                          uint64_t *set_off_out , uint64_t *cards_out );
int d2g_kmer_sets_dev(d2g_ctx *ctx, const d2g_oph_plan *plan, const uint8_t *packed_dev, int canon, uint64_t xormask,
                      double count_threshold, uint64_t *keys_dev, uint32_t *counts_dev , size_t cap,
                      uint64_t *set_off_dev , uint64_t *cards_dev , void *stream);
typedef struct d2g_kset d2g_kset;
int    d2g_kset_check(const uint64_t *keys, const uint32_t *counts , const uint64_t *set_off , size_t nsets,
                      char *err, size_t errcap);
int    d2g_kset_create(d2g_ctx *ctx, const uint64_t *keys, const uint32_t *counts , const uint64_t *set_off ,
                       size_t nsets, d2g_kset **out);
int    d2g_kset_create_dev(d2g_ctx *ctx, const uint64_t *keys_dev, const uint32_t *counts_dev , const uint64_t *set_off_dev,
                           size_t nsets, void *stream, d2g_kset **out);
void   d2g_kset_destroy(d2g_kset *ks);
size_t d2g_kset_size(const d2g_kset *ks);
size_t d2g_kset_device_bytes(const d2g_kset *ks);
int    d2g_kset_slice_bits(const d2g_kset *ks);
int    d2g_kset_isz_ut_dev(d2g_ctx *ctx, const d2g_kset *ks, size_t r0, size_t r1, uint64_t *out_dev, void *stream);
int    d2g_kset_isz_rect_dev(d2g_ctx *ctx, const d2g_kset *ks, size_t a0, size_t a1, size_t b0, size_t b1, uint64_t *out_dev, void *stream);
float  d2g_epilogue_exact(uint64_t isz, double lhcard, double rhcard, int measure, int k);
int    d2g_epilogue_exact_ut(const uint64_t *isz, const double *cards, size_t N, size_t r0, size_t r1, int measure, int k, int nthreads,
                             float *out);
int    d2g_epilogue_exact_rect(const uint64_t *isz, const double *cards, size_t N, size_t a0, size_t a1, size_t b0, size_t b1,
                               int measure, int k, int nthreads, float *out);

int  d2g_ut_partition(size_t N, int nparts, size_t *bounds_out);

#ifdef __cplusplus
}
#endif
#endif
```

Before: 208.5 billion.

## Let the fast rank kernel carry a share of the announced output fill

The fast single-partition rank kernel now takes a leading share of the announced output fill (controlled by a new rank_share knob) and issues its nontemporal stores while its own column loads are in flight. The rider mask widens to 127 so the rank kernel is an eligible rider. This moves fill traffic into an otherwise latency-bound kernel instead of later kernels or a side stream. The risk is that extra store traffic and an explicit vmcnt wait slow the rank kernel itself. A fill_detail diagnostic API is also added.

```diff
diff --git a/dashing2_amd/capi.py b/dashing2_amd/capi.py
--- a/dashing2_amd/capi.py
+++ b/dashing2_amd/capi.py
@@ -188,6 +188,7 @@
     "d2g_cmp_set_sparse_info": (_int, [_vp, _vp, _vp, _vp]),
     "d2g_cmp_set_debug_pairs": (_int, [_vp, _vp, _vp, _vp, _sz, C.POINTER(_sz), _vp]),
     "d2g_cmp_set_sparse_detail": (_int, [_vp, _vp, _vp, _vp]),
+    "d2g_cmp_set_fill_detail": (_int, [_vp, _vp, _vp]),
     "d2g_sparse_bin_geometry": (_int, [_sz, C.POINTER(C.c_uint32), C.POINTER(C.c_uint32), C.POINTER(C.c_uint32), C.POINTER(_int)]),
     "d2g_warmup": (_int, [_vp, _int]),
     "d2g_device_name": (_int, [_int, C.c_char_p, _sz]),
@@ -1379,6 +1380,11 @@
         return {"looked": bool(a[0]), "looked_dense": bool(a[1]), "entries": int(a[2]), "family_pairs": int(a[3]), "shared_values": int(a[4]),
                 "planes": int(a[5]), "binned": bool(a[6]), "bin_cshift": int(a[7]), "schedule": "merged" if a[8] else "classic", "prepare_kernels": int(a[9])}
 
+    def fill_detail(self):
+        a = np.zeros(4, np.uint64)
+        self.ctx._check(lib().d2g_cmp_set_fill_detail(self.ctx._h, self._h, a.ctypes.data))
+        return {"announced": int(a[0]), "rank": int(a[1]), "riders": int(a[2]), "launch": int(a[3])}
+
     def debug_pairs(self, cap=1 << 24, stream=None):
         buf = np.empty(cap, np.uint64)
         roots = np.empty(self.N, np.uint32)
diff --git a/dashing2_amd/csrc/d2g_internal.h b/dashing2_amd/csrc/d2g_internal.h
--- a/dashing2_amd/csrc/d2g_internal.h
+++ b/dashing2_amd/csrc/d2g_internal.h
@@ -71,7 +71,8 @@
     double tile_frac = 0.35;
     int olink = 1;
     int emit_big = 0;
-    int ride = 63;
+    int ride = 127;
+    int rank_share = 35;
     int merge = 1;
     int remember = 1;
     size_t long_list = 786432;
diff --git a/dashing2_amd/csrc/d2g_k2.h b/dashing2_amd/csrc/d2g_k2.h
--- a/dashing2_amd/csrc/d2g_k2.h
+++ b/dashing2_amd/csrc/d2g_k2.h
@@ -15,6 +15,9 @@
 #endif
 constexpr unsigned SP_RW_PLAN = 6, SP_RW_FLATTEN = 5, SP_RW_COUNT = 5, SP_RW_ATTACH = 5, SP_RW_SCAN = 8, SP_RW_ALL = 35;
 constexpr unsigned SP_RW_M_LINK0 = D2G_SP_RW_M_LINK0, SP_RW_M_PLANES = D2G_SP_RW_M_PLANES;
+constexpr int BS_RANK_THREADS = 1024, BS_RANK_PF = 12;
+constexpr uint32_t SP_RANK_FILL_PER_WG = (uint32_t)(BS_RANK_PF * BS_RANK_THREADS * 16 / (SP_FILL_THREADS * SP_FILL_PER_THREAD * 16));
+static_assert(SP_RANK_FILL_PER_WG * SP_FILL_THREADS * SP_FILL_PER_THREAD == BS_RANK_PF * BS_RANK_THREADS, "the rank kernel's stores of one workgroup are whole pieces");
 
 struct SpInit {
     uint32_t *label = nullptr, *ones = nullptr, *zero = nullptr;
@@ -43,6 +46,13 @@
     }
     uint32_t riding() const { return total; }
     SpRider take_all() { next = total; return SpRider{out, cnt, vsrc, vimm, 0u, 0u}; }
+    SpRider take_first(unsigned weight, uint64_t cap, uint32_t *n) {
+        *n = 0;
+        if (next != 0 || !total || !(mask & 64)) return SP_NO_RIDER;
+        *n = (uint32_t)std::min<uint64_t>(std::min<uint64_t>(total, cap), ((uint64_t)total * weight + SP_RW_ALL - 1) / SP_RW_ALL);
+        next = *n;
+        return SpRider{out, cnt, vsrc, vimm, 0u, 0u};
+    }
     SpRider take(unsigned own, unsigned weight, bool last, int bit, unsigned *grid) {
         *grid = own;
         if (next >= total || !(mask & bit)) return SP_NO_RIDER;
@@ -79,6 +89,7 @@
     bool pred_valid = false, pred_dense = false; double pred_entries = 0, pred_family_pairs = 0;
     bool big = true;
     bool looked = false, looked_dense = false; uint32_t samp_sums[4] = {0, 0, 0, 0};
+    uint64_t fill_announced = 0, fill_rank = 0, fill_carried = 0;
 };
 
 struct SpState {
@@ -176,6 +187,7 @@
 int  d2g_bitslice_managed_ready(d2g_ctx *ctx, d2g_cmp_set *set, hipStream_t s);
 int  d2g_bitslice_sparse_info(d2g_ctx *ctx, const d2g_cmp_set *set, hipStream_t s, uint32_t *out4);
 int  d2g_bitslice_sparse_detail(d2g_ctx *ctx, const d2g_cmp_set *set, hipStream_t s, uint64_t *out10);
+void d2g_bitslice_fill_detail(const d2g_cmp_set *set, uint64_t *out4);
 SpInit d2g_bitslice_sp_init(const d2g_cmp_set *set);
 int  d2g_bitslice_debug_read(d2g_ctx *ctx, const d2g_cmp_set *set, hipStream_t s, uint64_t *pairs_out, size_t cap, size_t *npairs, uint32_t *root_out);
 int  d2g_bitslice_status(d2g_ctx *ctx, const d2g_cmp_set *set, hipStream_t s);
diff --git a/dashing2_amd/csrc/d2g_k2.hip b/dashing2_amd/csrc/d2g_k2.hip
--- a/dashing2_amd/csrc/d2g_k2.hip
+++ b/dashing2_amd/csrc/d2g_k2.hip
@@ -323,6 +323,15 @@
     for (int x = 0; x < 10; ++x) out10[x] = 0;
     if (set->algo != D2G_CMP_BITSLICE) { D2G_HIP(ctx, hipStreamSynchronize(as_stream(stream))); return D2G_OK; }
     return d2g_bitslice_sparse_detail(ctx, set, as_stream(stream), out10);
+}
+
+int d2g_cmp_set_fill_detail(d2g_ctx *ctx, const d2g_cmp_set *set, uint64_t *out4) {
+    if (!ctx || !out4) return D2G_ERR_INVALID;
+    D2G_CHECK(ctx, set && set->ctx == ctx, "cmp_set_fill_detail: set belongs to another context");
+    D2G_NO_CODE_SET(ctx, set, "cmp_set_fill_detail");
+    for (int x = 0; x < 4; ++x) out4[x] = 0;
+    if (set->algo == D2G_CMP_BITSLICE) d2g_bitslice_fill_detail(set, out4);
+    return D2G_OK;
 }
 
 int d2g_cmp_set_status(d2g_ctx *ctx, const d2g_cmp_set *set, void *stream) {
diff --git a/dashing2_amd/csrc/d2g_k2_bitslice.hip b/dashing2_amd/csrc/d2g_k2_bitslice.hip
--- a/dashing2_amd/csrc/d2g_k2_bitslice.hip
+++ b/dashing2_amd/csrc/d2g_k2_bitslice.hip
@@ -11,7 +11,6 @@
 typedef uint32_t u32x16 __attribute__((ext_vector_type(16)));
 typedef u32x16 __attribute__((aligned(4))) u32x16_u;
 constexpr uint32_t BS_EMPTY = 0xFFFFFFFFu;
-constexpr int BS_RANK_THREADS = 1024;
 
 constexpr uint32_t BS_DUP = 0x80000000u;
 constexpr uint32_t BS_UNIQ = 0x80000000u;
@@ -29,6 +28,24 @@
 }
 
 constexpr uint32_t BS_SPLIT_SHIFT = 28, BS_RANK_MASK = (1u << BS_SPLIT_SHIFT) - 1u;
+typedef uint32_t u32x4 __attribute__((ext_vector_type(4)));
+constexpr int BS_WAIT_VM0 = (0x7 << 4) | (0xF << 8);
+#if defined(__HIP_DEVICE_COMPILE__) && !defined(__GFX9__)
+#error "BS_WAIT_VM0 is the s_waitcnt encoding of the gfx9 family"
+#endif
+struct SpFillAddr { u32x4 *body; size_t nb; uint32_t head, v; };
+constexpr size_t SP_PIECE_VECS = (size_t)SP_FILL_THREADS * SP_FILL_PER_THREAD;
+__device__ __forceinline__ SpFillAddr sp_fill_addr(const SpRider &r) {
+    const size_t head = min(r.cnt, (size_t)((16 - ((uintptr_t)r.out & 15)) & 15) / 4);
+    return SpFillAddr{reinterpret_cast<u32x4 *>(r.out + head), (r.cnt - head) / 4, (uint32_t)head, r.vsrc ? r.vsrc[0] : r.vimm};
+}
+__device__ __forceinline__ void sp_fill_store(const SpFillAddr &a, size_t i) { __builtin_nontemporal_store(u32x4{a.v, a.v, a.v, a.v}, &a.body[i]); }
+__device__ __forceinline__ void sp_fill_ends(const SpRider &r, const SpFillAddr &a) {
+    if (threadIdx.x < a.head) r.out[threadIdx.x] = a.v;
+    const size_t tail0 = a.head + a.nb * 4;
+    if (tail0 + threadIdx.x < r.cnt) r.out[tail0 + threadIdx.x] = a.v;
+}
+
 #ifdef D2G_RANK_TRACE
 __device__ unsigned long long g_rank_trace[8192 * 16];
 #define RK_STAMP(k) do { if (threadIdx.x == 0 && blockIdx.x < 8192 && (k) < 16) g_rank_trace[blockIdx.x * 16 + (k)] = __builtin_amdgcn_s_memrealtime(); } while (0)
@@ -39,7 +56,7 @@
 __global__ __launch_bounds__(BS_RANK_THREADS) void bs_rank_kernel(const uint64_t *__restrict__ cols, size_t N, size_t Npad,
                                                                   uint32_t T, int logT, void *ids_void, uint32_t *colcnt,
                                                                   uint32_t *status, int tagbits_max, uint32_t S, int nsplit,
-                                                                  uint32_t *__restrict__ owner_all, size_t ostride) {
+                                                                  uint32_t *__restrict__ owner_all, size_t ostride, SpRider fill, uint32_t fill_n) {
     extern __shared__ __attribute__((aligned(16))) uint32_t own[];
     const uint32_t split = MULTI ? blockIdx.x / S : 0u;
     const size_t t = MULTI ? blockIdx.x - split * S : blockIdx.x;
@@ -111,8 +128,19 @@
         return h;
     };
 
-    constexpr int PF = 12;
+    constexpr int PF = BS_RANK_PF;
     if constexpr (FAST) {
+        SpFillAddr fa{nullptr, 0, 0u, 0u};
+        uint32_t fcnt = 0;
+        if (fill_n) {
+            fa = sp_fill_addr(fill);
+            if (blockIdx.x == 0) sp_fill_ends(fill, fa);
+            const uint32_t per = (fill_n + gridDim.x - 1) / gridDim.x;
+            const size_t p0 = (size_t)blockIdx.x * per;
+            const size_t b0 = min(p0 * SP_PIECE_VECS, fa.nb), b1 = min(min(p0 + per, (size_t)fill_n) * SP_PIECE_VECS, fa.nb);
+            fa.body += b0;
+            fcnt = b1 > b0 ? (uint32_t)(b1 - b0) : 0u;
+        }
         uint64_t v[PF];
         uint32_t hs[PF];
 #pragma unroll
@@ -122,12 +150,14 @@
         }
         for (uint32_t h = tid; h < Tl; h += BS_RANK_THREADS) own[h] = BS_EMPTY;
         __syncthreads();
+        __builtin_amdgcn_s_waitcnt(BS_WAIT_VM0);
         RK_STAMP(1);
         uint32_t candidate = 0;
 #pragma unroll
         for (int i = 0; i < PF; ++i) {
             const size_t j = (size_t)i * BS_RANK_THREADS + tid;
             hs[i] = 0;
+            if ((uint32_t)(i * BS_RANK_THREADS + tid) < fcnt) sp_fill_store(fa, (uint32_t)(i * BS_RANK_THREADS + tid));
             if (j < N) {
                 const uint64_t prod = v[i] * 0x9E3779B97F4A7C15ull;
                 const uint32_t mine = slot_word(prod, (uint32_t)j);
@@ -315,18 +345,10 @@
 }
 
 __device__ __forceinline__ void sp_ride_piece(const SpRider &r, size_t piece) {
-    typedef uint32_t u32x4 __attribute__((ext_vector_type(4)));
-    const uint32_t v = r.vsrc ? r.vsrc[0] : r.vimm;
-    const size_t head = min(r.cnt, (size_t)((16 - ((uintptr_t)r.out & 15)) & 15) / 4);
-    u32x4 *body = reinterpret_cast<u32x4 *>(r.out + head);
-    const size_t nb = (r.cnt - head) / 4;
-    const size_t end = min((piece + 1) * (size_t)2048, nb);
-    for (size_t i = piece * 2048 + threadIdx.x; i < end; i += blockDim.x) __builtin_nontemporal_store(u32x4{v, v, v, v}, &body[i]);
-    if (piece == 0) {
-        if (threadIdx.x < head) r.out[threadIdx.x] = v;
-        const size_t tail0 = head + nb * 4;
-        if (tail0 + threadIdx.x < r.cnt) r.out[tail0 + threadIdx.x] = v;
-    }
+    const SpFillAddr a = sp_fill_addr(r);
+    const size_t end = min((piece + 1) * SP_PIECE_VECS, a.nb);
+    for (size_t i = piece * SP_PIECE_VECS + threadIdx.x; i < end; i += blockDim.x) sp_fill_store(a, i);
+    if (piece == 0) sp_fill_ends(r, a);
 }
 __device__ __forceinline__ void sp_ride(const SpRider &r) { sp_ride_piece(r, (size_t)r.piece0 + (blockIdx.x - r.own)); }
 #define SP_RIDE_OR_WORK(r) do { if (blockIdx.x >= (r).own) { sp_ride(r); return; } } while (0)
@@ -777,6 +799,8 @@
     if (sp) {
         sp->dec.skip_cached = sparse_path ? (sp_will_skip(ctx, *sp) ? 1 : 0) : -1;
         sp->announced.begin(ctx->k2.ride, sparse_path && sp->dec.skip_cached != 1);
+        const size_t pieces = sp->announced.out ? sp_fill_pieces(sp->announced.cnt) : 0;
+        sp->dec.fill_announced = pieces; sp->dec.fill_rank = sp->dec.fill_carried = 0;
     }
     if (sp && sp->announced.riding() >= SP_SIDE_FILL_PIECES) {
         if (!sp->fill_stream) {
@@ -802,18 +826,24 @@
         const size_t lds = (size_t(1) << logTl) * sizeof(uint32_t);
         const bool id16 = set->id_bits == 16;
         D2G_CHECK(ctx, !(multi && id16), "bitslice: the multi-partition rank kernel with 16-bit ids");
-        void (*kern)(const uint64_t *, size_t, size_t, uint32_t, int, void *, uint32_t *, uint32_t *, int, uint32_t, int, uint32_t *, size_t) = bs_rank_kernel<false, false>;
+        void (*kern)(const uint64_t *, size_t, size_t, uint32_t, int, void *, uint32_t *, uint32_t *, int, uint32_t, int, uint32_t *, size_t, SpRider, uint32_t) = bs_rank_kernel<false, false>;
+        const bool fast = !multi && N <= (size_t)BS_RANK_PF * BS_RANK_THREADS;
         if (multi) kern = bs_rank_kernel<true, false>;
-        else if (N <= (size_t)12 * BS_RANK_THREADS) kern = id16 ? bs_rank_kernel<false, true, uint16_t> : bs_rank_kernel<false, true>;
+        else if (fast) kern = id16 ? bs_rank_kernel<false, true, uint16_t> : bs_rank_kernel<false, true>;
         else if (id16) kern = bs_rank_kernel<false, false, uint16_t>;
         if (lds > 48 * 1024)
             D2G_HIP(ctx, hipFuncSetAttribute((const void *)kern, hipFuncAttributeMaxDynamicSharedMemorySize, (int)lds));
         if (nsplit > 1) D2G_HIP(ctx, hipMemsetAsync(set->d_ids, 0, S * Npad * sizeof(uint32_t), s));
+        const bool look = sparse_path && sp_sample_due(ctx, set);
+        SpRider rank_fill = SP_NO_RIDER; uint32_t rank_n = 0;
+        if (sparse_path && fast && !look && sp->announced.riding() < SP_SIDE_FILL_PIECES)
+            rank_fill = sp->announced.take_first((unsigned)ctx->k2.rank_share, (uint64_t)SP_RANK_FILL_PER_WG * S, &rank_n);
+        D2G_CHECK(ctx, rank_n <= (uint64_t)SP_RANK_FILL_PER_WG * S * nsplit, "bitslice: the rank kernel's share of the fill does not fit its grid");
+        if (sp) sp->dec.fill_rank = rank_n;
         hipLaunchKernelGGL(kern, dim3((unsigned)(S * nsplit)), dim3(BS_RANK_THREADS), lds, s, set->d_cols, N, Npad, set->T, set->logT,
                            (void *)set->d_ids.get(), set->d_colcnt, set->d_meta + set->ntb, ctx->k2.tagbits_max, (uint32_t)S, nsplit,
-                           (sp && nsplit == 1) ? sp->d_owner.get() : (uint32_t *)nullptr, sp ? sp->owner_stride : 0);
+                           (sp && nsplit == 1) ? sp->d_owner.get() : (uint32_t *)nullptr, sp ? sp->owner_stride : 0, rank_fill, rank_n);
         if (sp) sp->dec.kernels = 2 + (join.ev ? 1 : 0);
-        const bool look = sparse_path && sp_sample_due(ctx, set);
         if (look) { if (int rc = sp_sample_enqueue(ctx, set, s)) return rc; if (sp->dec.sample_pending) sp->dec.kernels += 2; }
         const bool merged = sparse_path && !look && ctx->k2.merge && nsplit == 1 && sp->d_owner && ctx->k2.olink && ctx->k2.link && sp->dec.skip_cached != 1;
         if (sp) sp->dec.merged = merged;
@@ -830,6 +860,7 @@
         if (int rc = sp_prepare_order(ctx, set, nsplit > 1, s)) return rc;
         if (int rc = sp_permute(ctx, set, s)) return rc;
         set->srt_valid = true; set->nat_valid = true;
+        sp->dec.fill_carried = sp->announced.next - sp->dec.fill_rank;
         if (sp->announced.riding()) sp->filled.set_by_riders(sp->announced);
         else sp->filled.void_after_prepare();
         sp->announced.served();
@@ -1000,6 +1031,13 @@
     return D2G_OK;
 }
 
+void d2g_bitslice_fill_detail(const d2g_cmp_set *set, uint64_t *out4) {
+    out4[0] = out4[1] = out4[2] = out4[3] = 0;
+    if (!set->sp) return;
+    const SpDecision &d = set->sp->dec;
+    out4[0] = d.fill_announced; out4[1] = d.fill_rank; out4[2] = d.fill_carried; out4[3] = d.fill_announced - d.fill_rank - d.fill_carried;
+}
+
 int d2g_sparse_bin_geometry(size_t N, uint32_t *cshift, uint32_t *nch, uint32_t *nbins, int *binned_ok) {
     if (!N) return D2G_ERR_INVALID;
     const SpBinGeom g = sp_bin_geometry(N);
@@ -1027,7 +1065,7 @@
 uint64_t d2g_k2_tuning_hash(const d2g_ctx *ctx) {
     const d2g_k2_tuning &t = ctx->k2;
     const long long v[] = {t.sparse, (long long)t.min_n, t.link, (long long)(t.tile_frac * 1e6), t.olink, t.emit_big, t.ride, t.remember, (long long)t.list_div, (long long)t.long_list,
-                           t.list_form, t.predict, t.sort ? 1 : 0, t.tagbits_max, t.nsplit_req, t.merge};
+                           t.list_form, t.predict, t.sort ? 1 : 0, t.tagbits_max, t.nsplit_req, t.merge, t.rank_share};
     uint64_t h = 1469598103934665603ull;
     for (long long x : v) for (int b = 0; b < 8; ++b) { h ^= (uint64_t)(x >> (8 * b)) & 0xFF; h *= 1099511628211ull; }
     return h;
@@ -1037,8 +1075,8 @@
     const d2g_k2_tuning &t = ctx->k2;
     char b[640];
     std::snprintf(b, sizeof b, "{\"D2G_BS_SPARSE\": %d, \"D2G_BS_SPARSE_MIN_N\": %zu, \"D2G_BS_SORT\": %d, \"D2G_SP_LINK\": %d, \"D2G_SP_OLINK\": %d, \"D2G_SP_TILE_FRAC\": %.3f, "
-                  "\"D2G_SP_LIST_DIV\": %zu, \"D2G_SP_LONG_LIST\": %zu, \"D2G_SP_LIST_FORM\": %d, \"D2G_SP_PREDICT\": %d, \"D2G_SP_REMEMBER\": %d, \"D2G_SP_RIDE\": %d, \"D2G_SP_EMIT_BIG\": %d, \"D2G_K2_MERGE\": %d, \"D2G_BS_ID16\": %d}",
-                  t.sparse ? 1 : 0, t.min_n, t.sort ? 1 : 0, t.link, t.olink, t.tile_frac, t.list_div, t.long_list, t.list_form, t.predict, t.remember, t.ride, t.emit_big, t.merge, t.id16);
+                  "\"D2G_SP_LIST_DIV\": %zu, \"D2G_SP_LONG_LIST\": %zu, \"D2G_SP_LIST_FORM\": %d, \"D2G_SP_PREDICT\": %d, \"D2G_SP_REMEMBER\": %d, \"D2G_SP_RIDE\": %d, \"D2G_SP_EMIT_BIG\": %d, \"D2G_K2_MERGE\": %d, \"D2G_BS_ID16\": %d, \"D2G_SP_RANK_SHARE\": %d}",
+                  t.sparse ? 1 : 0, t.min_n, t.sort ? 1 : 0, t.link, t.olink, t.tile_frac, t.list_div, t.long_list, t.list_form, t.predict, t.remember, t.ride, t.emit_big, t.merge, t.id16, t.rank_share);
     return b;
 }
 
diff --git a/dashing2_amd/csrc/d2g_runtime.hip b/dashing2_amd/csrc/d2g_runtime.hip
--- a/dashing2_amd/csrc/d2g_runtime.hip
+++ b/dashing2_amd/csrc/d2g_runtime.hip
@@ -6,7 +6,7 @@
 
 static const char *const kTuningNames[] = {
     "D2G_BS_SORT", "D2G_BS_NSPLIT", "D2G_BS_TAGBITS", "D2G_BS_ID16", "D2G_K2_MERGE",
-    "D2G_BS_SPARSE", "D2G_BS_SPARSE_MIN_N", "D2G_SP_LINK", "D2G_SP_TILE_FRAC", "D2G_SP_LIST_DIV", "D2G_SP_LONG_LIST", "D2G_SP_LIST_FORM", "D2G_SP_PREDICT", "D2G_SP_REMEMBER", "D2G_SP_EMIT_BIG", "D2G_SP_OLINK", "D2G_SP_RIDE",
+    "D2G_BS_SPARSE", "D2G_BS_SPARSE_MIN_N", "D2G_SP_LINK", "D2G_SP_TILE_FRAC", "D2G_SP_LIST_DIV", "D2G_SP_LONG_LIST", "D2G_SP_LIST_FORM", "D2G_SP_PREDICT", "D2G_SP_REMEMBER", "D2G_SP_EMIT_BIG", "D2G_SP_OLINK", "D2G_SP_RIDE", "D2G_SP_RANK_SHARE",
     "D2G_MGPU_CHUNKS",
     "D2G_K3_COMPACT", "D2G_K3_L1BITS", "D2G_K3_BUCKET_KEYS", "D2G_K3_SUB_KEYS", "D2G_K3_SPLIT_MIN", "D2G_K3_SUBBATCH", "D2G_K3_ROUND_KEYS",
     "D2G_K3_GUESS_SCALE", "D2G_K3_GRID_PER_CU", "D2G_K3_LIGHT", "D2G_K3_GQ_SCALE",
@@ -29,7 +29,8 @@
     if (const char *e = t.get("D2G_K2_MERGE")) v.merge = std::atoi(e) != 0;
     if (const char *e = t.get("D2G_SP_EMIT_BIG")) v.emit_big = std::atoi(e) != 0;
     if (const char *e = t.get("D2G_SP_REMEMBER")) v.remember = std::atoi(e) != 0;
-    if (const char *e = t.get("D2G_SP_RIDE")) v.ride = std::atoi(e) & 63;
+    if (const char *e = t.get("D2G_SP_RIDE")) v.ride = std::atoi(e) & 127;
+    if (const char *e = t.get("D2G_SP_RANK_SHARE")) { const int d = std::atoi(e); if (d >= 0 && d <= 35) v.rank_share = d; }
     if (const char *e = t.get("D2G_SP_LONG_LIST")) { const long long d = std::atoll(e); if (d >= 0) v.long_list = (size_t)d; }
     if (const char *e = t.get("D2G_SP_PREDICT")) v.predict = std::atoi(e) != 0;
     if (const char *e = t.get("D2G_SP_LIST_FORM")) { const int d = std::atoi(e); if (d >= 0 && d <= 2) v.list_form = d; }
diff --git a/include/d2g.h b/include/d2g.h
--- a/include/d2g.h
+++ b/include/d2g.h
@@ -318,6 +318,7 @@
 int  d2g_cmp_set_sparse_info(d2g_ctx *ctx, const d2g_cmp_set *set, void *stream, uint32_t *info4);
 int  d2g_cmp_set_debug_pairs(d2g_ctx *ctx, const d2g_cmp_set *set, void *stream, uint64_t *pairs_out, size_t cap, size_t *npairs, uint32_t *root_out);
 int  d2g_cmp_set_sparse_detail(d2g_ctx *ctx, const d2g_cmp_set *set, void *stream, uint64_t *out10);
+int  d2g_cmp_set_fill_detail(d2g_ctx *ctx, const d2g_cmp_set *set, uint64_t *out4);
 int  d2g_sparse_bin_geometry(size_t N, uint32_t *cshift, uint32_t *nch, uint32_t *nbins, int *binned_ok);
 int  d2g_operand_layout(size_t N, size_t sketchsize, size_t *group_words, size_t *ngroups);
 int  d2g_cmp_set_export_operand_dev(d2g_ctx *ctx, const d2g_cmp_set *set, uint32_t *planes_out_dev,
```

Result: faster. 213.6 billion (median of 6 runs) (+2.4%).
